# treangenlab/Seqwin

Measured on AMD Instinct MI355X. Metric: Gbp/s minimizer-indexed, higher is better.
Workload: dtype u64

## Files before the change

seqwin_amd/csrc/device.hpp:

```cpp
#pragma once

#include <hip/hip_runtime.h>

#include <functional>
#include <memory>
#include <string>

#include "common.hpp"

namespace sw {

#define SW_HIP(expr)                                                                                   \
    do {                                                                                               \
        hipError_t _e = (expr);                                                                        \
        if (_e != hipSuccess)                                                                          \
            ::sw::raise(SW_ERR_DEVICE, "HIP error %d (%s) at %s:%d: %s", (int)_e, hipGetErrorString(_e), \
                        __FILE__, __LINE__, #expr);                                                    \
    } while (0)

__host__ __device__ inline uint64_t mix64(uint64_t x)
{
    x ^= x >> 30; x *= 0xbf58476d1ce4e5b9ULL;
    x ^= x >> 27; x *= 0x94d049bb133111ebULL;
    x ^= x >> 31;
// ... 94 lines not shown
struct Plan {
    uint32_t k = 0, w = 0;
    uint32_t w_full = 0;
    uint32_t L = 0;
    uint32_t NE = 0;
    uint32_t TW = 0;
    uint32_t Lf = 0, Lg_list = 0, halo_f = 0;
    uint32_t n_tiles = 0, n_tiles_gen = 0;
    struct FastClass {
        uint32_t B = 0;
        uint32_t TW = 0;
        uint32_t n_tiles = 0, n_gap = 0;
        DevArray<uint32_t> rec_off;
        DevArray<TileDesc> desc;
        DevArray<uint32_t> gap_list;
    } fc[2];
    uint64_t n_windows = 0;
    uint64_t n_valid = 0;
    size_t lds_bytes = 0;
    DevArray<uint32_t> rec_seg_off;
    DevArray<uint32_t> rec_nvalid;
    DevArray<uint32_t> rec_tile_off;
    DevArray<uint32_t> gen_tile_off;
    DevArray<uint32_t> gen_tile_rec;
    uint32_t slot_cap = 0;
    DevArray<uint32_t> seg_pos;
    DevArray<uint32_t> seg_idx;
    DevArray<uint64_t> lut;
    DevArray<uint64_t> t4;
    uint64_t mult = 0;
    double build_ms = 0;
};

}

struct sw_batch {
    int device = 0;
    sw::HostBatch host;
    uint64_t n_records = 0;
    uint64_t packed_words = 0;
    sw::DevArray<uint32_t> d_packed;
    sw::DevArray<uint64_t> d_rec_base;
    sw::DevArray<uint32_t> d_rec_asm;
    std::mutex plan_mu;
    std::map<std::pair<uint32_t, uint32_t>, sw::Plan> plans;
};

namespace sw { struct OrderedOcc; }
namespace sw {
bool device_gz_ingest(const char *const *paths, size_t n_paths, uint64_t n_cpu, sw_batch &b);
}

struct sw_occ {
    const sw_batch *batch = nullptr;
    sw::OrderedOcc *occ = nullptr;
    float sketch_ms = 0.f;
    hipStream_t last_stream = nullptr;
    ~sw_occ();
};

namespace sw { struct EdgeHashJob; }
struct sw_index {
    int device = 0;
    uint64_t n_kmers = 0, n_nodes = 0, n_edges = 0;
    sw::DevArray<sw_kmer> kmers;
    sw::DevArray<sw_node> nodes;
    sw::DevArray<sw_edge> edges;
    sw_timings timings{};
    bool ranks_marked = false;
    hipStream_t last_stream = nullptr;
    bool edges_hold_ranks = false;
    sw::EdgeHashJob *hash_job = nullptr;
    sw_index() = default;
    sw_index(const sw_index &) = delete;
    sw_index &operator=(const sw_index &) = delete;
    ~sw_index();
};

namespace sw {

struct MultiGraph {
    std::vector<std::unique_ptr<sw_index>> slices;
    std::vector<uint32_t> record_offsets;
    std::string ids_blob;
    uint64_t n_assemblies = 0, total_bp = 0;
    const char *hash_route = "";
    std::string copy_route;
};
std::vector<int> devices_from_env();
void build_multi_device(const char *const *paths, size_t n_paths, uint64_t k, uint64_t w, uint64_t n_cpu, std::vector<int> devs,
                        MultiGraph &out, uint64_t chunk_bp = 0);

Plan &get_plan(sw_batch &b, uint64_t k, uint64_t w, bool *cached = nullptr);

struct SketchOut {
    DevArray<uint64_t> stage_hash;
    DevArray<uint64_t> stage_kmer;
    DevArray<uint32_t> tile_count;
    DevArray<uint64_t> tile_offset;
    uint64_t n_occ = 0;
    uint64_t launches = 0;
    uint64_t n_ovf_tiles = 0;
};
void run_sketch(const sw_batch &b, const Plan &plan, hipStream_t stream, SketchOut &out, float *sketch_ms);

void radix_sort_keys64(uint64_t *&keys, uint64_t *&alt, uint64_t n, unsigned begin_bit, unsigned end_bit, hipStream_t stream,
                       uint32_t *d_fail, bool perm_hi32 = false, unsigned long long *d_hist_given = nullptr, unsigned layout_bits = 0);
void radix_layout(unsigned bits, unsigned *digit_bits, unsigned *n_passes);
bool radix_unsort_perm(uint64_t *&keys, uint64_t *&alt, uint64_t n, unsigned low_bits, unsigned nbit, hipStream_t stream, uint32_t *d_fail);
constexpr uint32_t UNSORT_CURSOR_STRIDE = 32;
struct UnsortPerm {
    DevArray<unsigned long long> cur_a, cur_b;
    DevArray<uint32_t> tickets;
    unsigned low_bits = 0, hi_bits = 0;
    uint32_t n_groups = 0, n_tiles = 0, grid = 0;
};
bool radix_unsort_perm_begin(UnsortPerm &u, uint64_t n, unsigned low_bits, unsigned nbit, hipStream_t stream);
void radix_unsort_perm_first(UnsortPerm &u, const uint64_t *keys, uint64_t *alt, uint64_t n, hipStream_t stream, uint32_t *d_fail);
void radix_unsort_perm_second(UnsortPerm &u, const uint64_t *keys, uint64_t *alt, uint64_t n, hipStream_t stream, uint32_t *d_fail);

int radix_edge_buckets(uint64_t *&keys, uint64_t *&alt, uint64_t m, unsigned key_bits, uint64_t sentinel,
                       const unsigned long long *d_hist_top, uint32_t cap, uint32_t slots, uint64_t *ukeys, uint32_t *ucnt,
                       uint32_t *n_runs, hipStream_t stream, uint32_t *d_fail, bool debug);

void sort_keys64(uint64_t *&keys, uint64_t *&keys_alt, size_t n, unsigned begin_bit, unsigned end_bit, hipStream_t stream,
                 uint32_t *d_fail, bool perm_hi32 = false, unsigned long long *d_hist_given = nullptr, unsigned layout_bits = 0);
bool sort_keys64_is_own(size_t n);
void check_sort_failed(uint32_t fail_word);

struct alignas(16) OccPay {
    uint32_t low, pos, rec, idx;
};
int radix_rank_mode();
bool radix_pairs_available();
uint64_t radix_trim_state();
void radix_demote_rank();
constexpr uint32_t STAGE_WIN = 32;
constexpr uint32_t STAGE_ROW = STAGE_WIN + 9;
constexpr uint32_t STAGE_PAD = 1;
struct StageSource {
    const uint64_t *stage_hash, *stage_kmer;
    const uint32_t *tile_count;
    const uint64_t *tile_offset;
    const uint64_t *dst_off;
    uint32_t n_tiles;
    uint64_t mult;
    uint32_t *rec_out;
    const unsigned long long *chunk_dir;
    const uint64_t *rows;
};
void radix_sort_pairs32(uint32_t *&keys, uint32_t *&keys_alt, OccPay *&vals, OccPay *&vals_alt, uint64_t n, unsigned end_bit,
                        hipStream_t stream, uint32_t *d_fail, const StageSource *src = nullptr,
                        const std::function<void()> &after_first = std::function<void()>(), uint32_t *low_out = nullptr);
bool sort_pairs32(uint32_t *&keys, uint32_t *&keys_alt, OccPay *&vals, OccPay *&vals_alt, uint64_t n, unsigned end_bit,
                  hipStream_t stream, uint32_t *d_fail, uint32_t *low_out = nullptr);
struct PartState;
void part_state_delete(PartState *p);
uint32_t occ_partition_owners(const struct OrderedOcc &occ);
struct OrderedOcc {
    DevArray<uint64_t> hash;
    DevArray<uint64_t> kmer;
    DevArray<uint32_t> key32;
    DevArray<OccPay> pay;
    DevArray<uint32_t> rec;
    DevArray<uint64_t> cand_rows;
    bool staged = false;
    SketchOut stage;
    DevArray<uint64_t> dst_off;
    uint32_t stage_tiles = 0;
    uint64_t stage_mult = 0;
    uint64_t n = 0;
    PartState *part = nullptr;
    OrderedOcc() = default;
    OrderedOcc(OrderedOcc &&o) noexcept { *this = std::move(o); }
    OrderedOcc &operator=(OrderedOcc &&o) noexcept
    {
        if (this != &o) {
            hash = std::move(o.hash); kmer = std::move(o.kmer); key32 = std::move(o.key32); pay = std::move(o.pay);
            rec = std::move(o.rec); cand_rows = std::move(o.cand_rows); n = o.n; o.n = 0;
            staged = o.staged; o.staged = false; stage = std::move(o.stage); dst_off = std::move(o.dst_off);
            stage_tiles = o.stage_tiles; stage_mult = o.stage_mult;
            part_state_delete(part); part = o.part; o.part = nullptr;
        }
        return *this;
    }
    ~OrderedOcc() { part_state_delete(part); }
};
void order_tuples(SketchOut &sk, const Plan &plan, hipStream_t stream, OrderedOcc &out, bool index_form = false, bool take_stage = false);
void concat_occ(std::vector<OrderedOcc> &chunks, const std::vector<uint64_t> &rec_base, hipStream_t stream, OrderedOcc &out);
void build_index(const uint32_t *d_rec_asm, uint64_t n_records, uint64_t n_assemblies, OrderedOcc &occ,
                 const uint8_t *d_is_target, uint64_t n_targets, uint64_t n_non_targets, hipStream_t stream, sw_index &ix);
void pack_export(const sw_node *nodes, uint64_t n_nodes, uint64_t n_kmers, const sw_edge *edges, uint64_t n_edges, uint64_t per, uint32_t *pn,
                 uint64_t *bases, uint32_t *pe, uint32_t *flag, hipStream_t stream);
void device_get_penalty(const sw_kmer *d_kmers, uint64_t n_kmers, sw_node *d_nodes, uint64_t n_nodes,
                        const uint32_t *d_rec_asm, uint64_t n_records, const uint8_t *d_is_target,
                        uint64_t n_targets, uint64_t n_non_targets, hipStream_t stream, uint64_t *err_flags_host);
void device_filter_kmers(const sw_kmer *d_kmers, uint64_t n_kmers, const sw_node *d_nodes, uint64_t n_nodes,
                         const uint64_t *d_used_sorted, uint64_t n_used, hipStream_t stream,
                         DevArray<sw_kmer> &kmers_out, DevArray<sw_node> &nodes_out, uint64_t *n_kmers_out,
                         uint64_t *n_nodes_out);
void device_identity(const sw_index &ix, hipStream_t stream, uint64_t *sums2, uint64_t kbase = 0, uint64_t nbase = 0);
void slice_get_penalty(sw_index &ix, uint64_t kmer_base, const uint32_t *d_rec_asm, uint64_t n_records, const uint8_t *d_is_target,
                       uint64_t n_targets, uint64_t n_non_targets, hipStream_t stream, uint64_t *err_flags_host);
void device_checksums(const sw_index &ix, hipStream_t stream, uint64_t *sums3, uint64_t kbase = 0, uint64_t nbase = 0,
                      uint64_t ebase = 0);
void index_threshold_sums(const sw_index &ix, hipStream_t stream, uint64_t *sums3);
void index_verify(const sw_index &ix, uint64_t n_assemblies, bool scored, hipStream_t stream, uint64_t *out10);
void index_filter_graph(const sw_index &ix, uint64_t weight_th, hipStream_t stream, sw_index &out);
void index_occ_rows(const sw_index &ix, uint64_t rec_offset, uint64_t *d_rows, hipStream_t stream);
void index_splits(const sw_index &ix, const uint64_t *node_bounds, const uint64_t *edge_bounds, uint32_t n_bounds,
                  uint64_t *occ_split, uint64_t *edge_split, hipStream_t stream);
void merge_build(const uint64_t *d_occ_rows, uint64_t n, const uint64_t *d_edge_rows, uint64_t m, uint64_t kmer_base,
                 const uint32_t *d_rec_asm, uint64_t n_records, const uint8_t *d_is_target, uint64_t n_targets,
                 uint64_t n_non_targets, hipStream_t stream, sw_index &ix, uint32_t *d_rank_out = nullptr);
void occ_partition(const OrderedOcc &occ, const uint64_t *bounds, uint32_t n_bounds, uint64_t rec_offset, uint64_t *d_rows,
                   uint32_t *d_perm, uint64_t *counts_host, hipStream_t stream);
void occ_adjacency(const OrderedOcc &occ, const uint32_t *d_rec_asm, const uint32_t *d_perm, const uint32_t *d_rank_by_row,
                   unsigned nb, unsigned ab, uint64_t asm_base, const uint64_t *rank_bounds, uint32_t n_bounds,
                   uint64_t *d_rows_out, uint64_t *counts_host, hipStream_t stream);
void slice_edges(sw_index &ix, const uint64_t *d_adj_rows, uint64_t m, unsigned nb, unsigned ab, const uint64_t *d_rank_hash,
                 hipStream_t stream);
void occ_adjacency_pairs(OrderedOcc &occ, const uint32_t *d_rec_asm, const uint32_t *d_rank_by_row, const uint64_t *node_base,
                         uint64_t asm_base, const uint64_t *rank_bounds, uint32_t n_bounds, uint64_t *d_keys_out,
                         uint64_t *counts_host, uint64_t *cand_counts_host, uint64_t *key_bits_host, hipStream_t stream);
void slice_edges_pairs(sw_index &ix, uint64_t *d_keys, uint64_t m, const uint64_t *d_cand_rows, uint64_t c, unsigned lo_bits,
                       unsigned hi_bits, uint64_t lo_base, unsigned ab, const uint64_t *d_rank_hash, const uint64_t *node_base,
                       uint32_t n_owners, uint64_t pad, hipStream_t stream);
void index_node_hashes(const sw_index &ix, uint64_t *d_out, hipStream_t stream);
void subgraphs_csr(const sw_subgraphs *sg, int *device, uint64_t *n_sg, uint64_t *n_out, const uint64_t **offsets, const uint64_t **hashes);
uint64_t edge_hash_requests(sw_index &ix, const uint64_t *node_base, uint32_t n_owners, uint64_t *counts_host, hipStream_t stream);
void edge_hash_request_rows(const sw_index &ix, uint32_t *d_out, hipStream_t stream);
void node_hash_lookup(const sw_index &ix, const uint32_t *d_local_ranks, uint64_t n, uint64_t *d_out, hipStream_t stream);
void edge_hash_attach(sw_index &ix, const uint64_t *d_replies, uint64_t n, hipStream_t stream);

}
```

seqwin_amd/csrc/index.hip:

```cpp
#include <cstdlib>
#include <cstring>
#include <map>
#include <memory>

#include <rocprim/rocprim.hpp>

#include "device.hpp"

namespace sw {

namespace {

constexpr int TPB = 256;
inline unsigned blocks_for(uint64_t n, int per = TPB) { return (unsigned)((n + per - 1) / per); }
inline bool ranks_by_table()
{
    const char *e = SW_TEST_GETENV("SEQWIN_AMD_RANKS");
    return e && !strcmp(e, "table");
}

template <class K, class V>
void sort_pairs(K *&keys, K *&keys_alt, V *&vals, V *&vals_alt, size_t n, unsigned begin_bit, unsigned end_bit,
                hipStream_t stream)
{
    rocprim::double_buffer<K> dk(keys, keys_alt);
    rocprim::double_buffer<V> dv(vals, vals_alt);
    size_t tmp_bytes = 0;
    SW_HIP(rocprim::radix_sort_pairs(nullptr, tmp_bytes, dk, dv, n, begin_bit, end_bit, stream));
    DevArray<unsigned char> tmp(tmp_bytes);
    SW_HIP(rocprim::radix_sort_pairs(tmp.p, tmp_bytes, dk, dv, n, begin_bit, end_bit, stream));
    keys = dk.current();
    keys_alt = dk.alternate();
    vals = dv.current();
    vals_alt = dv.alternate();
}

}

bool sort_keys64_is_own(size_t n)
{
    const char *e = SW_TEST_GETENV("SEQWIN_AMD_SORT");
    const bool own = e ? !strcmp(e, "own") : n >= (1ull << 23);
    return own && !(e && !strcmp(e, "rocprim"));
}

void sort_keys64(uint64_t *&keys, uint64_t *&keys_alt, size_t n, unsigned begin_bit, unsigned end_bit, hipStream_t stream,
                 uint32_t *d_fail, bool perm_hi32, unsigned long long *d_hist_given, unsigned layout_bits)
{
    if (sort_keys64_is_own(n)) {
        radix_sort_keys64(keys, keys_alt, n, begin_bit, end_bit, stream, d_fail, perm_hi32, d_hist_given, layout_bits);
        return;
    }
    rocprim::double_buffer<uint64_t> dk(keys, keys_alt);
    size_t tmp_bytes = 0;
    SW_HIP(rocprim::radix_sort_keys(nullptr, tmp_bytes, dk, n, begin_bit, end_bit, stream));
    DevArray<unsigned char> tmp(tmp_bytes);
    SW_HIP(rocprim::radix_sort_keys(tmp.p, tmp_bytes, dk, n, begin_bit, end_bit, stream));
    keys = dk.current();
    keys_alt = dk.alternate();
}

bool sort_pairs_is_own(size_t n, unsigned bits)
{
    const char *e = SW_TEST_GETENV("SEQWIN_AMD_PAIR_SORT"), *all = SW_TEST_GETENV("SEQWIN_AMD_SORT");
    if (e && !strcmp(e, "rocprim")) return false;
    if (bits % 8 != 0 || bits > 32 || n >= 0xFFFFFFFFull) return false;
    bool own = n >= (1ull << 20);
    if (all) own = !strcmp(all, "own");
    if (e && !strcmp(e, "own")) own = true;
    return own && radix_pairs_available();
}

bool sort_pairs32(uint32_t *&keys, uint32_t *&keys_alt, OccPay *&vals, OccPay *&vals_alt, uint64_t n, unsigned end_bit,
                  hipStream_t stream, uint32_t *d_fail, uint32_t *low_out)
{
    if (sort_pairs_is_own(n, end_bit)) {
        radix_sort_pairs32(keys, keys_alt, vals, vals_alt, n, end_bit, stream, d_fail, nullptr, std::function<void()>(), low_out);
        return low_out != nullptr && n != 0 && end_bit != 0;
    }
    sort_pairs(keys, keys_alt, vals, vals_alt, n, 0, end_bit, stream);
    return false;
}

void check_sort_failed(uint32_t fail_word)
{
    if (fail_word)
        raise(SW_ERR_RUNTIME, "internal error: a radix pass gave up waiting for a lower-numbered workgroup (set SEQWIN_AMD_SORT=rocprim)");
}

namespace {

template <class InIt, class OutIt, class T>
void inclusive_sum(InIt in, OutIt out, size_t n, T, hipStream_t stream)
{
    size_t tmp_bytes = 0;
    SW_HIP(rocprim::inclusive_scan(nullptr, tmp_bytes, in, out, n, rocprim::plus<T>(), stream));
    DevArray<unsigned char> tmp(tmp_bytes);
    SW_HIP(rocprim::inclusive_scan(tmp.p, tmp_bytes, in, out, n, rocprim::plus<T>(), stream));
}

template <class InIt, class OutIt, class T>
void inclusive_sum_keep(InIt in, OutIt out, size_t n, T, hipStream_t stream, DevArray<unsigned char> &tmp)
{
    size_t tmp_bytes = 0;
    SW_HIP(rocprim::inclusive_scan(nullptr, tmp_bytes, in, out, n, rocprim::plus<T>(), stream));
    tmp.alloc(tmp_bytes);
    SW_HIP(rocprim::inclusive_scan(tmp.p, tmp_bytes, in, out, n, rocprim::plus<T>(), stream));
}

template <class InIt, class OutIt, class T>
void exclusive_sum(InIt in, OutIt out, size_t n, T init, hipStream_t stream)
{
    size_t tmp_bytes = 0;
    SW_HIP(rocprim::exclusive_scan(nullptr, tmp_bytes, in, out, init, n, rocprim::plus<T>(), stream));
    DevArray<unsigned char> tmp(tmp_bytes);
    SW_HIP(rocprim::exclusive_scan(tmp.p, tmp_bytes, in, out, init, n, rocprim::plus<T>(), stream));
}

struct U32ToU64 {
    __host__ __device__ uint64_t operator()(uint32_t v) const { return v; }
};

struct HeadFlag {
    const uint64_t *keys;
    uint64_t sentinel;
    __host__ __device__ uint32_t operator()(uint64_t s) const
    {
        const uint64_t k = keys[s];
        return (k != sentinel && (s == 0 || k != keys[s - 1])) ? 1u : 0u;
    }
};

template <bool INDEX, bool RAW = false>
__global__ void k_order(const uint64_t *__restrict__ stage_hash, const uint64_t *__restrict__ stage_kmer,
                        const uint32_t *__restrict__ tile_count, const uint64_t *__restrict__ tile_offset,
                        const uint64_t *__restrict__ dst_off, uint32_t n_tiles, uint64_t mult, uint64_t *__restrict__ hash,
                        uint64_t *__restrict__ kmer, uint32_t *__restrict__ key32, OccPay *__restrict__ pay,
                        uint32_t *__restrict__ rec)
{
    const uint32_t wave = (blockIdx.x * blockDim.x + threadIdx.x) >> 6;
    const uint32_t lane = threadIdx.x & 63u;
    if (wave >= n_tiles) return;
    const uint32_t c = tile_count[wave];
    const uint64_t src = tile_offset[wave], dst = dst_off[wave];
    for (uint32_t i = lane; i < c; i += 64) {
        uint64_t h = stage_hash[src + i];
        if (!RAW) {
            h *= mult;
            h ^= h >> 27;
        }
        const uint64_t km = stage_kmer[src + i];
        if (INDEX) {
            key32[dst + i] = (uint32_t)(h >> 32);
            OccPay p;
            p.low = (uint32_t)h;
            p.pos = (uint32_t)km;
            p.rec = (uint32_t)(km >> 32);
            p.idx = (uint32_t)(dst + i);
            pay[dst + i] = p;
            rec[dst + i] = p.rec;
            if (hash) hash[dst + i] = h;
        } else {
            hash[dst + i] = h;
            kmer[dst + i] = km;
        }
    }
}

__global__ void k_rows_to_pay(const uint64_t *__restrict__ rows, uint64_t n, uint32_t *__restrict__ key32, OccPay *__restrict__ pay)
{
    const uint64_t i = (uint64_t)blockIdx.x * blockDim.x + threadIdx.x;
    if (i >= n) return;
    const uint64_t h = rows[2 * i], km = rows[2 * i + 1];
    key32[i] = (uint32_t)(h >> 32);
    OccPay p;
    p.low = (uint32_t)h;
    p.pos = (uint32_t)km;
    p.rec = (uint32_t)(km >> 32);
    p.idx = (uint32_t)i;
    pay[i] = p;
}

__global__ void k_iota(uint32_t *v, uint64_t n)
{
    const uint64_t i = (uint64_t)blockIdx.x * blockDim.x + threadIdx.x;
    if (i < n) v[i] = (uint32_t)i;
}

#ifndef SW_NODES_ROWS
#define SW_NODES_ROWS 4
#endif
constexpr int NODES_ROWS = SW_NODES_ROWS;
constexpr int NODES_THREADS = 1024;
constexpr int NODES_WAVES = NODES_THREADS / 64;
constexpr uint32_t NODES_ROW = NODES_THREADS * 2;
constexpr uint32_t NODES_TILE = NODES_ROW * NODES_ROWS;
constexpr uint32_t UNSORT_BITS = 14;
constexpr uint32_t UNSORT_RANGE = 1u << UNSORT_BITS;
constexpr bool UNSORT_FUSED_DEFAULT = true;
constexpr uint64_t UNSORT_DIRECT_MAX = 1ull << 25;

constexpr unsigned long long TS_AGG = 1ull << 62, TS_INC = 2ull << 62;

__device__ __forceinline__ unsigned long long interleave32(uint32_t a, uint32_t b)
{
    unsigned long long x = a, y = b;
    x = (x | (x << 16)) & 0x0000FFFF0000FFFFull; y = (y | (y << 16)) & 0x0000FFFF0000FFFFull;
    x = (x | (x << 8)) & 0x00FF00FF00FF00FFull;  y = (y | (y << 8)) & 0x00FF00FF00FF00FFull;
    x = (x | (x << 4)) & 0x0F0F0F0F0F0F0F0Full;  y = (y | (y << 4)) & 0x0F0F0F0F0F0F0F0Full;
    x = (x | (x << 2)) & 0x3333333333333333ull;  y = (y | (y << 2)) & 0x3333333333333333ull;
    x = (x | (x << 1)) & 0x5555555555555555ull;  y = (y | (y << 1)) & 0x5555555555555555ull;
    return x | (y << 1);
}

constexpr uint32_t RANK_REP = 0x80000000u;
constexpr uint8_t OWNER_DROP = 0xFF;
constexpr uint32_t NODES_DIGITS = 256;
struct NodesScat {
    uint64_t stage[NODES_TILE];
    unsigned long long goff[NODES_DIGITS];
    uint32_t cnt[NODES_DIGITS];
    uint32_t lstart[NODES_DIGITS];
};
template <bool BITS, bool REP, bool SCAT = false>
__global__ __launch_bounds__(NODES_THREADS) void k_nodes(const uint32_t *__restrict__ key32, const OccPay *__restrict__ pay, uint64_t n,
                                               uint64_t base, const uint32_t *__restrict__ rec_flag, sw_kmer *__restrict__ kmers,
                                               uint64_t *__restrict__ node_hash, uint32_t *__restrict__ node_start,
                                               uint32_t *__restrict__ rank_direct,
                                               uint64_t *__restrict__ uval,
                                               unsigned long long *__restrict__ tbits, unsigned long long *__restrict__ nbits,
                                               unsigned long long *__restrict__ tile_state, uint32_t *__restrict__ ticket,
                                               uint32_t *__restrict__ n_nodes_out, uint32_t *__restrict__ order_bad,
                                               unsigned long long *__restrict__ cursor, uint32_t dig_shift, uint32_t dig_mask)
{
    __shared__ uint32_t s_tile, s_excl;
    __shared__ uint32_t s_row[NODES_ROWS * NODES_WAVES];
    static_assert(NODES_ROWS * NODES_WAVES <= 128, "the (row, wave) group counts are scanned by one wave, two per lane");
    const uint32_t lane = threadIdx.x & 63u, wave = threadIdx.x >> 6;
    NodesScat *sc = nullptr;
    if constexpr (SCAT) {
        __shared__ NodesScat s_scat;
        sc = &s_scat;
        if (threadIdx.x < NODES_DIGITS) sc->cnt[threadIdx.x] = 0;
    }
    if (threadIdx.x == 0) s_tile = atomicAdd(ticket, 1u);
    __syncthreads();
    const uint32_t tile = s_tile;
    const uint64_t s0 = (uint64_t)tile * NODES_TILE;
    uint32_t k[NODES_ROWS][2], within[NODES_ROWS], headm = 0, prec[NODES_ROWS];
    OccPay p[NODES_ROWS][2];
    unsigned long long misorder = 0;
#pragma unroll
    for (int r = 0; r < NODES_ROWS; ++r) {
        const uint64_t s = s0 + (uint64_t)r * NODES_ROW + 2 * threadIdx.x;
        k[r][0] = k[r][1] = 0;
        p[r][0] = p[r][1] = OccPay{0, 0, 0, 0};
        if (s + 1 < n) {
            const uint2 kk = *reinterpret_cast<const uint2 *>(key32 + s);
            k[r][0] = kk.x;
            k[r][1] = kk.y;
            p[r][0] = pay[s];
            p[r][1] = pay[s + 1];
        } else if (s < n) {
            k[r][0] = key32[s];
            p[r][0] = pay[s];
        }
        uint32_t pk = __shfl_up(k[r][1], 1, 64), plow = __shfl_up(p[r][1].low, 1, 64), pidx = __shfl_up(p[r][1].idx, 1, 64);
        prec[r] = __shfl_up(p[r][1].rec, 1, 64);
        if (lane == 0 && s < n && s) {
            pk = key32[s - 1];
            const OccPay q = pay[s - 1];
            plow = q.low;
            prec[r] = q.rec;
            pidx = q.idx;
        }
        const bool h0 = s < n && (s == 0 || k[r][0] != pk || p[r][0].low != plow);
        const bool h1 = s + 1 < n && (k[r][1] != k[r][0] || p[r][1].low != p[r][0].low);
#ifndef SW_NO_ORDER_GUARD
        {
            const unsigned long long hp = ((unsigned long long)pk << 32) | plow, h0v = ((unsigned long long)k[r][0] << 32) | p[r][0].low,
                                     h1v = ((unsigned long long)k[r][1] << 32) | p[r][1].low;
            const bool bad0 = s < n && s && (h0v < hp || (!h0 && p[r][0].idx <= pidx));
            const bool bad1 = s + 1 < n && (h1v < h0v || (!h1 && p[r][1].idx <= p[r][0].idx));
            misorder |= __ballot(bad0 || bad1);
        }
#else
        (void)pidx;
#endif
        const unsigned long long b0 = __ballot(h0), b1 = __ballot(h1), lt = (1ull << lane) - 1ull;
        within[r] = (uint32_t)__popcll(b0 & lt) + (uint32_t)__popcll(b1 & lt);
        if (h0) headm |= 1u << (2 * r);
        if (h1) headm |= 2u << (2 * r);
        if (lane == 0) s_row[r * NODES_WAVES + wave] = (uint32_t)__popcll(b0) + (uint32_t)__popcll(b1);
    }
    if (misorder && lane == 0) atomicAdd(order_bad, (uint32_t)__popcll(misorder));
    uint32_t drank[NODES_ROWS][2];
    if constexpr (SCAT) {
#pragma unroll
        for (int r = 0; r < NODES_ROWS; ++r)
#pragma unroll
            for (int e = 0; e < 2; ++e) {
                drank[r][e] = 0;
                if (s0 + (uint64_t)r * NODES_ROW + 2 * threadIdx.x + e < n)
                    drank[r][e] = atomicAdd(&sc->cnt[(p[r][e].idx >> dig_shift) & dig_mask], 1u);
            }
    }
    __syncthreads();
    if (SCAT && wave == 1) {
        const uint4 c4 = reinterpret_cast<const uint4 *>(sc->cnt)[lane];
        const uint32_t c[4] = {c4.x, c4.y, c4.z, c4.w};
        unsigned long long g[4];
#pragma unroll
        for (int j = 0; j < 4; ++j)
            g[j] = c[j] ? atomicAdd(&cursor[(size_t)(4 * lane + j) * UNSORT_CURSOR_STRIDE], (unsigned long long)c[j]) : 0ull;
        uint32_t incl = c[0] + c[1] + c[2] + c[3];
        for (uint32_t d = 1; d < 64; d <<= 1) {
            const uint32_t up = __shfl_up(incl, d, 64);
            if (lane >= d) incl += up;
        }
        uint32_t before = incl - (c[0] + c[1] + c[2] + c[3]);
#pragma unroll
        for (int j = 0; j < 4; ++j) {
            sc->lstart[4 * lane + j] = before;
            sc->goff[4 * lane + j] = g[j] - before;
            before += c[j];
        }
    }
    if (wave == 0) {
        constexpr uint32_t GROUPS = NODES_ROWS * NODES_WAVES;
        const uint32_t c0 = (2 * lane < GROUPS) ? s_row[2 * lane] : 0u, c1 = (2 * lane + 1 < GROUPS) ? s_row[2 * lane + 1] : 0u;
        uint32_t incl = c0 + c1;
        for (uint32_t d = 1; d < 64; d <<= 1) {
            const uint32_t up = __shfl_up(incl, d, 64);
            if (lane >= d) incl += up;
        }
        const uint32_t total = __shfl(incl, 63, 64);
        if (2 * lane < GROUPS) s_row[2 * lane] = incl - c0 - c1;
        if (2 * lane + 1 < GROUPS) s_row[2 * lane + 1] = incl - c1;
        if (lane == 0)
            __hip_atomic_store(&tile_state[tile], (tile == 0 ? TS_INC : TS_AGG) | total, __ATOMIC_RELAXED, __HIP_MEMORY_SCOPE_AGENT);
        uint32_t excl = 0;
        if (tile) {
            int64_t look = (int64_t)tile - 1;
            for (;;) {
                const int64_t idx = look - lane;
                const unsigned long long st = idx >= 0 ? __hip_atomic_load(&tile_state[idx], __ATOMIC_RELAXED, __HIP_MEMORY_SCOPE_AGENT)
                                                       : TS_INC;
                const unsigned long long inc = __ballot((st >> 62) == 2), none = __ballot((st >> 62) == 0);
                const uint32_t first_inc = inc ? (uint32_t)__builtin_ctzll(inc) : 64u;
                const unsigned long long needed = first_inc >= 63 ? ~0ull : ((2ull << first_inc) - 1ull);
                if (none & needed) {
                    __builtin_amdgcn_s_sleep(2);
                    continue;
                }
                uint32_t v = (lane <= first_inc) ? (uint32_t)st : 0u;
                for (int d = 32; d; d >>= 1) v += __shfl_xor(v, d, 64);
                excl += v;
                if (first_inc < 64) break;
                look -= 64;
            }
            if (lane == 0)
                __hip_atomic_store(&tile_state[tile], TS_INC | (unsigned long long)(excl + total), __ATOMIC_RELAXED,
                                   __HIP_MEMORY_SCOPE_AGENT);
        }
        if (lane == 0) {
            s_excl = excl;
            if (s0 + NODES_TILE >= n) *n_nodes_out = excl + total;
        }
    }
    __syncthreads();
    const uint32_t excl = s_excl;
    if constexpr (SCAT) {
#pragma unroll
        for (int r = 0; r < NODES_ROWS; ++r)
#pragma unroll
            for (int e = 0; e < 2; ++e) drank[r][e] += sc->lstart[(p[r][e].idx >> dig_shift) & dig_mask];
    }
#pragma unroll
    for (int r = 0; r < NODES_ROWS; ++r) {
        const uint64_t s = s0 + (uint64_t)r * NODES_ROW + 2 * threadIdx.x;
        const bool live0 = s < n, live1 = s + 1 < n;
        const bool h0 = (headm >> (2 * r)) & 1u, h1 = (headm >> (2 * r + 1)) & 1u;
        const uint32_t nid0 = excl + s_row[r * NODES_WAVES + wave] + within[r] + (h0 ? 1u : 0u) - 1u;
        const uint32_t nid1 = nid0 + (h1 ? 1u : 0u);
        uint32_t w0 = nid0, w1 = nid1;
        uint32_t f0 = 0, f1 = 0, pf = 0;
        if (BITS || REP) {
            f0 = live0 ? rec_flag[p[r][0].rec] : 0u;
            f1 = live1 ? rec_flag[p[r][1].rec] : 0u;
            pf = __shfl_up(f1, 1, 64);
            if (lane == 0 && live0 && s) pf = rec_flag[prec[r]];
        }
        if (REP) {
            uint32_t nk = __shfl_down(k[r][0], 1, 64), nlow = __shfl_down(p[r][0].low, 1, 64), nf = __shfl_down(f0, 1, 64);
            bool nlive = __shfl_down((int)live0, 1, 64) != 0;
            if (lane == 63) {
                nlive = s + 2 < n;
                if (nlive) {
                    nk = key32[s + 2];
                    const OccPay q = pay[s + 2];
                    nlow = q.low;
                    nf = rec_flag[q.rec];
                }
            }
            const bool same01 = live1 && !h1 && (f1 >> 1) == (f0 >> 1);
            const bool same_p0 = live0 && !h0 && (f0 >> 1) == (pf >> 1);
            const bool same_1n = live1 && nlive && nk == k[r][1] && nlow == p[r][1].low && (nf >> 1) == (f1 >> 1);
            if (same_p0 || same01) w0 |= RANK_REP;
            if (same01 || same_1n) w1 |= RANK_REP;
        }
        if (live1) {
            *reinterpret_cast<uint4 *>(kmers + s) = make_uint4(p[r][0].pos, p[r][0].rec, p[r][1].pos, p[r][1].rec);
            if (!SCAT && uval)
                *reinterpret_cast<ulonglong2 *>(uval + s) = make_ulonglong2(((uint64_t)p[r][0].idx << 32) | w0,
                                                                          ((uint64_t)p[r][1].idx << 32) | w1);
        } else if (live0) {
            sw_kmer km;
            km.pos = p[r][0].pos;
            km.record_idx = p[r][0].rec;
            kmers[s] = km;
            if (!SCAT && uval) uval[s] = ((uint64_t)p[r][0].idx << 32) | w0;
        }
        if constexpr (SCAT) {
            if (live0) sc->stage[drank[r][0]] = ((uint64_t)p[r][0].idx << 32) | w0;
            if (live1) sc->stage[drank[r][1]] = ((uint64_t)p[r][1].idx << 32) | w1;
        }
        if (rank_direct) {
            if (live0) rank_direct[p[r][0].idx] = w0;
            if (live1) rank_direct[p[r][1].idx] = w1;
        }
#pragma unroll
        for (int e = 0; e < 2; ++e) {
            const bool head = e ? h1 : h0;
            if (head) {
                const uint32_t nid = e ? nid1 : nid0;
                node_hash[nid] = ((uint64_t)k[r][e] << 32) | p[r][e].low;
                node_start[nid] = (uint32_t)(s + e);
            }
        }
        if (BITS) {
            const bool first0 = live0 && (h0 || (f0 >> 1) != (pf >> 1)), first1 = live1 && (h1 || (f1 >> 1) != (f0 >> 1));
            const unsigned long long t0 = __ballot(first0 && (f0 & 1u)), t1 = __ballot(first1 && (f1 & 1u));
            const unsigned long long g0 = __ballot(first0 && !(f0 & 1u)), g1 = __ballot(first1 && !(f1 & 1u));
            if (lane == 0 && live0) {
                const uint64_t wd = s >> 6;
                tbits[wd] = interleave32((uint32_t)t0, (uint32_t)t1);
                nbits[wd] = interleave32((uint32_t)g0, (uint32_t)g1);
                if (s + 64 < n) {
                    tbits[wd + 1] = interleave32((uint32_t)(t0 >> 32), (uint32_t)(t1 >> 32));
                    nbits[wd + 1] = interleave32((uint32_t)(g0 >> 32), (uint32_t)(g1 >> 32));
                }
            }
        }
    }
    if constexpr (SCAT) {
        asm volatile("s_waitcnt lgkmcnt(0)" ::: "memory");
        __builtin_amdgcn_s_barrier();
        asm volatile("" ::: "memory");
        const uint32_t cnt_tile = (uint32_t)min((uint64_t)NODES_TILE, n - s0);
        constexpr int OUT = NODES_TILE / NODES_THREADS;
        uint64_t word[OUT], at[OUT];
#pragma unroll
        for (int j = 0; j < OUT; ++j) word[j] = sc->stage[j * NODES_THREADS + threadIdx.x];
#pragma unroll
        for (int j = 0; j < OUT; ++j) at[j] = sc->goff[(uint32_t)(word[j] >> (32 + dig_shift)) & dig_mask] + (j * NODES_THREADS + threadIdx.x);
#pragma unroll
        for (int j = 0; j < OUT; ++j)
            if (j * NODES_THREADS + threadIdx.x < cnt_tile && at[j] < n) uval[at[j]] = word[j];
    }
}

__device__ __forceinline__ uint32_t popc_range(const unsigned long long *__restrict__ w, uint64_t a, uint64_t b)
{
    if (a >= b) return 0;
    const uint64_t wa = a >> 6, wb = (b - 1) >> 6;
    const unsigned long long ma = ~0ull << (a & 63u), mb = ~0ull >> (63u - ((b - 1) & 63u));
    if (wa == wb) return (uint32_t)__popcll(w[wa] & ma & mb);
    uint32_t c = (uint32_t)__popcll(w[wa] & ma) + (uint32_t)__popcll(w[wb] & mb);
    for (uint64_t i = wa + 1; i < wb; ++i) c += (uint32_t)__popcll(w[i]);
    return c;
}

constexpr int FIN_THREADS = 256;
template <bool BITS>
__global__ __launch_bounds__(FIN_THREADS) void k_finish_nodes(sw_node *__restrict__ nodes, uint64_t n_nodes, const uint64_t *__restrict__ node_hash,
                                                              const uint32_t *__restrict__ node_start, uint64_t base, uint64_t end,
                                                              const unsigned long long *__restrict__ tbits,
                                                              const unsigned long long *__restrict__ nbits, double inv_tar, double inv_neg)
{
    static_assert(sizeof(sw_node) == 40, "five 8-byte words per node");
    __shared__ __align__(16) unsigned long long stage[FIN_THREADS * 5];
    const uint64_t i0 = (uint64_t)blockIdx.x * FIN_THREADS, i = i0 + threadIdx.x;
    if (i < n_nodes) {
        const uint32_t a = node_start[i];
        const uint64_t b = i + 1 < n_nodes ? (uint64_t)node_start[i + 1] : end - base;
        uint32_t n_tar = 0, n_neg = 0;
        double pen = 0.0;
        if (BITS) {
            n_tar = popc_range(tbits, a, b);
            n_neg = popc_range(nbits, a, b);
            {
#pragma clang fp contract(off)
                const double ft = (double)n_tar * inv_tar;
                const double fn = (double)n_neg * inv_neg;
                const double omf = 1.0 - ft;
                const double aa = omf * omf;
                const double bb = fn * fn;
                const double sum = aa + bb;
                pen = __dsqrt_rn(sum);
            }
        }
        unsigned long long *w = stage + threadIdx.x * 5;
        w[0] = node_hash[i];
        w[1] = base + a;
        w[2] = base + b;
        w[3] = ((unsigned long long)n_neg << 32) | n_tar;
        w[4] = (unsigned long long)__double_as_longlong(pen);
    }
    __syncthreads();
    const uint64_t cnt = min((uint64_t)FIN_THREADS, n_nodes - i0);
    const uint32_t n16 = (uint32_t)(cnt * 40 / 16), tail8 = (uint32_t)((cnt * 40) % 16) / 8;
    uint4 *dst = reinterpret_cast<uint4 *>(nodes + i0);
    const uint4 *src = reinterpret_cast<const uint4 *>(stage);
    for (uint32_t t = threadIdx.x; t < n16; t += FIN_THREADS) dst[t] = src[t];
    if (tail8 && threadIdx.x == 0) reinterpret_cast<unsigned long long *>(nodes + i0)[n16 * 2] = stage[n16 * 2];
}

__global__ void k_rec_flag(const uint32_t *__restrict__ rec_asm, const uint8_t *__restrict__ is_target, uint64_t n_records,
                           uint32_t *__restrict__ rec_flag)
{
    const uint64_t r = (uint64_t)blockIdx.x * blockDim.x + threadIdx.x;
    if (r < n_records) {
        const uint32_t a = rec_asm[r];
        rec_flag[r] = (a << 1) | ((is_target && is_target[a]) ? 1u : 0u);
    }
}

constexpr unsigned long long TABLE_EMPTY = ~0ull;
__device__ __forceinline__ uint64_t table_mix(uint64_t x)
{
    return x ^ (x >> 29);
}

__global__ void k_table_build(const sw_node *__restrict__ nodes, uint64_t n_nodes, ulonglong2 *__restrict__ slots, uint64_t mask,
                              uint32_t *__restrict__ rank_of_empty_key)
{
    const uint64_t r = (uint64_t)blockIdx.x * blockDim.x + threadIdx.x;
    if (r >= n_nodes) return;
    const unsigned long long h = nodes[r].hash;
    if (h == TABLE_EMPTY) {
        *rank_of_empty_key = (uint32_t)r;
        return;
    }
    uint64_t s = table_mix(h) & mask;
    for (;;) {
// ... 942 lines not shown
    nd.start = ns;
    nd.stop = ns + sz;
    nodes_out[o] = nd;
}

__global__ void k_filter_kmers(const sw_kmer *__restrict__ kmers, const uint64_t *__restrict__ src_start,
                               const uint64_t *__restrict__ dst_start, uint64_t n_kept, uint64_t n_out,
                               sw_kmer *__restrict__ out)
{
    const uint64_t j = (uint64_t)blockIdx.x * blockDim.x + threadIdx.x;
    if (j >= n_out) return;
    uint64_t lo = 0, hi = n_kept;
    while (hi - lo > 1) {
        const uint64_t mid = (lo + hi) >> 1;
        if (dst_start[mid] <= j) lo = mid; else hi = mid;
    }
    out[j] = kmers[src_start[lo] + (j - dst_start[lo])];
}

__global__ void k_checksum(const sw_kmer *kmers, uint64_t nk, const sw_node *nodes, uint64_t nn, const sw_edge *edges,
                           uint64_t ne, uint64_t kbase, uint64_t nbase, uint64_t ebase, unsigned long long *sums)
{
    const uint64_t i = (uint64_t)blockIdx.x * blockDim.x + threadIdx.x;
    uint64_t a = 0, b = 0, c = 0;
    if (i < nk) a = ck_kmer(kbase + i, kmers[i]);
    if (i < nn) b = ck_node(nbase + i, nodes[i]);
    if (i < ne) c = ck_edge(ebase + i, edges[i]);
    for (int d = 32; d; d >>= 1) {
        a += __shfl_down(a, d, 64);
        b += __shfl_down(b, d, 64);
        c += __shfl_down(c, d, 64);
    }
    if ((threadIdx.x & 63u) == 0) {
        if (a) atomicAdd(&sums[0], (unsigned long long)a);
        if (b) atomicAdd(&sums[1], (unsigned long long)b);
        if (c) atomicAdd(&sums[2], (unsigned long long)c);
    }
}

__global__ void k_verify_nodes(const sw_node *__restrict__ nodes, uint64_t n_nodes, uint64_t n_kmers, uint64_t base,
                               uint64_t n_assemblies, int scored, uint32_t *__restrict__ start_bits,
                               unsigned long long *__restrict__ out)
{
    const uint64_t i = (uint64_t)blockIdx.x * blockDim.x + threadIdx.x;
    if (i >= n_nodes) return;
    const sw_node nd = nodes[i];
    if (i && !(nodes[i - 1].hash < nd.hash)) atomicAdd(&out[0], 1ull);
    const uint64_t prev_stop = i ? nodes[i - 1].stop : base;
    bool bad = nd.start != prev_stop || nd.stop <= nd.start || nd.stop - base > n_kmers;
    if (i == n_nodes - 1 && nd.stop - base != n_kmers) bad = true;
    if (bad) atomicAdd(&out[1], 1ull);
    else atomicOr(&start_bits[(nd.start - base) >> 5], 1u << ((nd.start - base) & 31u));
    if (scored) {
        const uint64_t c = (uint64_t)nd.n_tar + nd.n_neg, size = nd.stop - nd.start;
        if (c < 1 || c > size || c > n_assemblies) atomicAdd(&out[7], 1ull);
    }
}

__global__ void k_verify_kmers(const sw_kmer *__restrict__ kmers, uint64_t n, const uint32_t *__restrict__ start_bits,
                               unsigned long long *__restrict__ out)
{
    const uint64_t s = (uint64_t)blockIdx.x * blockDim.x + threadIdx.x;
    unsigned long long bad = 0, first_of_record = 0;
    if (s < n) {
        const uint64_t cur = ((uint64_t)kmers[s].record_idx << 32) | kmers[s].pos;
        const bool head = (start_bits[s >> 5] >> (s & 31u)) & 1u;
        if (s && !head) {
            const uint64_t prev = ((uint64_t)kmers[s - 1].record_idx << 32) | kmers[s - 1].pos;
            if (!(prev < cur)) bad = 1;
        }
    }
    (void)first_of_record;
    for (int d = 32; d; d >>= 1) bad += __shfl_down(bad, d, 64);
    if ((threadIdx.x & 63u) == 0 && bad) atomicAdd(&out[2], bad);
}

__global__ void k_verify_edges(const sw_edge *__restrict__ edges, uint64_t n_edges, const sw_node *__restrict__ nodes,
                               uint64_t n_nodes, const uint64_t *__restrict__ rank_hash, uint64_t n_rank_hash,
                               uint64_t n_assemblies, unsigned long long *__restrict__ out)
{
    const uint64_t e = (uint64_t)blockIdx.x * blockDim.x + threadIdx.x;
    unsigned long long wsum = 0;
    if (e < n_edges) {
        const sw_edge ed = edges[e];
        if (e) {
            const sw_edge pe = edges[e - 1];
            if (!(pe.first < ed.first || (pe.first == ed.first && pe.second < ed.second))) atomicAdd(&out[3], 1ull);
        }
        if (ed.first > ed.second) atomicAdd(&out[4], 1ull);
        if (ed.weight < 1 || ed.weight > n_assemblies) atomicAdd(&out[5], 1ull);
        wsum = ed.weight;
        for (int side = 0; side < 2; ++side) {
            const uint64_t h = side ? ed.second : ed.first;
            bool found;
            if (rank_hash) {
                uint64_t lo = 0, hi = n_rank_hash;
                while (lo < hi) {
                    const uint64_t mid = (lo + hi) >> 1;
                    if (rank_hash[mid] < h) lo = mid + 1; else hi = mid;
                }
                found = lo < n_rank_hash && rank_hash[lo] == h;
            } else {
                const uint64_t lo = node_index_of(nodes, n_nodes, h);
                found = lo < n_nodes && nodes[lo].hash == h;
            }
            if (!found) atomicAdd(&out[6], 1ull);
        }
    }
    for (int d = 32; d; d >>= 1) wsum += __shfl_down(wsum, d, 64);
    if ((threadIdx.x & 63u) == 0 && wsum) atomicAdd(&out[8], wsum);
}

__global__ void k_rot_keys(uint32_t *__restrict__ key32, uint64_t n, unsigned left)
{
    const uint64_t i = (uint64_t)blockIdx.x * blockDim.x + threadIdx.x;
    if (i < n) {
        const uint32_t k = key32[i];
        key32[i] = (k << left) | (k >> (32u - left));
    }
}

constexpr uint32_t DESC_BLOCK = 1024;

struct PayView {
    using Key = uint32_t;
    using Elem = OccPay;
    uint32_t *key32;
    OccPay *pay;
    __device__ uint32_t key(uint64_t q) const { return key32[q]; }
    __device__ uint64_t low(uint64_t q) const { return pay[q].low; }
    __device__ static uint64_t low_of(const OccPay &v) { return v.low; }
    __device__ void load(uint64_t q, uint32_t &k, OccPay &v) const { k = key32[q]; v = pay[q]; }
    __device__ void store(uint64_t q, uint32_t k, const OccPay &v) const { key32[q] = k; pay[q] = v; }
};
struct LowView {
    using Key = uint32_t;
    const uint32_t *key32;
    const uint32_t *low32;
    __device__ uint32_t key(uint64_t q) const { return key32[q]; }
    __device__ uint64_t low(uint64_t q) const { return low32[q]; }
};
struct EdgeKeyView {
    using Key = uint64_t;
    using Elem = uint64_t;
    uint64_t *keys;
    unsigned low_bits;
    __device__ uint64_t key(uint64_t q) const { return keys[q] >> low_bits; }
    __device__ uint64_t low(uint64_t q) const { return keys[q]; }
    __device__ static uint64_t low_of(const uint64_t &v) { return v; }
    __device__ void load(uint64_t q, uint64_t &k, uint64_t &v) const { v = keys[q]; k = v >> low_bits; }
    __device__ void store(uint64_t q, uint64_t, const uint64_t &v) const { keys[q] = v; }
};

template <class View>
__device__ __forceinline__ uint32_t descents_of_thread(const View &V, typename View::Key kmask, uint64_t n, uint64_t q0, uint32_t *heads = nullptr)
{
    uint32_t m = 0, hm = 0;
    if (heads) *heads = 0;
    if (q0 >= n) return 0;
    typename View::Key kp = q0 ? V.key(q0 - 1) : 0;
    uint64_t lp = q0 ? V.low(q0 - 1) : 0;
#pragma unroll
    for (uint32_t i = 0; i < 4; ++i) {
        const uint64_t q = q0 + i;
        if (q >= n) break;
        const typename View::Key kq = V.key(q);
        const uint64_t lq = V.low(q);
        if (q && (kq & kmask) == (kp & kmask) && (kq < kp || (kq == kp && lq < lp))) m |= 1u << i;
        if (q == 0 || kq != kp || lq != lp) hm |= 1u << i;
        kp = kq;
        lp = lq;
    }
    if (heads) *heads = (uint32_t)__popc(hm);
    return m;
}

__device__ __forceinline__ uint32_t descents_of_thread(const PayView &V, uint32_t kmask, uint64_t n, uint64_t q0, uint32_t *heads = nullptr)
{
    uint32_t m = 0, hm = 0;
    if (heads) *heads = 0;
    if (q0 >= n) return 0;
    uint32_t kq[4];
    uint64_t lq[4];
    if (q0 + 4 <= n) {
        const uint4 kv = *reinterpret_cast<const uint4 *>(V.key32 + q0);
        kq[0] = kv.x; kq[1] = kv.y; kq[2] = kv.z; kq[3] = kv.w;
#pragma unroll
        for (uint32_t i = 0; i < 4; ++i) lq[i] = reinterpret_cast<const uint4 *>(V.pay + q0 + i)->x;
    } else {
#pragma unroll
        for (uint32_t i = 0; i < 4; ++i) {
            kq[i] = (q0 + i < n) ? V.key32[q0 + i] : 0u;
            lq[i] = (q0 + i < n) ? V.pay[q0 + i].low : 0u;
        }
    }
    uint32_t kp = q0 ? V.key32[q0 - 1] : 0;
    uint64_t lp = q0 ? V.pay[q0 - 1].low : 0;
#pragma unroll
    for (uint32_t i = 0; i < 4; ++i) {
        const uint64_t q = q0 + i;
        if (q >= n) break;
        if (q && (kq[i] & kmask) == (kp & kmask) && (kq[i] < kp || (kq[i] == kp && lq[i] < lp))) m |= 1u << i;
        if (q == 0 || kq[i] != kp || lq[i] != lp) hm |= 1u << i;
        kp = kq[i];
        lp = lq[i];
    }
    if (heads) *heads = (uint32_t)__popc(hm);
    return m;
}

__device__ __forceinline__ uint32_t descents_of_thread(const LowView &V, uint32_t kmask, uint64_t n, uint64_t q0, uint32_t *heads = nullptr)
{
    uint32_t m = 0, hm = 0;
    if (heads) *heads = 0;
    if (q0 >= n) return 0;
    uint32_t kq[4], lq[4];
    if (q0 + 4 <= n) {
        const uint4 kv = *reinterpret_cast<const uint4 *>(V.key32 + q0), lv = *reinterpret_cast<const uint4 *>(V.low32 + q0);
        kq[0] = kv.x; kq[1] = kv.y; kq[2] = kv.z; kq[3] = kv.w;
        lq[0] = lv.x; lq[1] = lv.y; lq[2] = lv.z; lq[3] = lv.w;
    } else {
#pragma unroll
        for (uint32_t i = 0; i < 4; ++i) {
            kq[i] = (q0 + i < n) ? V.key32[q0 + i] : 0u;
            lq[i] = (q0 + i < n) ? V.low32[q0 + i] : 0u;
        }
    }
    uint32_t kp = q0 ? V.key32[q0 - 1] : 0, lp = q0 ? V.low32[q0 - 1] : 0;
#pragma unroll
    for (uint32_t i = 0; i < 4; ++i) {
        const uint64_t q = q0 + i;
        if (q >= n) break;
        if (q && (kq[i] & kmask) == (kp & kmask) && (kq[i] < kp || (kq[i] == kp && lq[i] < lp))) m |= 1u << i;
        if (q == 0 || kq[i] != kp || lq[i] != lp) hm |= 1u << i;
        kp = kq[i];
        lp = lq[i];
    }
    if (heads) *heads = (uint32_t)__popc(hm);
    return m;
}

constexpr uint32_t DESC_SLOT = 4;
template <class View>
__global__ __launch_bounds__(256) void k_count_descents(const View V, typename View::Key kmask, uint64_t n, unsigned long long *__restrict__ cnt,
                                                        uint32_t *__restrict__ slot_q, uint32_t *__restrict__ slot_k)
{
    const uint64_t q0 = (uint64_t)blockIdx.x * DESC_BLOCK + threadIdx.x * 4u;
    uint32_t heads = 0;
    const uint32_t m = descents_of_thread(V, kmask, n, q0, &heads);
    const uint32_t c = (uint32_t)__popc(m);
    __shared__ unsigned long long s;
    __shared__ uint32_t s_n, s_q[DESC_SLOT], s_kk[DESC_SLOT];
    if (threadIdx.x == 0) {
        s = 0;
        s_n = 0;
    }
    __syncthreads();
    unsigned long long w = ((unsigned long long)heads << 32) | c;
    for (int d = 32; d; d >>= 1) w += __shfl_down(w, d, 64);
    if ((threadIdx.x & 63u) == 0 && w) atomicAdd(&s, w);
    __syncthreads();
    const uint32_t dc = (uint32_t)s;
    if (threadIdx.x == 0) cnt[blockIdx.x] = s;
    if (dc == 0 || dc > DESC_SLOT) return;
    uint32_t mm = m;
    while (mm) {
        const uint32_t i = (uint32_t)__builtin_ctz(mm);
        mm &= mm - 1;
        const uint32_t at = atomicAdd(&s_n, 1u);
        s_q[at] = (uint32_t)(q0 + i);
        s_kk[at] = (uint32_t)(V.key(q0 + i) & kmask);
    }
    __syncthreads();
    if (threadIdx.x == 0) {
        for (uint32_t i = 1; i < dc; ++i)
            for (uint32_t j = i; j > 0 && s_q[j] < s_q[j - 1]; --j) {
                const uint32_t tq = s_q[j], tk = s_kk[j];
                s_q[j] = s_q[j - 1];
                s_kk[j] = s_kk[j - 1];
                s_q[j - 1] = tq;
                s_kk[j - 1] = tk;
            }
        for (uint32_t i = 0; i < dc; ++i) {
            slot_q[(size_t)blockIdx.x * DESC_SLOT + i] = s_q[i];
            slot_k[(size_t)blockIdx.x * DESC_SLOT + i] = s_kk[i];
        }
    }
}

template <class View>
__global__ __launch_bounds__(256) void k_list_descents(const View V, typename View::Key kmask, uint64_t n,
                                                       const unsigned long long *__restrict__ cnt,
                                                       const unsigned long long *__restrict__ off, uint32_t n_blocks,
                                                       uint32_t *__restrict__ bad, uint32_t cap, uint32_t *__restrict__ bad_q,
                                                       uint32_t cap_q, unsigned long long *__restrict__ n_desc,
                                                       const uint32_t *__restrict__ slot_q, const uint32_t *__restrict__ slot_k)
{
    const uint32_t b = blockIdx.x;
    const uint32_t c_blk = (uint32_t)cnt[b];
    if (b == n_blocks - 1 && threadIdx.x == 0) {
        const unsigned long long tot = off[b] + cnt[b];
        n_desc[0] = tot & 0xFFFFFFFFull;
        n_desc[1] = tot >> 32;
    }
    if (c_blk == 0) return;
    if (c_blk <= DESC_SLOT) {
        if (threadIdx.x < c_blk) {
            const uint32_t at = (uint32_t)off[b] + threadIdx.x;
            if (bad && at < cap) bad[at] = slot_k[(size_t)b * DESC_SLOT + threadIdx.x];
            if (at < cap_q) bad_q[at] = slot_q[(size_t)b * DESC_SLOT + threadIdx.x];
        }
        return;
    }
    const uint64_t q0 = (uint64_t)b * DESC_BLOCK + threadIdx.x * 4u;
    const uint32_t m = descents_of_thread(V, kmask, n, q0);
    const uint32_t c = (uint32_t)__popc(m);
    __shared__ uint32_t wsum[4];
    const uint32_t lane = threadIdx.x & 63u, wave = threadIdx.x >> 6;
    uint32_t incl = c;
    for (uint32_t d = 1; d < 64; d <<= 1) {
        const uint32_t up = __shfl_up(incl, d, 64);
        if (lane >= d) incl += up;
    }
    if (lane == 63) wsum[wave] = incl;
    __syncthreads();
    uint32_t base = (uint32_t)off[b] + (incl - c);
    for (uint32_t i = 0; i < wave; ++i) base += wsum[i];
    uint32_t mm = m;
    while (mm) {
        const uint32_t i = (uint32_t)__builtin_ctz(mm);
        mm &= mm - 1;
        if (base < cap) bad[base] = (uint32_t)(V.key(q0 + i) & kmask);
        if (base < cap_q) bad_q[base] = (uint32_t)(q0 + i);
        ++base;
    }
}

constexpr uint32_t REPAIR_MAX_DESC = 1u << 26;
constexpr uint32_t REPAIR_MAX_MID = 1u << 22;
constexpr uint32_t REPAIR_THREAD_RUN = 6;
constexpr uint32_t REPAIR_MAX_RUN = 2048;
constexpr uint32_t REPAIR_GRID = 2048;

__device__ __forceinline__ uint64_t readlane64(uint64_t v, uint32_t lane)
{
    const uint32_t lo = (uint32_t)__builtin_amdgcn_readlane((int)(uint32_t)v, (int)lane);
    const uint32_t hi = (uint32_t)__builtin_amdgcn_readlane((int)(uint32_t)(v >> 32), (int)lane);
    return ((uint64_t)hi << 32) | lo;
}

__device__ __forceinline__ uint32_t readlane_key(uint32_t v, uint32_t lane) { return (uint32_t)__builtin_amdgcn_readlane((int)v, (int)lane); }
__device__ __forceinline__ uint64_t readlane_key(uint64_t v, uint32_t lane) { return readlane64(v, lane); }

template <class View>
__global__ __launch_bounds__(256) void k_repair_thread(const View V, typename View::Key kmask, uint64_t n, const uint32_t *__restrict__ bad_q,
                                                       const unsigned long long *__restrict__ n_desc, uint32_t *__restrict__ mid,
                                                       uint32_t *__restrict__ n_mid, uint32_t *__restrict__ status)
{
// ... 95 lines not shown
        if (have) {
            V.load(a + lane, ki, vi);
            li = View::low_of(vi);
        }
        uint32_t rank = 0;
        for (uint32_t j = 0; j < len; ++j) {
            const typename View::Key kj = readlane_key(ki, j);
            const uint64_t lj = readlane64(li, j);
            rank += (kj < ki || (kj == ki && (lj < li || (lj == li && j < lane)))) ? 1u : 0u;
        }
        if (have) V.store(a + rank, ki, vi);
    }
}

constexpr uint32_t REPAIR_MAX_VALUES = 12;
template <class View>
__global__ __launch_bounds__(256) void k_repair_sort(const View V, const uint32_t *__restrict__ n_big, const uint32_t *__restrict__ big)
{
    __shared__ typename View::Elem sv[REPAIR_MAX_RUN];
    __shared__ typename View::Key sk[REPAIR_MAX_RUN];
    __shared__ uint16_t srank[REPAIR_MAX_RUN];
    __shared__ typename View::Key w_k[4];
    __shared__ uint32_t w_cnt[4];
    __shared__ uint64_t w_l[4];
    const uint32_t B = *n_big;
    const uint32_t tid = threadIdx.x, lane = tid & 63u, wave = tid >> 6;
    for (uint32_t b = blockIdx.x; b < B; b += gridDim.x) {
        const uint32_t a = big[2 * b], len = big[2 * b + 1];
        __syncthreads();
        for (uint32_t i = tid; i < len; i += blockDim.x) V.load(a + i, sk[i], sv[i]);
        __syncthreads();
        const uint32_t per = (len + 255u) / 256u, i0 = min(len, tid * per), i1 = min(len, i0 + per);
        uint32_t placed = 0;
        typename View::Key last_k = 0;
        uint64_t last_l = 0;
        bool have_last = false;
        for (uint32_t it = 0; it < REPAIR_MAX_VALUES && placed < len; ++it) {
            typename View::Key mk = ~(typename View::Key)0;
            uint64_t ml = ~0ull;
            bool any = false;
            for (uint32_t i = i0; i < i1; ++i) {
                const typename View::Key k = sk[i];
                const uint64_t l = View::low_of(sv[i]);
                if (have_last && !(k > last_k || (k == last_k && l > last_l))) continue;
                if (!any || k < mk || (k == mk && l < ml)) {
                    mk = k;
                    ml = l;
                    any = true;
                }
            }
            for (int d = 32; d; d >>= 1) {
                const typename View::Key ok = __shfl_xor(mk, d, 64);
                const uint64_t ol = __shfl_xor(ml, d, 64);
                const bool oany = __shfl_xor((int)any, d, 64) != 0;
                if (oany && (!any || ok < mk || (ok == mk && ol < ml))) {
                    mk = ok;
                    ml = ol;
                    any = true;
                }
            }
            __syncthreads();
            if (lane == 0) {
                w_k[wave] = mk;
                w_l[wave] = ml;
                w_cnt[wave] = any ? 1u : 0u;
            }
            __syncthreads();
            any = false;
            for (uint32_t w = 0; w < 4; ++w)
                if (w_cnt[w] && (!any || w_k[w] < mk || (w_k[w] == mk && w_l[w] < ml))) {
                    mk = w_k[w];
                    ml = w_l[w];
                    any = true;
                }
            uint32_t c = 0;
            for (uint32_t i = i0; i < i1; ++i) c += (sk[i] == mk && View::low_of(sv[i]) == ml) ? 1u : 0u;
            uint32_t incl = c;
            for (uint32_t d = 1; d < 64; d <<= 1) {
                const uint32_t up = __shfl_up(incl, d, 64);
                if (lane >= d) incl += up;
            }
            __syncthreads();
            if (lane == 63) w_cnt[wave] = incl;
            __syncthreads();
            uint32_t before = placed + incl - c, total = 0;
            for (uint32_t w = 0; w < 4; ++w) {
                if (w < wave) before += w_cnt[w];
                total += w_cnt[w];
            }
            for (uint32_t i = i0; i < i1; ++i)
                if (sk[i] == mk && View::low_of(sv[i]) == ml) srank[i] = (uint16_t)before++;
            placed += total;
            last_k = mk;
            last_l = ml;
            have_last = true;
        }
        __syncthreads();
        if (placed == len) {
            for (uint32_t i = tid; i < len; i += blockDim.x) V.store(a + srank[i], sk[i], sv[i]);
        } else {
            for (uint32_t i = tid; i < len; i += blockDim.x) {
                const typename View::Key ki = sk[i];
                const typename View::Elem vi = sv[i];
                const uint64_t li = View::low_of(vi);
                uint32_t rank = 0;
                for (uint32_t j = 0; j < len; ++j) {
                    const typename View::Key kj = sk[j];
                    const uint64_t lj = View::low_of(sv[j]);
                    rank += (kj < ki || (kj == ki && (lj < li || (lj == li && j < i)))) ? 1u : 0u;
                }
                V.store(a + rank, ki, vi);
            }
        }
    }
}

struct RepairState {
    DevArray<unsigned long long> n_desc;
    DevArray<unsigned long long> blk_cnt, blk_off;
    DevArray<uint32_t> slot_q, slot_k;
    DevArray<uint32_t> bad_q, mid, big, status;
};

template <class View, class Sweep>
void enqueue_repair(const View &V, const Sweep &W, typename View::Key kmask, uint64_t n, uint32_t *bad, uint32_t cap, RepairState &r,
                    hipStream_t stream)
{
    const uint32_t n_blocks = (uint32_t)((n + DESC_BLOCK - 1) / DESC_BLOCK);
    const uint32_t max_desc = (uint32_t)std::min<uint64_t>(REPAIR_MAX_DESC, std::max<uint64_t>(n, 1));
    const uint32_t max_mid = std::min(max_desc, REPAIR_MAX_MID);
    r.bad_q.alloc(max_desc);
    r.mid.alloc(max_mid);
    r.big.alloc(2 * (size_t)max_mid);
    r.n_desc.alloc(2);
    r.status.alloc(3);
    r.blk_cnt.alloc(n_blocks);
    r.blk_off.alloc(n_blocks);
    r.slot_q.alloc((size_t)n_blocks * DESC_SLOT);
    r.slot_k.alloc((size_t)n_blocks * DESC_SLOT);
    SW_HIP(hipMemsetAsync(r.status.p, 0, 12, stream));
    hipLaunchKernelGGL(k_count_descents<Sweep>, dim3(n_blocks), dim3(256), 0, stream, W, kmask, n, r.blk_cnt.p, r.slot_q.p, r.slot_k.p);
    SW_HIP(hipGetLastError());
    exclusive_sum(r.blk_cnt.p, r.blk_off.p, n_blocks, 0ull, stream);
    hipLaunchKernelGGL(k_list_descents<Sweep>, dim3(n_blocks), dim3(256), 0, stream, W, kmask, n, r.blk_cnt.p, r.blk_off.p,
                       n_blocks, bad, cap, r.bad_q.p, max_desc, r.n_desc.p, r.slot_q.p, r.slot_k.p);
    hipLaunchKernelGGL(k_repair_thread<View>, dim3(REPAIR_GRID), dim3(256), 0, stream, V, kmask, n, r.bad_q.p, r.n_desc.p, r.mid.p,
                       r.status.p + 2, r.status.p);
    hipLaunchKernelGGL(k_repair_wave<View>, dim3(REPAIR_GRID), dim3(256), 0, stream, V, kmask, n, r.bad_q.p, r.n_desc.p,
                       (const uint32_t *)r.mid.p, (const uint32_t *)(r.status.p + 2), r.big.p, r.status.p + 1, r.status.p);
    hipLaunchKernelGGL(k_repair_sort<View>, dim3(REPAIR_GRID), dim3(256), 0, stream, V, r.status.p + 1, r.big.p);
    SW_HIP(hipGetLastError());
}

__global__ void k_bad_runs(const uint32_t *__restrict__ bad, uint32_t n_bad, const uint32_t *__restrict__ key32,
                           uint32_t kmask, uint64_t n, uint32_t *__restrict__ run_start, uint32_t *__restrict__ run_len)
{
    const uint32_t i = blockIdx.x * blockDim.x + threadIdx.x;
    if (i >= n_bad) return;
    const uint32_t k = bad[i];
    if (i && bad[i - 1] == k) {
        run_start[i] = 0;
        run_len[i] = 0;
        return;
    }
    uint64_t lo = 0, hi = n;
    while (lo < hi) {
        const uint64_t mid = (lo + hi) >> 1;
        if ((key32[mid] & kmask) < k) lo = mid + 1; else hi = mid;
    }
    const uint64_t a = lo;
    hi = n;
    while (lo < hi) {
        const uint64_t mid = (lo + hi) >> 1;
        if ((key32[mid] & kmask) <= k) lo = mid + 1; else hi = mid;
    }
    run_start[i] = (uint32_t)a;
    run_len[i] = (uint32_t)(lo - a);
}

__global__ void k_gather_sub(const uint32_t *__restrict__ key32, const OccPay *__restrict__ pay,
                             const uint32_t *__restrict__ run_start, const uint64_t *__restrict__ run_off, uint32_t n_bad,
                             uint64_t n_sub, uint64_t *__restrict__ sub_h, OccPay *__restrict__ sub_v,
                             uint32_t *__restrict__ pos)
{
    const uint64_t t = (uint64_t)blockIdx.x * blockDim.x + threadIdx.x;
    if (t >= n_sub) return;
    uint64_t q = t;
    if (run_off) {
        uint32_t lo = 0, hi = n_bad;
        while (hi - lo > 1) {
            const uint32_t mid = (lo + hi) >> 1;
            if (run_off[mid] <= t) lo = mid; else hi = mid;
        }
        q = (uint64_t)run_start[lo] + (t - run_off[lo]);
        pos[t] = (uint32_t)q;
    }
    const OccPay v = pay[q];
    sub_h[t] = ((uint64_t)key32[q] << 32) | v.low;
    sub_v[t] = v;
}

__global__ void k_scatter_sub(const uint64_t *__restrict__ sub_h, const OccPay *__restrict__ sub_v,
                              const uint32_t *__restrict__ pos, uint64_t n_sub, uint32_t *__restrict__ key32,
                              OccPay *__restrict__ pay)
{
    const uint64_t t = (uint64_t)blockIdx.x * blockDim.x + threadIdx.x;
    if (t >= n_sub) return;
    const uint64_t q = pos ? pos[t] : t;
    key32[q] = (uint32_t)(sub_h[t] >> 32);
    pay[q] = sub_v[t];
}

struct PaySort {
    DevArray<uint32_t> key_a, key_b;
    DevArray<OccPay> pay_a, pay_b;
    uint32_t *key32 = nullptr;
    OccPay *pay = nullptr;
    uint64_t n_repaired = 0;
    DevArray<uint32_t> bad;
    RepairState rep;
    uint32_t cap = 0, kmask = ~0u;
    uint64_t n = 0;
    DevArray<uint32_t> fail;
    DevArray<uint32_t> low;
    const uint64_t *rows_src = nullptr;
    OrderedOcc *staged = nullptr;
};

void sort_pay(uint64_t n, hipStream_t stream, PaySort &o)
{
    unsigned bits = 32;
    if (const char *e = SW_TEST_GETENV("SEQWIN_AMD_SORT_KEYBITS")) {
        const int b = atoi(e);
        if (b >= 1 && b <= 32) bits = (unsigned)b;
    }
    o.kmask = ~0u << (32 - bits);
    o.n = n;
    o.key_b.alloc(n);
    o.pay_b.alloc(n);
    uint32_t *keys = o.key_a.p, *keys_alt = o.key_b.p;
    OccPay *vals = o.pay_a.p, *vals_alt = o.pay_b.p;
    bool have_low = false;
    const bool want_low = bits == 32 && !(SW_AB_GETENV("SEQWIN_AMD_DESC_LOW") && atoi(SW_AB_GETENV("SEQWIN_AMD_DESC_LOW")) == 0);
    if (o.staged) {
        OrderedOcc &occ = *o.staged;
        StageSource S{};
        S.stage_hash = occ.stage.stage_hash.p;
        S.stage_kmer = occ.stage.stage_kmer.p;
        S.tile_count = occ.stage.tile_count.p;
        S.tile_offset = occ.stage.tile_offset.p;
        S.dst_off = occ.dst_off.p;
        S.n_tiles = occ.stage_tiles;
        S.mult = occ.stage_mult;
        S.rec_out = occ.rec.p;
        o.fail.alloc(1);
        SW_HIP(hipMemsetAsync(o.fail.p, 0, 4, stream));
        if (want_low) o.low.alloc(n);
        have_low = want_low && n != 0;
        radix_sort_pairs32(keys, keys_alt, vals, vals_alt, n, 32, stream, o.fail.p, &S, [&] {
            occ.stage = SketchOut();
            occ.dst_off.release();
            occ.staged = false;
            o.key_a.alloc(n);
            o.pay_a.alloc(n);
            keys = o.key_a.p;
            vals = o.pay_a.p;
        }, o.low.p);
        o.staged = nullptr;
    } else if (o.rows_src) {
        StageSource S{};
        S.rows = o.rows_src;
        o.fail.alloc(1);
        SW_HIP(hipMemsetAsync(o.fail.p, 0, 4, stream));
        if (want_low) o.low.alloc(n);
        have_low = want_low && n != 0;
        radix_sort_pairs32(keys, keys_alt, vals, vals_alt, n, 32, stream, o.fail.p, &S, [&] {
            o.key_a.alloc(n);
            o.pay_a.alloc(n);
            keys = o.key_a.p;
            vals = o.pay_a.p;
        }, o.low.p);
    } else {
        if (bits < 32) {
            hipLaunchKernelGGL(k_rot_keys, dim3(blocks_for(n)), dim3(TPB), 0, stream, keys, n, bits);
            SW_HIP(hipGetLastError());
        }
        o.fail.alloc(1);
        SW_HIP(hipMemsetAsync(o.fail.p, 0, 4, stream));
        if (want_low && sort_pairs_is_own(n, bits)) o.low.alloc(n);
        have_low = sort_pairs32(keys, keys_alt, vals, vals_alt, n, bits, stream, o.fail.p, o.low.p);
        if (bits < 32) {
            hipLaunchKernelGGL(k_rot_keys, dim3(blocks_for(n)), dim3(TPB), 0, stream, keys, n, 32 - bits);
            SW_HIP(hipGetLastError());
        }
    }
    o.key32 = keys;
    o.pay = vals;
    o.cap = (uint32_t)std::min<uint64_t>(n, std::max<uint64_t>(1u << 16, n / 16));
    o.bad.alloc(o.cap);
    if (have_low) enqueue_repair(PayView{keys, vals}, LowView{keys, o.low.p}, o.kmask, n, o.bad.p, o.cap, o.rep, stream);
    else enqueue_repair(PayView{keys, vals}, PayView{keys, vals}, o.kmask, n, o.bad.p, o.cap, o.rep, stream);
}

bool sort_pay_settle(PaySort &o, unsigned long long D, uint32_t status, hipStream_t stream)
{
    if (D == 0 || status == 0) {
        o.n_repaired = D;
        return false;
    }
    const uint64_t n = o.n;
    const uint32_t kmask = o.kmask, cap = o.cap;
    uint32_t *keys = o.key32;
    OccPay *vals = o.pay;
    DevArray<uint32_t> &bad = o.bad;
    uint64_t n_sub = n;
    DevArray<uint32_t> run_start, run_len, pos;
    DevArray<uint64_t> run_off;
    const bool listed = D <= cap;
    if (listed) {
        const uint32_t nb = (uint32_t)D;
        run_start.alloc(nb);
        run_len.alloc(nb);
        run_off.alloc((size_t)nb + 1);
        hipLaunchKernelGGL(k_bad_runs, dim3((unsigned)blocks_for(nb)), dim3(TPB), 0, stream, bad.p, nb, keys, kmask, n,
                           run_start.p, run_len.p);
        SW_HIP(hipGetLastError());
        exclusive_sum(rocprim::make_transform_iterator(run_len.p, U32ToU64()), run_off.p, nb, (uint64_t)0, stream);
        uint64_t last_off = 0;
        uint32_t last_len = 0;
        SW_HIP(hipMemcpyAsync(&last_off, run_off.p + (nb - 1), 8, hipMemcpyDeviceToHost, stream));
        SW_HIP(hipMemcpyAsync(&last_len, run_len.p + (nb - 1), 4, hipMemcpyDeviceToHost, stream));
        SW_HIP(hipStreamSynchronize(stream));
        n_sub = last_off + last_len;
        pos.alloc(n_sub);
    }
    DevArray<uint64_t> sh0(n_sub), sh1(n_sub);
    DevArray<OccPay> sp0(n_sub), sp1(n_sub);
    hipLaunchKernelGGL(k_gather_sub, dim3(blocks_for(n_sub)), dim3(TPB), 0, stream, keys, vals, run_start.p,
                       listed ? run_off.p : (const uint64_t *)nullptr, (uint32_t)(listed ? D : 0), n_sub, sh0.p, sp0.p, pos.p);
    SW_HIP(hipGetLastError());
    uint64_t *sk = sh0.p, *sk_alt = sh1.p;
    OccPay *sv = sp0.p, *sv_alt = sp1.p;
    sort_pairs(sk, sk_alt, sv, sv_alt, n_sub, 0, 64, stream);
    hipLaunchKernelGGL(k_scatter_sub, dim3(blocks_for(n_sub)), dim3(TPB), 0, stream, sk, sv,
                       listed ? pos.p : (const uint32_t *)nullptr, n_sub, keys, vals);
    SW_HIP(hipGetLastError());
    SW_HIP(hipStreamSynchronize(stream));
    o.n_repaired = n_sub;
    return true;
}

uint64_t settle_sort(PaySort &ps, hipStream_t stream)
{
    uint32_t status = 0, failed = 0;
    unsigned long long dh[2] = {0, 0};
    SW_HIP(hipMemcpyAsync(&status, ps.rep.status.p, 4, hipMemcpyDeviceToHost, stream));
    SW_HIP(hipMemcpyAsync(dh, ps.rep.n_desc.p, 16, hipMemcpyDeviceToHost, stream));
    if (ps.fail.p) SW_HIP(hipMemcpyAsync(&failed, ps.fail.p, 4, hipMemcpyDeviceToHost, stream));
    SW_HIP(hipStreamSynchronize(stream));
    check_sort_failed(failed);
    sort_pay_settle(ps, dh[0], status, stream);
    return dh[1];
}

struct UnsortHold {
    DevArray<uint64_t> a, b;
    const uint64_t *sorted = nullptr;
};
struct NodeParts {
    DevArray<uint64_t> hash;
    DevArray<uint32_t> start;
};
void finish_nodes(sw_index &ix, const NodeParts &np, uint64_t base, uint64_t end, const unsigned long long *tbits,
                  const unsigned long long *nbits, double inv_tar, double inv_neg, hipStream_t stream)
{
    if (!ix.n_nodes) return;
    const dim3 grid((unsigned)((ix.n_nodes + FIN_THREADS - 1) / FIN_THREADS));
    if (tbits && nbits)
        hipLaunchKernelGGL(k_finish_nodes<true>, grid, dim3(FIN_THREADS), 0, stream, ix.nodes.p, ix.n_nodes, (const uint64_t *)np.hash.p,
                           (const uint32_t *)np.start.p, base, end, tbits, nbits, inv_tar, inv_neg);
    else
        hipLaunchKernelGGL(k_finish_nodes<false>, grid, dim3(FIN_THREADS), 0, stream, ix.nodes.p, ix.n_nodes, (const uint64_t *)np.hash.p,
                           (const uint32_t *)np.start.p, base, end, (const unsigned long long *)nullptr,
                           (const unsigned long long *)nullptr, 0.0, 0.0);
    SW_HIP(hipGetLastError());
}

__global__ void k_restore_stream(const uint32_t *__restrict__ key32, const OccPay *__restrict__ pay, uint64_t n, uint64_t *__restrict__ key64,
                                 OccPay *__restrict__ out, uint32_t *__restrict__ bad)
{
    const uint64_t i = (uint64_t)blockIdx.x * blockDim.x + threadIdx.x;
    if (i >= n) return;
    const OccPay q = pay[i];
    if (q.idx >= n) {
        atomicAdd(bad, 1u);
        return;
    }
    key64[q.idx] = ((uint64_t)key32[i] << 32) | q.low;
    out[q.idx] = q;
}
__global__ void k_split_restored(const uint64_t *__restrict__ key64, const OccPay *__restrict__ pay, uint64_t n, uint32_t *__restrict__ key32,
                                 uint32_t *__restrict__ bad)
{
    const uint64_t i = (uint64_t)blockIdx.x * blockDim.x + threadIdx.x;
    if (i >= n) return;
    key32[i] = (uint32_t)(key64[i] >> 32);
    if (pay[i].idx == 0xFFFFFFFFu) atomicAdd(bad, 1u);
}
void resort_pay_stable(PaySort &ps, uint64_t n, hipStream_t stream)
{
    OccPay *cur = ps.pay, *other = (ps.pay == ps.pay_a.p) ? ps.pay_b.p : ps.pay_a.p;
    if (!other || !cur) raise(SW_ERR_RUNTIME, "internal error: the node sort's second buffer is gone");
    DevArray<uint64_t> k0(n), k1(n);
    DevArray<uint32_t> bad(1);
    SW_HIP(hipMemsetAsync(bad.p, 0, 4, stream));
    SW_HIP(hipMemsetAsync(other, 0xFF, n * sizeof(OccPay), stream));
    hipLaunchKernelGGL(k_restore_stream, dim3(blocks_for(n)), dim3(TPB), 0, stream, ps.key32, cur, n, k0.p, other, bad.p);
    SW_HIP(hipGetLastError());
    uint64_t *k = k0.p, *k_alt = k1.p;
    OccPay *v = other, *v_alt = cur;
    sort_pairs(k, k_alt, v, v_alt, n, 0, 64, stream);
    hipLaunchKernelGGL(k_split_restored, dim3(blocks_for(n)), dim3(TPB), 0, stream, k, v, n, ps.key32, bad.p);
    SW_HIP(hipGetLastError());
    uint32_t nbad = 0;
    SW_HIP(hipMemcpyAsync(&nbad, bad.p, 4, hipMemcpyDeviceToHost, stream));
    SW_HIP(hipStreamSynchronize(stream));
    if (nbad) raise(SW_ERR_RUNTIME, "internal error: the node sort lost %u occurrences (not a permutation of its input)", nbad);
    ps.pay = v;
}
uint32_t group_occurrences(PaySort &ps, uint64_t n, uint64_t base, const uint32_t *rec_flag, hipStream_t stream, sw_index &ix,
                           uint32_t *rank_out, DevArray<unsigned long long> *tbits, DevArray<unsigned long long> *nbits,
                           bool *rep_marked = nullptr, UnsortHold *hold = nullptr, NodeParts *parts = nullptr)
{
    sort_pay(n, stream, ps);
    const uint64_t node_cap = settle_sort(ps, stream);
    ix.nodes.alloc(node_cap);
    NodeParts own_parts;
    NodeParts &np = parts ? *parts : own_parts;
    np.hash.alloc(node_cap);
    np.start.alloc(node_cap);
    uint64_t direct_max = UNSORT_DIRECT_MAX;
    if (const char *e = SW_TEST_GETENV("SEQWIN_AMD_UNSORT_DIRECT")) direct_max = 1ull << std::min(40, std::max(0, atoi(e)));
    const bool direct = rank_out && n <= direct_max;
    DevArray<uint64_t> uv0, uv1;
    if (rank_out && !direct) uv0.alloc(n);
    const bool bits = rec_flag && tbits && nbits;
    const bool rep = rec_flag && rep_marked && rank_out && node_cap < (1ull << 31);
    if (rep_marked) *rep_marked = rep;
    if (bits) {
        tbits->alloc((n + 63) / 64);
        nbits->alloc((n + 63) / 64);
    }
    const unsigned blocks = (unsigned)((n + NODES_TILE - 1) / NODES_TILE);
    DevArray<unsigned long long> tile_state(blocks);
    DevArray<uint32_t> words(4);
    uint32_t back[3] = {0, 0, 0};
    if (rank_out && !direct) uv1.alloc(n);
    unsigned nbit = 1;
    while (nbit < 32 && (1ull << nbit) < n) ++nbit;
    bool want_fused = UNSORT_FUSED_DEFAULT;
    if (const char *e = SW_TEST_GETENV("SEQWIN_AMD_UNSORT_FUSED")) want_fused = atoi(e) != 0;
    UnsortPerm perm;
    const char *route = !rank_out ? "none" : direct ? "direct" : nbit <= UNSORT_BITS ? "one bucket" : "sort";
    for (int attempt = 0;; ++attempt) {
        SW_HIP(hipMemsetAsync(tile_state.p, 0, (size_t)blocks * 8, stream));
        SW_HIP(hipMemsetAsync(words.p, 0, 16, stream));
        const bool fused = want_fused && rank_out && !direct && nbit > UNSORT_BITS && sort_keys64_is_own(n) &&
                           radix_unsort_perm_begin(perm, n, UNSORT_BITS, nbit, stream);
        {
            auto launch = [&](auto kern) {
                hipLaunchKernelGGL(kern, dim3(blocks), dim3(NODES_THREADS), 0, stream, ps.key32, ps.pay, n, base, rec_flag, ix.kmers.p,
                                   np.hash.p, np.start.p, direct ? rank_out : (uint32_t *)nullptr, fused ? uv1.p : uv0.p,
                                   bits ? tbits->p : (unsigned long long *)nullptr, bits ? nbits->p : (unsigned long long *)nullptr,
                                   tile_state.p, words.p, words.p + 1, words.p + 3, fused ? perm.cur_a.p : (unsigned long long *)nullptr,
                                   fused ? perm.low_bits + 8 : 0u, fused ? (1u << perm.hi_bits) - 1u : 0u);
            };
            if (fused) {
                if (bits && rep) launch(k_nodes<true, true, true>);
                else if (bits) launch(k_nodes<true, false, true>);
                else if (rep) launch(k_nodes<false, true, true>);
                else launch(k_nodes<false, false, true>);
            } else if (bits && rep) launch(k_nodes<true, true>);
            else if (bits) launch(k_nodes<true, false>);
            else if (rep) launch(k_nodes<false, true>);
            else launch(k_nodes<false, false>);
        }
        SW_HIP(hipGetLastError());
        if (rank_out && !direct) {
            uint64_t *v = uv0.p;
            if (fused) {
                radix_unsort_perm_second(perm, uv1.p, uv0.p, n, stream, words.p + 2);
                route = "fused";
            } else if (nbit > UNSORT_BITS) {
                uint64_t *v_alt = uv1.p;
                if (sort_keys64_is_own(n) && radix_unsort_perm(v, v_alt, n, UNSORT_BITS, nbit, stream, words.p + 2)) route = "two passes";
                else sort_keys64(v, v_alt, n, 32 + UNSORT_BITS, 32 + nbit, stream, words.p + 2, true);
            }
            if (hold && rep && nbit > UNSORT_BITS && !SW_TEST_GETENV("SEQWIN_AMD_ADJ_SEPARATE")) {
                hold->sorted = v;
            } else {
                hipLaunchKernelGGL(k_unsort_bucket, dim3((unsigned)((n + UNSORT_RANGE - 1) / UNSORT_RANGE)), dim3(1024), 0, stream, v, n,
                                   rank_out);
                SW_HIP(hipGetLastError());
            }
        }
        SW_HIP(hipMemcpyAsync(back, words.p + 1, 12, hipMemcpyDeviceToHost, stream));
        SW_HIP(hipStreamSynchronize(stream));
        if (getenv("SEQWIN_AMD_DEBUG_NODES"))
            fprintf(stderr, "[nodes] %llu occurrences (indices of %u bits), attempt %d: unsort route %s, %u nodes, order guard %u\n",
                    (unsigned long long)n, nbit, attempt, route, back[0], back[2]);
        if (back[2] == 0) break;
        if (attempt)
            raise(SW_ERR_RUNTIME, "internal error: the node sort is still out of order after the rocPRIM re-sort (%u places)", back[2]);
        order_guard_tripped(0, back[2]);
        radix_demote_rank();
        resort_pay_stable(ps, n, stream);
    }
    const uint32_t n_nodes = back[0];
    check_sort_failed(back[1]);
    if (n_nodes > node_cap) raise(SW_ERR_RUNTIME, "internal error: %u nodes exceed the bound %llu", n_nodes, (unsigned long long)node_cap);
    ix.n_nodes = n_nodes;
    if (!parts) {
        finish_nodes(ix, np, base, base + n, nullptr, nullptr, 0.0, 0.0, stream);
        SW_HIP(hipStreamSynchronize(stream));
    }
    if (hold && hold->sorted) {
        hold->a = std::move(uv0);
        hold->b = std::move(uv1);
    }
    return n_nodes;
}

void ranks_from_table(const sw_index &ix, const uint64_t *hash, uint64_t n, hipStream_t stream, uint32_t *rank)
{
    uint64_t cap = 1024;
    while (cap < 2 * ix.n_nodes) cap <<= 1;
    DevArray<ulonglong2> slots(cap);
    DevArray<uint32_t> special(1);
    SW_HIP(hipMemsetAsync(slots.p, 0xFF, cap * sizeof(ulonglong2), stream));
    SW_HIP(hipMemsetAsync(special.p, 0xFF, 4, stream));
    if (ix.n_nodes)
        hipLaunchKernelGGL(k_table_build, dim3(blocks_for(ix.n_nodes)), dim3(TPB), 0, stream, ix.nodes.p, ix.n_nodes, slots.p, cap - 1,
                           special.p);
    hipLaunchKernelGGL(k_table_lookup, dim3(blocks_for(n)), dim3(TPB), 0, stream, hash, n, slots.p, cap - 1, special.p, rank);
    SW_HIP(hipGetLastError());
    SW_HIP(hipStreamSynchronize(stream));
}

__global__ void k_append_chunk(const uint32_t *__restrict__ key32, const OccPay *__restrict__ pay, const uint32_t *__restrict__ rec,
                               uint64_t n, uint32_t occ_base, uint32_t rec_base, uint32_t *__restrict__ key32_out,
                               OccPay *__restrict__ pay_out, uint32_t *__restrict__ rec_out)
{
    const uint64_t i = (uint64_t)blockIdx.x * blockDim.x + threadIdx.x;
    if (i >= n) return;
    OccPay p = pay[i];
    p.rec += rec_base;
    p.idx += occ_base;
    key32_out[occ_base + i] = key32[i];
    pay_out[occ_base + i] = p;
    rec_out[occ_base + i] = rec[i] + rec_base;
}

}

void concat_occ(std::vector<OrderedOcc> &chunks, const std::vector<uint64_t> &rec_base, hipStream_t stream, OrderedOcc &out)
{
    uint64_t n = 0;
    for (const OrderedOcc &c : chunks) n += c.n;
    if (n > occ_cap()) raise_occ_cap(n, "minimizer occurrences");
    out.n = n;
    out.key32.alloc(n);
    out.pay.alloc(n);
    out.rec.alloc(n);
    uint64_t at = 0;
    for (size_t c = 0; c < chunks.size(); ++c) {
        OrderedOcc &ch = chunks[c];
        if (ch.n) {
            hipLaunchKernelGGL(k_append_chunk, dim3(blocks_for(ch.n)), dim3(TPB), 0, stream, ch.key32.p, ch.pay.p, ch.rec.p, ch.n,
                               (uint32_t)at, (uint32_t)rec_base[c], out.key32.p, out.pay.p, out.rec.p);
            SW_HIP(hipGetLastError());
        }
        at += ch.n;
        ch = OrderedOcc();
    }
    if (chunks.size() > 1) {
        SW_HIP(hipStreamSynchronize(stream));
        dev_pool_trim();
    }
}

namespace {

struct MinTree {
    const uint64_t *lvl[7];
    uint64_t size[7];
    int levels;
};
constexpr uint64_t LW_NONE = ~0ull;

__global__ void k_lw_level(const uint64_t *__restrict__ in, uint64_t n_in, uint64_t *__restrict__ out, uint64_t n_out)
{
    const uint64_t node = ((uint64_t)blockIdx.x * blockDim.x + threadIdx.x) >> 6;
    const uint32_t lane = threadIdx.x & 63u;
    if (node >= n_out) return;
    const uint64_t i = node * 64 + lane;
    uint64_t v = i < n_in ? in[i] : ~0ull;
    for (int d = 32; d; d >>= 1) {
        const uint64_t o = __shfl_xor(v, d, 64);
        v = o < v ? o : v;
    }
    if (lane == 0) out[node] = v;
}

__device__ uint64_t lw_nearest_left(const MinTree &T, uint64_t i, uint64_t lo, uint64_t h)
{
    uint64_t pos = i, q = 0;
    int t = 0;
    for (;;) {
        const uint64_t gstart = pos & ~63ull, lo_t = lo >> (6 * t), stop = gstart > lo_t ? gstart : lo_t;
        bool found = false;
        for (q = pos; q > stop;) {
            --q;
            if (T.lvl[t][q] < h) {
                found = true;
                break;
            }
        }
        if (found) break;
        if (gstart <= lo_t || t + 1 >= T.levels) return LW_NONE;
        pos >>= 6;
        ++t;
    }
    while (t > 0) {
        const uint64_t cfirst = q << 6, clo = lo >> (6 * (t - 1));
        uint64_t c = cfirst + 64 < T.size[t - 1] ? cfirst + 64 : T.size[t - 1];
        const uint64_t stop = cfirst > clo ? cfirst : clo;
        bool found = false;
        while (c > stop) {
            --c;
            if (T.lvl[t - 1][c] < h) {
                found = true;
                break;
            }
        }
        if (!found) return LW_NONE;
        q = c;
        --t;
    }
    return q;
}

__device__ uint64_t lw_nearest_right(const MinTree &T, uint64_t i, uint64_t hi, uint64_t h)
{
    uint64_t pos = i, q = 0;
    int t = 0;
    for (;;) {
        const uint64_t gend = (pos | 63ull) + 1, hi_t = (hi + ((1ull << (6 * t)) - 1)) >> (6 * t);
        uint64_t stop = gend < hi_t ? gend : hi_t;
        if (T.size[t] < stop) stop = T.size[t];
        bool found = false;
        for (q = pos + 1; q < stop; ++q)
            if (T.lvl[t][q] <= h) {
                found = true;
                break;
            }
        if (found) break;
        if (gend >= hi_t || gend >= T.size[t] || t + 1 >= T.levels) return LW_NONE;
        pos >>= 6;
        ++t;
    }
    while (t > 0) {
        const uint64_t cfirst = q << 6, chi = (hi + ((1ull << (6 * (t - 1))) - 1)) >> (6 * (t - 1));
        uint64_t stop = cfirst + 64 < T.size[t - 1] ? cfirst + 64 : T.size[t - 1];
        if (chi < stop) stop = chi;
        uint64_t c = cfirst;
        bool found = false;
        for (; c < stop; ++c)
            if (T.lvl[t - 1][c] <= h) {
                found = true;
                break;
            }
        if (!found) return LW_NONE;
        q = c;
        --t;
    }
    return q;
}

__global__ void k_lw_index(const uint64_t *__restrict__ kmer, uint64_t c, const uint32_t *__restrict__ rec_seg_off,
                           const uint32_t *__restrict__ seg_pos, const uint32_t *__restrict__ seg_idx, uint32_t *__restrict__ g)
{
    const uint64_t i = (uint64_t)blockIdx.x * blockDim.x + threadIdx.x;
    if (i >= c) return;
    const uint32_t pos = (uint32_t)kmer[i], rec = (uint32_t)(kmer[i] >> 32);
    uint32_t a = rec_seg_off[rec], b = rec_seg_off[rec + 1];
    while (b - a > 1) {
        const uint32_t mid = (a + b) >> 1;
        if (seg_pos[mid] <= pos) a = mid; else b = mid;
    }
    g[i] = seg_idx[a] + (pos - seg_pos[a]);
}

__global__ void k_lw_select(const MinTree T, const uint64_t *__restrict__ kmer, const uint32_t *__restrict__ g, uint64_t c,
                            const uint32_t *__restrict__ rec_nvalid, uint32_t w, uint32_t *__restrict__ keep)
{
    const uint64_t i = (uint64_t)blockIdx.x * blockDim.x + threadIdx.x;
    if (i >= c) return;
    const uint64_t h = T.lvl[0][i];
    const uint32_t rec = (uint32_t)(kmer[i] >> 32);
    const int64_t n = rec_nvalid[rec], gi = g[i];
    uint32_t k = 0;
    if (n >= (int64_t)w && h != ~0ull) {
        uint64_t lo = 0, hi = i;
        while (lo < hi) {
            const uint64_t mid = (lo + hi) >> 1;
            if ((uint32_t)(kmer[mid] >> 32) < rec) lo = mid + 1; else hi = mid;
        }
        uint64_t a = i + 1;
        hi = c;
        while (a < hi) {
            const uint64_t mid = (a + hi) >> 1;
            if ((uint32_t)(kmer[mid] >> 32) <= rec) a = mid + 1; else hi = mid;
        }
        const uint64_t jl = lw_nearest_left(T, i, lo, h), jr = lw_nearest_right(T, i, hi, h);
        const int64_t Lg = jl == LW_NONE ? -1 : (int64_t)g[jl], Rg = jr == LW_NONE ? n : (int64_t)g[jr];
        int64_t x_lo = Lg + 1, x_hi = Rg - (int64_t)w;
        if (gi - (int64_t)w + 1 > x_lo) x_lo = gi - (int64_t)w + 1;
        if (x_lo < 0) x_lo = 0;
        if (gi < x_hi) x_hi = gi;
        if (n - (int64_t)w < x_hi) x_hi = n - (int64_t)w;
        k = x_lo <= x_hi ? 1u : 0u;
    }
    keep[i] = k;
}

template <bool INDEX>
__global__ void k_lw_emit(const uint64_t *__restrict__ canon, const uint64_t *__restrict__ kmer, const uint32_t *__restrict__ keep,
                          const uint64_t *__restrict__ dst, uint64_t c, uint64_t mult, uint64_t *__restrict__ hash,
                          uint64_t *__restrict__ kmer_out, uint32_t *__restrict__ key32, OccPay *__restrict__ pay,
                          uint32_t *__restrict__ rec, unsigned long long *__restrict__ total)
{
    const uint64_t i = (uint64_t)blockIdx.x * blockDim.x + threadIdx.x;
    if (i >= c) return;
    if (i == c - 1) *total = dst[i] + keep[i];
    if (!keep[i]) return;
    const uint64_t d = dst[i], km = kmer[i];
    uint64_t h = canon[i] * mult;
    h ^= h >> 27;
    if (INDEX) {
        key32[d] = (uint32_t)(h >> 32);
        OccPay p;
        p.low = (uint32_t)h;
        p.pos = (uint32_t)km;
        p.rec = (uint32_t)(km >> 32);
        p.idx = (uint32_t)d;
        pay[d] = p;
        rec[d] = p.rec;
        if (hash) hash[d] = h;
    } else {
        hash[d] = h;
        kmer_out[d] = km;
    }
}

}

static bool stage_fits_sort(uint64_t n, uint32_t n_tiles)
{
    if (const char *e = SW_TEST_GETENV("SEQWIN_AMD_ORDER")) {
        if (!strcmp(e, "copy")) return false;
        if (!strcmp(e, "stage")) return n > 0 && radix_pairs_available() && !SW_TEST_GETENV("SEQWIN_AMD_SORT_KEYBITS");
    }
    return n > 0 && sort_pairs_is_own(n, 32) && !SW_TEST_GETENV("SEQWIN_AMD_SORT_KEYBITS") && n / 16 >= n_tiles;
}

__global__ void k_fill_u64(uint64_t *p, uint32_t n, uint64_t v)
{
    if (threadIdx.x < n) p[threadIdx.x] = v;
}

void order_tuples(SketchOut &sk, const Plan &plan, hipStream_t stream, OrderedOcc &out, bool index_form, bool take_stage)
{
    const bool large = plan.w_full > plan.w;
    out.n = sk.n_occ;
    out.staged = false;
    if (!large && out.n > occ_cap()) raise_occ_cap(out.n, "minimizer occurrences");
    const bool table_ranks = index_form && ranks_by_table();
    if (take_stage && index_form && !large && !table_ranks && plan.n_tiles && stage_fits_sort(sk.n_occ, plan.n_tiles)) {
        out.rec.alloc(out.n);
        out.dst_off.alloc((size_t)plan.n_tiles + STAGE_PAD);
        exclusive_sum(rocprim::make_transform_iterator(sk.tile_count.p, U32ToU64()), out.dst_off.p, plan.n_tiles, (uint64_t)0, stream);
        hipLaunchKernelGGL(k_fill_u64, dim3(1), dim3(64), 0, stream, out.dst_off.p + plan.n_tiles, STAGE_PAD, out.n);
        SW_HIP(hipGetLastError());
        out.stage = std::move(sk);
        out.stage_tiles = plan.n_tiles;
        out.stage_mult = plan.mult;
        out.staged = true;
        return;
    }
    auto alloc_out = [&](uint64_t n) {
        if (index_form) {
            out.key32.alloc(n);
            out.pay.alloc(n);
            out.rec.alloc(n);
            if (table_ranks) out.hash.alloc(n);
        } else {
            out.hash.alloc(n);
            out.kmer.alloc(n);
        }
    };
    if (!large) alloc_out(out.n);
    if (plan.n_tiles == 0 || sk.n_occ == 0) {
        out.n = 0;
        if (large) alloc_out(0);
        return;
    }
    DevArray<uint64_t> dst_off(plan.n_tiles);
    exclusive_sum(rocprim::make_transform_iterator(sk.tile_count.p, U32ToU64()), dst_off.p, plan.n_tiles,
                  (uint64_t)0, stream);
    const uint64_t threads = (uint64_t)plan.n_tiles * 64;
    if (large) {
        const uint64_t c = sk.n_occ;
        if (c > occ_cap()) raise_occ_cap(c, "window candidates");
        DevArray<uint64_t> canon(c), kmer(c), keep_off(c);
        DevArray<uint32_t> g(c), keep(c);
        DevArray<unsigned long long> total(1);
        hipLaunchKernelGGL((k_order<false, true>), dim3(blocks_for(threads)), dim3(TPB), 0, stream, sk.stage_hash.p, sk.stage_kmer.p,
                           sk.tile_count.p, sk.tile_offset.p, dst_off.p, plan.n_tiles, plan.mult, canon.p, kmer.p,
                           (uint32_t *)nullptr, (OccPay *)nullptr, (uint32_t *)nullptr);
        hipLaunchKernelGGL(k_lw_index, dim3(blocks_for(c)), dim3(TPB), 0, stream, kmer.p, c, plan.rec_seg_off.p, plan.seg_pos.p,
                           plan.seg_idx.p, g.p);
        SW_HIP(hipGetLastError());
        MinTree T;
        std::vector<DevArray<uint64_t>> levels;
        levels.reserve(7);
        T.lvl[0] = canon.p;
        T.size[0] = c;
        T.levels = 1;
        while (T.size[T.levels - 1] > 64) {
            const int t = T.levels;
            if (t >= 7) raise(SW_ERR_RUNTIME, "internal error: more than 2^36 window candidates");
            const uint64_t n_in = T.size[t - 1], n_out = (n_in + 63) / 64;
            levels.emplace_back(n_out);
            hipLaunchKernelGGL(k_lw_level, dim3(blocks_for(n_out * 64)), dim3(TPB), 0, stream, T.lvl[t - 1], n_in, levels.back().p,
                               n_out);
            SW_HIP(hipGetLastError());
            T.lvl[t] = levels.back().p;
            T.size[t] = n_out;
            T.levels = t + 1;
        }
        for (int t = T.levels; t < 7; ++t) {
            T.lvl[t] = nullptr;
            T.size[t] = 0;
        }
        hipLaunchKernelGGL(k_lw_select, dim3(blocks_for(c)), dim3(TPB), 0, stream, T, kmer.p, g.p, c, plan.rec_nvalid.p, plan.w_full,
                           keep.p);
        SW_HIP(hipGetLastError());
        exclusive_sum(rocprim::make_transform_iterator(keep.p, U32ToU64()), keep_off.p, c, (uint64_t)0, stream);
        alloc_out(c);
        if (index_form)
            hipLaunchKernelGGL(k_lw_emit<true>, dim3(blocks_for(c)), dim3(TPB), 0, stream, canon.p, kmer.p, keep.p, keep_off.p, c,
                               plan.mult, table_ranks ? out.hash.p : (uint64_t *)nullptr, (uint64_t *)nullptr, out.key32.p,
                               out.pay.p, out.rec.p, total.p);
        else
            hipLaunchKernelGGL(k_lw_emit<false>, dim3(blocks_for(c)), dim3(TPB), 0, stream, canon.p, kmer.p, keep.p, keep_off.p, c,
                               plan.mult, out.hash.p, out.kmer.p, (uint32_t *)nullptr, (OccPay *)nullptr, (uint32_t *)nullptr,
                               total.p);
        SW_HIP(hipGetLastError());
        unsigned long long n_keep = 0;
        SW_HIP(hipMemcpyAsync(&n_keep, total.p, 8, hipMemcpyDeviceToHost, stream));
        SW_HIP(hipStreamSynchronize(stream));
        out.n = n_keep;
        if (out.n > occ_cap()) raise_occ_cap(out.n, "minimizer occurrences");
        return;
    }
    if (index_form)
        hipLaunchKernelGGL(k_order<true>, dim3(blocks_for(threads)), dim3(TPB), 0, stream, sk.stage_hash.p, sk.stage_kmer.p,
                           sk.tile_count.p, sk.tile_offset.p, dst_off.p, plan.n_tiles, plan.mult,
                           table_ranks ? out.hash.p : (uint64_t *)nullptr, (uint64_t *)nullptr, out.key32.p, out.pay.p, out.rec.p);
    else
        hipLaunchKernelGGL(k_order<false>, dim3(blocks_for(threads)), dim3(TPB), 0, stream, sk.stage_hash.p, sk.stage_kmer.p,
                           sk.tile_count.p, sk.tile_offset.p, dst_off.p, plan.n_tiles, plan.mult, out.hash.p, out.kmer.p,
                           (uint32_t *)nullptr, (OccPay *)nullptr, (uint32_t *)nullptr);
    SW_HIP(hipGetLastError());
}

namespace {
struct PenaltyJob {
    DevArray<uint64_t> X, Y;
    DevArray<uint32_t> err;
    DevArray<unsigned char> tmp_x, tmp_y;
    hipStream_t stream = nullptr;
    bool active = false;
    ~PenaltyJob() { if (active) (void)hipStreamSynchronize(stream); }
};

void penalty_launch(const sw_kmer *d_kmers, uint64_t n_kmers, sw_node *d_nodes, uint64_t n_nodes,
                    const uint32_t *d_rec_asm, uint64_t n_records, const uint8_t *d_is_target, uint64_t n_targets,
                    uint64_t n_non_targets, hipStream_t stream, PenaltyJob &job)
{
    job.stream = stream;
    job.active = n_nodes != 0;
    if (!job.active) return;
    job.X.alloc(n_kmers);
    job.Y.alloc(n_kmers);
    job.err.alloc(1);
    DevArray<uint64_t> &X = job.X, &Y = job.Y;
    DevArray<uint32_t> &err = job.err;
    SW_HIP(hipMemsetAsync(err.p, 0, 4, stream));
    const double inv_tar = 1.0 / (double)n_targets;
    const double inv_neg = 1.0 / (double)n_non_targets;
    if (n_kmers) {
        hipLaunchKernelGGL(k_pen_flags, dim3(blocks_for(n_kmers)), dim3(TPB), 0, stream, d_kmers, n_kmers, d_rec_asm, n_records,
                           d_is_target, X.p, Y.p);
        SW_HIP(hipGetLastError());
        inclusive_sum_keep(X.p, X.p, n_kmers, (uint64_t)0, stream, job.tmp_x);
        inclusive_sum_keep(Y.p, Y.p, n_kmers, (uint64_t)0, stream, job.tmp_y);
    }
    hipLaunchKernelGGL(k_pen_nodes, dim3(blocks_for(n_nodes)), dim3(TPB), 0, stream, d_kmers, n_kmers, d_nodes, n_nodes, d_rec_asm,
                       n_records, d_is_target, X.p, Y.p, inv_tar, inv_neg, err.p);
    SW_HIP(hipGetLastError());
}

uint64_t penalty_finish(PenaltyJob &job)
{
    if (!job.active) return 0;
    uint32_t e = 0;
    SW_HIP(hipMemcpyAsync(&e, job.err.p, 4, hipMemcpyDeviceToHost, job.stream));
    SW_HIP(hipStreamSynchronize(job.stream));
    job.active = false;
    return e;
}

hipStream_t side_stream()
{
    static thread_local std::map<int, hipStream_t> streams;
    int dev = 0;
    SW_HIP(hipGetDevice(&dev));
    hipStream_t &s = streams[dev];
    if (!s) SW_HIP(hipStreamCreateWithFlags(&s, hipStreamNonBlocking));
    return s;
}
}

namespace {
struct PackedChangeAny {
// ... 205 lines not shown
        auto flags = rocprim::make_transform_iterator(rocprim::make_counting_iterator<uint64_t>(0), RepeatFlag{k, a});
        size_t tmp_bytes = 0;
        SW_HIP(rocprim::reduce_by_key(nullptr, tmp_bytes, k, flags, c, rkeys.p, rdups.p, rcount.p, rocprim::plus<uint32_t>(),
                                      rocprim::equal_to<uint64_t>(), stream));
        DevArray<unsigned char> tmp(tmp_bytes);
        SW_HIP(rocprim::reduce_by_key(tmp.p, tmp_bytes, k, flags, c, rkeys.p, rdups.p, rcount.p, rocprim::plus<uint32_t>(),
                                      rocprim::equal_to<uint64_t>(), stream));
        uint32_t n_runs = 0;
        SW_HIP(hipMemcpyAsync(&n_runs, rcount.p, 4, hipMemcpyDeviceToHost, stream));
        SW_HIP(hipStreamSynchronize(stream));
        if (n_runs) {
            hipLaunchKernelGGL(k_subtract_repeats, dim3(blocks_for(n_runs)), dim3(TPB), 0, stream, rkeys.p, rdups.p, n_runs, ukeys.p,
                               (uint64_t)ix.n_edges, ix.edges.p);
            SW_HIP(hipGetLastError());
        }
    }
    SW_HIP(hipStreamSynchronize(stream));
}

void edges_from_adjacency(uint64_t *keys, uint64_t *keys_alt, uint32_t *vals, uint32_t *vals_alt, uint64_t m,
                          uint64_t sentinel, unsigned nb, const uint64_t *rank_hash, hipStream_t stream, sw_index &ix)
{
    ix.n_edges = 0;
    if (m == 0) return;
    sort_pairs(keys, keys_alt, vals, vals_alt, m, 0, 2 * nb, stream);
    DevArray<uint64_t> ukeys(m);
    DevArray<uint32_t> usum(m);
    DevArray<uint32_t> ucount(1);
    {
        auto flags = rocprim::make_transform_iterator(rocprim::make_counting_iterator<uint64_t>(0), AsmChangeAny{keys, vals});
        size_t tmp_bytes = 0;
        SW_HIP(rocprim::reduce_by_key(nullptr, tmp_bytes, keys, flags, m, ukeys.p, usum.p, ucount.p, rocprim::plus<uint32_t>(),
                                      rocprim::equal_to<uint64_t>(), stream));
        DevArray<unsigned char> tmp(tmp_bytes);
        SW_HIP(rocprim::reduce_by_key(tmp.p, tmp_bytes, keys, flags, m, ukeys.p, usum.p, ucount.p, rocprim::plus<uint32_t>(),
                                      rocprim::equal_to<uint64_t>(), stream));
        hipLaunchKernelGGL(k_drop_sentinel_run, dim3(1), dim3(1), 0, stream, ukeys.p, sentinel, ucount.p);
        SW_HIP(hipGetLastError());
        uint32_t n_edges = 0;
        SW_HIP(hipMemcpyAsync(&n_edges, ucount.p, 4, hipMemcpyDeviceToHost, stream));
        SW_HIP(hipStreamSynchronize(stream));
        ix.n_edges = n_edges;
    }
    if (ix.n_edges == 0) return;
    ix.edges.alloc(ix.n_edges);
    hipLaunchKernelGGL(k_edges_runs<false>, dim3(blocks_for(ix.n_edges)), dim3(TPB), 0, stream, ukeys.p, usum.p, 0u, ~0ull,
                       (uint64_t)ix.n_edges, nb, ix.nodes.p, rank_hash, ix.edges.p);
    SW_HIP(hipGetLastError());
    SW_HIP(hipStreamSynchronize(stream));
}
}

__global__ void k_pack_export_nodes(const sw_node *__restrict__ nodes, uint64_t n, uint64_t n_kmers, uint64_t per, uint32_t *__restrict__ out,
                                    uint64_t *__restrict__ bases, uint32_t *__restrict__ flag)
{
    const uint64_t i = (uint64_t)blockIdx.x * blockDim.x + threadIdx.x;
    if (i >= n) return;
    const sw_node nd = nodes[i];
    const uint64_t cnt = nd.stop - nd.start, next = i + 1 < n ? nodes[i + 1].start : n_kmers;
    uint64_t pen;
    memcpy(&pen, &nd.penalty, 8);
    if (nd.stop < nd.start || cnt > 0xFFFFFFFFull || next != nd.stop || (i == 0 && nd.start != 0) || nd.n_tar || nd.n_neg || pen) atomicOr(flag, 1u);
    out[3 * i] = (uint32_t)nd.hash;
    out[3 * i + 1] = (uint32_t)(nd.hash >> 32);
    out[3 * i + 2] = (uint32_t)cnt;
    if (i % per == 0) bases[i / per] = nd.start;
}
__global__ void k_pack_export_edges(const sw_edge *__restrict__ edges, uint64_t n, uint32_t *__restrict__ out, uint32_t *__restrict__ flag)
{
    const uint64_t i = (uint64_t)blockIdx.x * blockDim.x + threadIdx.x;
    if (i >= n) return;
    const sw_edge e = edges[i];
    if (e.weight > 0xFFFFFFFFull) atomicOr(flag, 1u);
    out[5 * i] = (uint32_t)e.first;
    out[5 * i + 1] = (uint32_t)(e.first >> 32);
    out[5 * i + 2] = (uint32_t)e.second;
    out[5 * i + 3] = (uint32_t)(e.second >> 32);
    out[5 * i + 4] = (uint32_t)e.weight;
}
void pack_export(const sw_node *nodes, uint64_t n_nodes, uint64_t n_kmers, const sw_edge *edges, uint64_t n_edges, uint64_t per, uint32_t *pn,
                 uint64_t *bases, uint32_t *pe, uint32_t *flag, hipStream_t stream)
{
    hipLaunchKernelGGL(k_pack_export_nodes, dim3(blocks_for(n_nodes)), dim3(TPB), 0, stream, nodes, n_nodes, n_kmers, per, pn, bases, flag);
    SW_HIP(hipGetLastError());
    hipLaunchKernelGGL(k_pack_export_edges, dim3(blocks_for(n_edges)), dim3(TPB), 0, stream, edges, n_edges, pe, flag);
    SW_HIP(hipGetLastError());
    SW_HIP(hipStreamSynchronize(stream));
}

void device_get_penalty(const sw_kmer *d_kmers, uint64_t n_kmers, sw_node *d_nodes, uint64_t n_nodes,
                        const uint32_t *d_rec_asm, uint64_t n_records, const uint8_t *d_is_target,
                        uint64_t n_targets, uint64_t n_non_targets, hipStream_t stream, uint64_t *err_flags_host)
{
    PenaltyJob job;
    penalty_launch(d_kmers, n_kmers, d_nodes, n_nodes, d_rec_asm, n_records, d_is_target, n_targets, n_non_targets,
                   stream, job);
    *err_flags_host = penalty_finish(job);
}

void slice_get_penalty(sw_index &ix, uint64_t kmer_base, const uint32_t *d_rec_asm, uint64_t n_records, const uint8_t *d_is_target,
                       uint64_t n_targets, uint64_t n_non_targets, hipStream_t stream, uint64_t *err_flags_host)
{
    *err_flags_host = 0;
    if (!ix.n_nodes) return;
    hipLaunchKernelGGL(k_rebase_nodes, dim3(blocks_for(ix.n_nodes)), dim3(TPB), 0, stream, ix.nodes.p, ix.n_nodes, (uint64_t)0 - kmer_base);
    SW_HIP(hipGetLastError());
    struct Restore {
        sw_index &ix;
        uint64_t base;
        hipStream_t st;
        ~Restore()
        {
            hipLaunchKernelGGL(k_rebase_nodes, dim3(blocks_for(ix.n_nodes)), dim3(TPB), 0, st, ix.nodes.p, ix.n_nodes, base);
            (void)hipGetLastError();
            (void)hipStreamSynchronize(st);
        }
    } restore{ix, kmer_base, stream};
    device_get_penalty(ix.kmers.p, ix.n_kmers, ix.nodes.p, ix.n_nodes, d_rec_asm, n_records, d_is_target, n_targets, n_non_targets,
                       stream, err_flags_host);
}

void build_index(const uint32_t *d_rec_asm, uint64_t n_records, uint64_t n_assemblies, OrderedOcc &occ,
                 const uint8_t *d_is_target, uint64_t n_targets, uint64_t n_non_targets, hipStream_t stream, sw_index &ix)
{
    const uint64_t n = occ.n;
    if (n > occ_cap()) raise_occ_cap(n, "minimizer occurrences");
    Event ev[6];
    SW_HIP(hipEventRecord(ev[0], stream));

    ix.n_kmers = n;
    ix.kmers.alloc(n);
    DevArray<uint32_t> rank(n);
    const bool want_counts = d_is_target != nullptr;
    const bool check_order = want_counts && SW_TEST_GETENV("SEQWIN_AMD_CHECK_ORDER") != nullptr;
    const bool by_table = occ.hash.p != nullptr;
    const bool pair_edges = !SW_TEST_GETENV("SEQWIN_AMD_NO_PACKED_EDGES") && !by_table;
    bool rep_marked = false;
    DevArray<uint32_t> rec_flag;
    DevArray<unsigned long long> tbits, nbits;
    NodeParts parts;
    UnsortHold unsort_hold;
    if (n) {
        const bool bits = want_counts && !check_order;
        if (bits || pair_edges) {
            rec_flag.alloc(n_records);
            hipLaunchKernelGGL(k_rec_flag, dim3(blocks_for(n_records)), dim3(TPB), 0, stream, d_rec_asm, bits ? d_is_target : nullptr,
                               n_records, rec_flag.p);
            SW_HIP(hipGetLastError());
        }
        PaySort ps;
        ps.key_a = std::move(occ.key32);
        ps.pay_a = std::move(occ.pay);
        if (occ.staged) ps.staged = &occ;
        group_occurrences(ps, n, 0, rec_flag.p, stream, ix, by_table ? nullptr : rank.p, bits ? &tbits : nullptr,
                          bits ? &nbits : nullptr, pair_edges ? &rep_marked : nullptr, pair_edges ? &unsort_hold : nullptr, &parts);
        if (!bits || by_table) {
            finish_nodes(ix, parts, 0, n, nullptr, nullptr, 0.0, 0.0, stream);
            if (by_table) ranks_from_table(ix, occ.hash.p, n, stream, rank.p);
        }
    } else {
        ix.n_nodes = 0;
        ix.nodes.alloc(0);
    }
    SW_HIP(hipEventRecord(ev[1], stream));

    PenaltyJob pen;
    hipStream_t side = side_stream();
    bool forked = false;
    if (want_counts && ix.n_nodes) {
        alloc_fork(side);
        forked = true;
        SW_HIP(hipStreamWaitEvent(side, ev[1], 0));
        SW_HIP(hipEventRecord(ev[4], side));
        if (check_order) {
            penalty_launch(ix.kmers.p, n, ix.nodes.p, ix.n_nodes, d_rec_asm, n_records, d_is_target, n_targets, n_non_targets,
                           side, pen);
        } else {
            finish_nodes(ix, parts, 0, n, tbits.p, nbits.p, 1.0 / (double)n_targets, 1.0 / (double)n_non_targets, side);
        }
        SW_HIP(hipEventRecord(ev[5], side));
    }
    SW_HIP(hipEventRecord(ev[2], stream));

    ix.n_edges = 0;
    if (n >= 2) {
        const uint64_t m = n - 1;
        unsigned nb = 1;
        while (((1ull << nb) - 1ull) < ix.n_nodes) ++nb;
        unsigned ab = 1;
        while ((1ull << ab) < n_assemblies) ++ab;
        const unsigned adj_blocks = (unsigned)((n + 1023) / 1024);
        const uint64_t sentinel = (nb == 32) ? ~0ull : ((1ull << (2 * nb)) - 1ull);
        DevArray<uint64_t> k0(m), k1(m);
        if (rep_marked) {
            DevArray<uint64_t> ck(m);
            DevArray<uint32_t> ca(m);
            DevArray<unsigned long long> n_cand(1);
            SW_HIP(hipMemsetAsync(n_cand.p, 0, 8, stream));
            DevArray<unsigned long long> ehist;
            unsigned hbits = 0, hpasses = 0;
            uint32_t iters = 1;
            if (sort_keys64_is_own(m) && !SW_AB_GETENV("SEQWIN_AMD_NO_ADJ_HIST")) {
                radix_layout(2 * nb, &hbits, &hpasses);
                ehist.alloc((size_t)hpasses << hbits);
                SW_HIP(hipMemsetAsync(ehist.p, 0, ehist.bytes(), stream));
                iters = 32;
            }
            if (unsort_hold.sorted) {
                const uint32_t n_buckets = (uint32_t)((n + UNSORT_RANGE - 1) / UNSORT_RANGE);
                const uint32_t per_wg = 4;
                DevArray<uint32_t> edge_rank(2 * (size_t)n_buckets);
                hipLaunchKernelGGL(k_unsort_adj<RecArray>, dim3((n_buckets + per_wg - 1) / per_wg), dim3(1024),
                                   ehist.p ? ((size_t)hpasses << hbits) * 4 : 0, stream, unsort_hold.sorted,
                                   n, RecArray{occ.rec.p}, d_rec_asm, 0u, nb, sentinel, k0.p, ck.p, ca.p, n_cand.p,
                                   ehist.p, hbits, hpasses, 2 * nb, edge_rank.p, per_wg);
                hipLaunchKernelGGL(k_adj_bounds<RecArray>, dim3((n_buckets + 255) / 256), dim3(256), 0, stream, edge_rank.p, n_buckets,
                                   RecArray{occ.rec.p}, d_rec_asm, 0u, nb, sentinel, k0.p, ck.p, ca.p, n_cand.p, ehist.p, hbits, hpasses,
                                   2 * nb);
                unsort_hold.a.release();
                unsort_hold.b.release();
            } else {
                hipLaunchKernelGGL(k_adj_pairs<RecArray>, dim3((adj_blocks + iters - 1) / iters), dim3(256), 0, stream, RecArray{occ.rec.p},
                                   rank.p, d_rec_asm, 0u, n, nb, sentinel, k0.p, ck.p, ca.p, n_cand.p, ehist.p, hbits, hpasses, 2 * nb, iters);
            }
            SW_HIP(hipGetLastError());
            edges_from_pairs(k0.p, k1.p, m, sentinel, nb, ab, ck.p, ca.p, n_cand.p, 0, parts.hash.p, stream, ix, (hipEvent_t) nullptr,
                             ehist.p);
        } else {
            DevArray<uint32_t> v0(m), v1(m);
            hipLaunchKernelGGL(k_adj_keys, dim3(adj_blocks), dim3(256), 0, stream, occ.rec.p, rank.p, d_rec_asm, n, nb,
                               sentinel, k0.p, v0.p);
            SW_HIP(hipGetLastError());
            edges_from_adjacency(k0.p, k1.p, v0.p, v1.p, m, sentinel, nb, parts.hash.p, stream, ix);
        }
    }
    if (ix.n_edges == 0) ix.edges.alloc(0);
    if (forked) {
        const uint64_t err = pen.active ? penalty_finish(pen) : 0;
        SW_HIP(hipStreamWaitEvent(stream, ev[5], 0));
        alloc_join(side);
        if (err) raise(SW_ERR_RUNTIME, "internal error: inconsistent occurrence order in device index (%llu)",
                       (unsigned long long)err);
    }
    SW_HIP(hipEventRecord(ev[3], stream));
    SW_HIP(hipEventSynchronize(ev[3]));
    float ms = 0.f;
    SW_HIP(hipEventElapsedTime(&ms, ev[0], ev[1]));
    ix.timings.nodes_ms = ms;
    ix.timings.counts_ms = 0;
    if (forked) {
        SW_HIP(hipEventElapsedTime(&ms, ev[4], ev[5]));
        ix.timings.counts_ms = ms;
    }
    SW_HIP(hipEventElapsedTime(&ms, ev[2], ev[3]));
    ix.timings.edges_ms = ms;
}

void index_occ_rows(const sw_index &ix, uint64_t rec_offset, uint64_t *d_rows, hipStream_t stream)
{
    if (ix.n_kmers == 0) return;
    DevArray<uint32_t> start(ix.n_nodes);
    hipLaunchKernelGGL(k_node_starts, dim3(blocks_for(ix.n_nodes)), dim3(TPB), 0, stream, ix.nodes.p, ix.n_nodes, start.p);
    hipLaunchKernelGGL(k_occ_rows, dim3(blocks_for(ix.n_kmers)), dim3(TPB), 0, stream, ix.kmers.p, ix.nodes.p, start.p,
                       ix.n_nodes, ix.n_kmers, rec_offset, d_rows);
    SW_HIP(hipGetLastError());
    SW_HIP(hipStreamSynchronize(stream));
}

void index_splits(const sw_index &ix, const uint64_t *node_bounds, const uint64_t *edge_bounds, uint32_t n_bounds,
                  uint64_t *occ_split, uint64_t *edge_split, hipStream_t stream)
{
    if (n_bounds == 0) return;
    DevArray<uint64_t> nb(n_bounds), eb(n_bounds), os(n_bounds), es(n_bounds);
    SW_HIP(hipMemcpyAsync(nb.p, node_bounds, n_bounds * 8, hipMemcpyHostToDevice, stream));
    SW_HIP(hipMemcpyAsync(eb.p, edge_bounds, n_bounds * 8, hipMemcpyHostToDevice, stream));
    hipLaunchKernelGGL(k_lower_bounds, dim3(blocks_for(n_bounds)), dim3(TPB), 0, stream, ix.nodes.p, ix.n_nodes, ix.n_kmers,
                       ix.edges.p, ix.n_edges, nb.p, eb.p, n_bounds, os.p, es.p);
    SW_HIP(hipGetLastError());
    SW_HIP(hipMemcpyAsync(occ_split, os.p, n_bounds * 8, hipMemcpyDeviceToHost, stream));
    SW_HIP(hipMemcpyAsync(edge_split, es.p, n_bounds * 8, hipMemcpyDeviceToHost, stream));
    SW_HIP(hipStreamSynchronize(stream));
}

void merge_build(const uint64_t *d_occ_rows, uint64_t n, const uint64_t *d_edge_rows, uint64_t m, uint64_t kmer_base,
                 const uint32_t *d_rec_asm, uint64_t n_records, const uint8_t *d_is_target, uint64_t n_targets,
                 uint64_t n_non_targets, hipStream_t stream, sw_index &ix, uint32_t *d_rank_out)
{
    if (n > occ_cap() || m > occ_cap()) raise_occ_cap(std::max<uint64_t>(n, m), "rows");
    ix.n_kmers = n;
    ix.kmers.alloc(n);
    ix.n_nodes = 0;
    ix.n_edges = 0;
    const bool slice = d_rank_out && m == 0 && d_rec_asm && n_records && !SW_TEST_GETENV("SEQWIN_AMD_CHECK_ORDER");
    if (n) {
        PaySort ps;
        const char *order = SW_TEST_GETENV("SEQWIN_AMD_ORDER");
        if (sort_pairs_is_own(n, 32) && !SW_TEST_GETENV("SEQWIN_AMD_SORT_KEYBITS") && !(order && !strcmp(order, "copy"))) {
            ps.rows_src = d_occ_rows;
        } else {
            ps.key_a.alloc(n);
            ps.pay_a.alloc(n);
            hipLaunchKernelGGL(k_rows_to_pay, dim3(blocks_for(n)), dim3(TPB), 0, stream, d_occ_rows, n, ps.key_a.p, ps.pay_a.p);
            SW_HIP(hipGetLastError());
        }
        DevArray<uint32_t> rec_flag;
        DevArray<unsigned long long> tbits, nbits;
// ... 772 lines not shown
```

seqwin_amd/csrc/radix.hip:

```cpp
#include <algorithm>
#include <cstdlib>
#include <cstring>
#include <vector>
#include <map>
#include <mutex>

#include "device.hpp"

namespace sw {
namespace {

constexpr int RS_ITEMS = 16;
#ifdef SW_RS_STAMPS
__device__ unsigned long long *g_rs_stamps = nullptr;
#define RS_STAMP(i)                                                                                        \
    do {                                                                                                   \
        if (g_rs_stamps && (tile & 63u) == 0 && threadIdx.x == 0) g_rs_stamps[(size_t)(tile >> 6) * 16 + (i)] = clock64(); \
    } while (0)
#else
#define RS_STAMP(i) do { } while (0)
#endif
#ifndef RS_LOOK
#define RS_LOOK 4
#endif
// ... 402 lines not shown
        unsigned long long pre[RS_LOOK];
        unsigned long long *st = state + (size_t)tile * RADIX;
        if (tid < RADIX) {
            const uint32_t d = tid;
#pragma unroll
            for (uint32_t w = 0; w < WAVES; ++w) {
                const uint32_t c = whist[w][d];
                whist[w][d] = (uint16_t)total;
                total += c;
            }
            if (cursor) {
                const uint64_t group = SEG ? seg_bucket(seg) : group_shift < 64u ? (((uint64_t)tile * TILE) >> group_shift) : 0ull;
                pre[0] = total ? atomicAdd(&cursor[(group * RADIX + d) * cursor_stride], (unsigned long long)total) : 0ull;
            } else {
                __hip_atomic_store(&st[d], rse_pack(epoch, tile == 0 ? 2u : 1u, total), __ATOMIC_RELAXED, __HIP_MEMORY_SCOPE_AGENT);
#pragma unroll
                for (int j = 0; j < RS_LOOK; ++j)
                    pre[j] = (int64_t)tile - 1 - j >= 0
                                 ? __hip_atomic_load(&state[(size_t)(tile - 1 - j) * RADIX + d], __ATOMIC_RELAXED, __HIP_MEMORY_SCOPE_AGENT)
                                 : rse_pack(epoch, 2u, 0);
            }
            incl = total;
            for (uint32_t dd = 1; dd < 64; dd <<= 1) {
                const uint32_t up = __shfl_up(incl, dd, 64);
                if (lane >= dd) incl += up;
            }
            if (lane == 63) wsum[wave] = incl;
        }
        RS_STAMP(3);
        __syncthreads();
        uint32_t before = 0;
        if (tid < RADIX) {
            before = incl - total;
            for (uint32_t w = 0; w < wave; ++w) before += wsum[w];
            lstart[tid] = before;
        }
        if (tid == 0) s_tile = fut;
        __syncthreads();
        const uint32_t ntile = s_tile;
        if constexpr (SEG) nseg = ntile < n_tiles ? digit_base[ntile] : 0ull;
        auto place_and_fetch = [&]() {
#pragma unroll
            for (int i = 0; i < RS_ITEMS; ++i) {
                const uint32_t li = wave * (64 * RS_ITEMS) + i * 64 + lane;
                if (li < cnt_tile) {
                    const uint32_t d = (uint32_t)(key[i] >> shift) & dmask;
                    sk[lstart[d] + whist[wave][d] + rank[i]] = key[i];
                }
            }
#pragma unroll
            for (int i = 0; i < RS_ITEMS; ++i) {
                const uint32_t li = wave * (64 * RS_ITEMS) + i * 64 + lane;
                if constexpr (SEG) {
                    key[i] = li < seg_count(nseg) ? in[seg_first(nseg) + li] : ~0ull;
                } else {
                    const uint64_t g = (uint64_t)ntile * TILE + li;
                    key[i] = (ntile < n_tiles && g < n && !(dbg & 4u)) ? in[g] : (dbg & 4u ? g * 0x9E3779B97F4A7C15ull : ~0ull);
                }
            }
            if (tid == 0) fut = atomicAdd(ticket, 1u);
        };
        const bool digit_wave = tid < RADIX;
        if (!digit_wave || cursor) place_and_fetch();
        RS_STAMP(4);
        if (tid < RADIX && cursor) {
            goff[tid] = pre[0] - before;
        } else if (tid < RADIX) {
            const uint32_t d = tid;
            unsigned long long excl = 0;
            if (tile) {
                int64_t t = (int64_t)tile - 1;
                uint32_t spins = 0;
                bool done = false;
                bool first_step = true;
#ifdef SW_RS_STAMPS
                uint32_t n_steps = 0, n_polls = 0;
#endif
                while (!done && t >= 0 && !(dbg & 1u)) {
#ifdef SW_RS_STAMPS
                    ++n_steps;
#endif
                    unsigned long long v[RS_LOOK];
#pragma unroll
                    for (int j = 0; j < RS_LOOK; ++j)
                        v[j] = first_step ? pre[j]
                               : t - j >= 0 ? __hip_atomic_load(&state[(size_t)(t - j) * RADIX + d], __ATOMIC_RELAXED, __HIP_MEMORY_SCOPE_AGENT)
                                            : rse_pack(epoch, 2u, 0);
                    first_step = false;
                    int j = 0;
#pragma unroll
                    for (; j < RS_LOOK; ++j) {
                        const uint32_t f = rse_flag(v[j], epoch);
                        if (f == 0) break;
                        excl += v[j] & RSE_VAL;
                        if (f == 2) {
                            done = true;
                            break;
                        }
                    }
                    if (done) break;
                    t -= j;
                    if (j < RS_LOOK) {
#ifdef SW_RS_STAMPS
                        ++n_polls;
#endif
                        if (++spins > RS_SPIN_LIMIT) {
                            atomicOr(fail, 1u);
                            break;
                        }
                        __builtin_amdgcn_s_sleep(1);
                    }
                }
#ifdef SW_RS_STAMPS
                if (g_rs_stamps && (tile & 63u) == 0 && tid == 0) {
                    g_rs_stamps[(size_t)(tile >> 6) * 16 + 8] = n_steps;
                    g_rs_stamps[(size_t)(tile >> 6) * 16 + 9] = n_polls;
                    g_rs_stamps[(size_t)(tile >> 6) * 16 + 10] = (unsigned long long)((int64_t)tile - 1 - t);
                }
#endif
                __hip_atomic_store(&st[d], rse_pack(epoch, 2u, excl + total), __ATOMIC_RELAXED, __HIP_MEMORY_SCOPE_AGENT);
            }
            goff[d] = digit_base[d] + excl - before;
        }
        RS_STAMP(5);
        if (digit_wave && !cursor) place_and_fetch();
        __syncthreads();
        RS_STAMP(6);
#pragma unroll
        for (int j = 0; j < RS_ITEMS; ++j) {
            const uint32_t t = j * THREADS + tid;
            if (t < cnt_tile) {
                const uint64_t k = sk[t];
                if (!(dbg & 2u)) out[goff[(uint32_t)(k >> shift) & dmask] + t] = k;
            }
        }
        RS_STAMP(7);
        tile = ntile;
        seg = nseg;
    }
}


__device__ __forceinline__ unsigned long long stage_search(const StageSource &S, uint32_t lo, uint64_t g)
{
    uint32_t hi = S.n_tiles;
    while (hi - lo > 1u) {
        const uint32_t mid = lo + ((hi - lo) >> 1);
        if (S.dst_off[mid] <= g) lo = mid; else hi = mid;
    }
    return S.tile_offset[lo] - S.dst_off[lo];
}

constexpr int RP_THREADS = 1024, RP_ITEMS = 7, RP_BITS = 8;
template <int SRC>
__global__ __launch_bounds__(RP_THREADS) void k_rs_pair_pass(const uint32_t *__restrict__ kin, const uint4 *__restrict__ pin,
                                                             uint32_t *__restrict__ kout, uint4 *__restrict__ pout, uint64_t n,
                                                             uint32_t n_tiles, unsigned shift,
                                                             const unsigned long long *__restrict__ digit_base,
                                                             unsigned long long *__restrict__ state, uint32_t epoch,
                                                             uint32_t *__restrict__ ticket, uint32_t *__restrict__ fail,
                                                             const StageSource S, uint32_t *__restrict__ lowout, uint32_t fault)
{
    constexpr bool STAGE = SRC == 1, ROWS = SRC == 2;
    constexpr uint32_t THREADS = RP_THREADS, ITEMS = RP_ITEMS, RADIX = 1u << RP_BITS, WAVES = THREADS / 64, TILE = THREADS * ITEMS;
    __shared__ uint4 sp[TILE];
    __shared__ uint32_t skey[TILE];
    __shared__ uint16_t whist[WAVES][RADIX];
    __shared__ uint32_t lstart[RADIX];
    __shared__ unsigned long long goff[RADIX];
    __shared__ uint32_t wsum[RADIX / 64];
    __shared__ uint32_t s_tile;
    const uint32_t tid0 = threadIdx.x;
    if (tid0 == 0) s_tile = atomicAdd(ticket, 1u);
    __syncthreads();
    uint32_t tile = s_tile;
    uint32_t key[ITEMS];
    uint4 pay[ITEMS];
    struct Window {
        unsigned long long word;
        bool ok;
    };
    auto fetch_window = [&](uint32_t tl, uint32_t lane, uint32_t wave) __attribute__((always_inline)) {
        Window w{0ull, false};
        if constexpr (STAGE) {
            const uint32_t wv = (uint32_t)__builtin_amdgcn_readfirstlane((int)wave);
            const uint64_t chunk = (uint64_t)tl * WAVES + wv;
            w.ok = tl < n_tiles && chunk * (64 * ITEMS) < n;
            if (w.ok && lane < STAGE_ROW) w.word = S.chunk_dir[chunk * STAGE_ROW + lane];
        }
        return w;
    };
    auto fetch = [&](uint32_t tl, uint32_t lane, uint32_t wave, const Window &w) __attribute__((always_inline)) {
        if constexpr (ROWS) {
#pragma unroll
            for (int i = 0; i < (int)ITEMS; ++i) {
                const uint64_t g = (uint64_t)tl * TILE + wave * (64 * ITEMS) + i * 64 + lane;
                pay[i] = (tl < n_tiles && g < n) ? reinterpret_cast<const uint4 *>(S.rows)[g] : uint4{0, 0, 0, 0};
            }
        } else if constexpr (!STAGE) {
#pragma unroll
            for (int i = 0; i < (int)ITEMS; ++i) {
                const uint64_t g = (uint64_t)tl * TILE + wave * (64 * ITEMS) + i * 64 + lane;
                const bool in_range = tl < n_tiles && g < n;
                key[i] = in_range ? kin[g] : ~0u;
                pay[i] = in_range ? pin[g] : uint4{0, 0, 0, 0};
            }
        } else {
#pragma unroll
            for (int i = 0; i < (int)ITEMS; ++i) pay[i] = uint4{0, 0, 0, 0};
            const uint32_t wv = (uint32_t)__builtin_amdgcn_readfirstlane((int)wave);
            const uint64_t c0 = ((uint64_t)tl * WAVES + wv) * (64 * ITEMS);
            if (w.ok) {
                const unsigned long long d_end = __shfl(w.word, (int)(STAGE_WIN + 7), 64);
                uint32_t before = 0;
#pragma unroll
                for (int i = 0; i < (int)ITEMS; ++i) {
                    const unsigned long long m = __shfl(w.word, (int)STAGE_WIN + i, 64);
                    const uint64_t g = c0 + i * 64 + lane;
                    const uint32_t r = before + (uint32_t)__popcll(m & ((2ull << lane) - 1ull));
                    before += (uint32_t)__popcll(m);
                    unsigned long long delta = __shfl(w.word, (int)min(r, STAGE_WIN - 1u), 64);
                    if (g < n) {
                        if (g >= d_end) delta = stage_search(S, (uint32_t)__shfl(w.word, (int)(STAGE_WIN + 8), 64) + STAGE_WIN, g);
                        const uint2 h = *reinterpret_cast<const uint2 *>(S.stage_hash + (g + delta));
                        const uint2 km = *reinterpret_cast<const uint2 *>(S.stage_kmer + (g + delta));
                        pay[i] = uint4{h.x, h.y, km.x, km.y};
                    }
                }
            }
        }
    };
    fetch(tile, tid0 & 63u, tid0 >> 6, fetch_window(tile, tid0 & 63u, tid0 >> 6));
    uint32_t fut = 0;
    if (tid0 == 0) fut = atomicAdd(ticket, 1u);
    while (tile < n_tiles) {
        uint32_t tid = tid0;
        asm volatile("" : "+v"(tid));
        const uint32_t lane = tid & 63u, wave = tid >> 6;
        for (uint32_t i = tid; i < WAVES * RADIX / 2; i += THREADS) (reinterpret_cast<uint32_t *>(&whist[0][0]))[i] = 0;
        const uint64_t t0 = (uint64_t)tile * TILE;
        const uint32_t cnt_tile = (uint32_t)min((uint64_t)TILE, n - t0);
        if constexpr (ROWS) {
#pragma unroll
            for (int i = 0; i < (int)ITEMS; ++i) {
                const uint32_t li = wave * (64 * ITEMS) + i * 64 + lane;
                key[i] = li < cnt_tile ? pay[i].y : ~0u;
                pay[i] = uint4{pay[i].x, pay[i].z, pay[i].w, (uint32_t)(t0 + li)};
            }
        }
        if constexpr (STAGE) {
#pragma unroll
            for (int i = 0; i < (int)ITEMS; ++i) {
                const uint32_t li = wave * (64 * ITEMS) + i * 64 + lane;
                unsigned long long h = ((unsigned long long)pay[i].y << 32) | pay[i].x;
                h *= S.mult;
                h ^= h >> 27;
                const uint32_t rec = pay[i].w;
                key[i] = li < cnt_tile ? (uint32_t)(h >> 32) : ~0u;
                pay[i] = uint4{(uint32_t)h, pay[i].z, rec, (uint32_t)(t0 + li)};
                if (li < cnt_tile) S.rec_out[t0 + li] = rec;
            }
        }
        __syncthreads();
        uint32_t pos[ITEMS];
#pragma unroll
        for (int i = 0; i < (int)ITEMS; ++i) {
            const uint32_t li = wave * (64 * ITEMS) + i * 64 + lane;
            const uint32_t d = (key[i] >> shift) & (RADIX - 1u);
            pos[i] = 0;
            if (li < cnt_tile) pos[i] = atomicAdd(reinterpret_cast<uint32_t *>(&whist[wave][d & ~1u]), 1u << ((d & 1u) << 4));
        }
#pragma unroll
        for (int i = 0; i < (int)ITEMS; ++i) {
            const uint32_t d = (key[i] >> shift) & (RADIX - 1u);
            pos[i] = (pos[i] >> ((d & 1u) << 4)) & 0xFFFFu;
        }
        if (fault && wave == 0) {
#pragma unroll
            for (int i = 0; i < (int)ITEMS; ++i) {
                const uint32_t li = i * 64 + lane;
                const uint32_t d = li < cnt_tile ? ((key[i] >> shift) & (RADIX - 1u)) : ~lane;
                const uint32_t od = __shfl_xor(d, 1, 64), opos = __shfl_xor(pos[i], 1, 64);
                if (od == d) pos[i] = opos;
            }
        }
        __syncthreads();
        uint32_t total = 0, incl = 0;
        unsigned long long *st = state + (size_t)tile * RADIX;
        if (tid < RADIX) {
            const uint32_t d = tid;
#pragma unroll
            for (uint32_t w = 0; w < WAVES; ++w) {
                const uint32_t c = whist[w][d];
                whist[w][d] = (uint16_t)total;
                total += c;
            }
            __hip_atomic_store(&st[d], rse_pack(epoch, tile == 0 ? 2u : 1u, total), __ATOMIC_RELAXED, __HIP_MEMORY_SCOPE_AGENT);
            incl = total;
            for (uint32_t dd = 1; dd < 64; dd <<= 1) {
                const uint32_t up = __shfl_up(incl, dd, 64);
                if (lane >= dd) incl += up;
            }
            if (lane == 63) wsum[wave] = incl;
        }
        __syncthreads();
        uint32_t before = 0;
        if (tid < RADIX) {
            before = incl - total;
            for (uint32_t w = 0; w < wave; ++w) before += wsum[w];
            lstart[tid] = before;
        }
        if (tid == 0) s_tile = fut;
        __syncthreads();
        const uint32_t ntile = s_tile;
        auto place_keys = [&](const Window &win) {
#pragma unroll
            for (int i = 0; i < (int)ITEMS; ++i) {
                const uint32_t li = wave * (64 * ITEMS) + i * 64 + lane;
                const uint32_t d = (key[i] >> shift) & (RADIX - 1u);
                const uint32_t at = pos[i] + lstart[d] + whist[wave][d];
                if (li < cnt_tile) {
                    skey[at] = key[i];
                    sp[at] = pay[i];
                }
            }
            fetch(ntile, lane, wave, win);
            if (tid == 0) fut = atomicAdd(ticket, 1u);
        };
        const bool look_wave = tid < RADIX;
        const Window win = fetch_window(ntile, lane, wave);
        if (!look_wave) place_keys(win);
        if (look_wave) {
            const uint32_t d = tid;
            unsigned long long excl = 0;
            if (tile) {
                int64_t t = (int64_t)tile - 1;
                uint32_t spins = 0;
                bool done = false;
                while (!done && t >= 0) {
                    unsigned long long v[RS_LOOK];
#pragma unroll
                    for (int j = 0; j < RS_LOOK; ++j)
                        v[j] = t - j >= 0 ? __hip_atomic_load(&state[(size_t)(t - j) * RADIX + d], __ATOMIC_RELAXED, __HIP_MEMORY_SCOPE_AGENT)
                                          : rse_pack(epoch, 2u, 0);
                    int j = 0;
#pragma unroll
                    for (; j < RS_LOOK; ++j) {
                        const uint32_t f = rse_flag(v[j], epoch);
                        if (f == 0) break;
                        excl += v[j] & RSE_VAL;
                        if (f == 2) {
                            done = true;
                            break;
                        }
                    }
                    if (done) break;
                    t -= j;
                    if (j < RS_LOOK) {
                        if (++spins > RS_SPIN_LIMIT) {
                            atomicOr(fail, 1u);
                            break;
                        }
                        __builtin_amdgcn_s_sleep(1);
                    }
                }
                __hip_atomic_store(&st[d], rse_pack(epoch, 2u, excl + total), __ATOMIC_RELAXED, __HIP_MEMORY_SCOPE_AGENT);
            }
            goff[d] = digit_base[d] + excl - before;
            place_keys(win);
        }
        __syncthreads();
#pragma unroll
        for (int j = 0; j < (int)ITEMS; ++j) {
            const uint32_t t = j * THREADS + tid;
            if (t < cnt_tile) {
                const uint32_t k = skey[t];
                const uint64_t dst = goff[(k >> shift) & (RADIX - 1u)] + t;
                const uint4 pv = sp[t];
                kout[dst] = k;
                pout[dst] = pv;
                if (lowout) lowout[dst] = pv.x;
            }
        }
        tile = ntile;
    }
}

__global__ __launch_bounds__(256) void k_rs_hist32(const uint32_t *__restrict__ keys, uint64_t n, unsigned n_passes,
                                                   unsigned long long *__restrict__ hist)
{
    constexpr uint32_t RADIX = 1u << RP_BITS;
    __shared__ uint32_t h[4 * RADIX];
    for (uint32_t i = threadIdx.x; i < n_passes * RADIX; i += 256) h[i] = 0;
    __syncthreads();
    const uint64_t chunk = 65536;
    const uint64_t i0 = (uint64_t)blockIdx.x * chunk, i1 = min(n, i0 + chunk);
    auto count = [&](uint32_t k) {
        for (unsigned p = 0; p < n_passes; ++p) atomicAdd(&h[p * RADIX + ((k >> (RP_BITS * p)) & (RADIX - 1u))], 1u);
    };
    for (uint64_t i = i0 + 4 * threadIdx.x; i < i1; i += 1024) {
        if (i + 3 < i1) {
            const uint4 kk = *reinterpret_cast<const uint4 *>(keys + i);
            count(kk.x); count(kk.y); count(kk.z); count(kk.w);
        } else {
            for (uint64_t j = i; j < i1; ++j) count(keys[j]);
        }
    }
    __syncthreads();
    for (uint32_t i = threadIdx.x; i < n_passes * RADIX; i += 256)
        if (h[i]) atomicAdd(&hist[i], (unsigned long long)h[i]);
}

__global__ __launch_bounds__(256) void k_rs_hist32_rows(const uint4 *__restrict__ rows, uint64_t n, unsigned n_passes,
                                                        unsigned long long *__restrict__ hist)
{
    constexpr uint32_t RADIX = 1u << RP_BITS;
    __shared__ uint32_t h[4 * RADIX];
    for (uint32_t i = threadIdx.x; i < n_passes * RADIX; i += 256) h[i] = 0;
    __syncthreads();
    const uint64_t chunk = 16384;
    const uint64_t i0 = (uint64_t)blockIdx.x * chunk, i1 = min(n, i0 + chunk);
    for (uint64_t i = i0 + threadIdx.x; i < i1; i += 1024) {
        uint32_t k[4];
#pragma unroll
        for (int j = 0; j < 4; ++j) k[j] = i + 256u * j < i1 ? rows[i + 256u * j].y : 0u;
#pragma unroll
        for (int j = 0; j < 4; ++j)
            if (i + 256u * j < i1)
                for (unsigned p = 0; p < n_passes; ++p) atomicAdd(&h[p * RADIX + ((k[j] >> (RP_BITS * p)) & (RADIX - 1u))], 1u);
    }
    __syncthreads();
    for (uint32_t i = threadIdx.x; i < n_passes * RADIX; i += 256)
        if (h[i]) atomicAdd(&hist[i], (unsigned long long)h[i]);
}

__global__ void k_rs_chunk_tiles(const uint32_t *__restrict__ tile_count, const uint64_t *__restrict__ dst_off, uint32_t n_tiles,
                                 uint32_t *__restrict__ chunk_tile)
{
    constexpr uint64_t CHUNK = 64 * RP_ITEMS;
    const uint32_t T = blockIdx.x * blockDim.x + threadIdx.x;
    if (T >= n_tiles) return;
    const uint32_t c = tile_count[T];
    const uint64_t d = dst_off[T];
    for (uint64_t m = (d + CHUNK - 1) / CHUNK; m * CHUNK < d + c; ++m) chunk_tile[m] = T;
}

__global__ __launch_bounds__(256) void k_rs_stage_prepare(const StageSource S, const uint32_t *__restrict__ chunk_tile, uint64_t n,
                                                          unsigned n_passes, unsigned long long *__restrict__ chunk_dir,
                                                          unsigned long long *__restrict__ hist)
{
    constexpr uint32_t RADIX = 1u << RP_BITS, CHUNK = 64 * RP_ITEMS;
    __shared__ uint32_t h[4 * RADIX];
    __shared__ unsigned long long s_row[4][STAGE_ROW];
    for (uint32_t i = threadIdx.x; i < n_passes * RADIX; i += 256) h[i] = 0;
    __syncthreads();
    const uint32_t lane = threadIdx.x & 63u, wv = (uint32_t)__builtin_amdgcn_readfirstlane((int)(threadIdx.x >> 6));
    const uint64_t n_chunks = (n + CHUNK - 1) / CHUNK;
    for (uint64_t chunk = (uint64_t)blockIdx.x * 4u + wv; chunk < n_chunks; chunk += (uint64_t)gridDim.x * 4u) {
        const uint64_t c0 = chunk * CHUNK;
        const uint32_t T0 = (uint32_t)__builtin_amdgcn_readfirstlane((int)chunk_tile[chunk]);
        const uint32_t Tj = T0 + lane;
        const bool in_win = lane < STAGE_WIN && Tj < S.n_tiles;
        const unsigned long long dj = lane <= STAGE_WIN ? S.dst_off[min(Tj, S.n_tiles)] : ~0ull;
        const unsigned long long oj = in_win ? S.tile_offset[Tj] - dj : 0ull;
        const uint32_t cj = in_win ? S.tile_count[Tj] : 0u;
        const bool marks = in_win && lane >= 1u && cj != 0u && dj < c0 + CHUNK;
        const unsigned long long bal = __ballot(marks);
        const uint32_t rank = 1u + (uint32_t)__popcll(bal & ((1ull << lane) - 1ull));
        if (lane < STAGE_ROW) s_row[wv][lane] = 0ull;
        __builtin_amdgcn_fence(__ATOMIC_RELEASE, "wavefront");
        __builtin_amdgcn_wave_barrier();
        if (lane == 0u) {
            s_row[wv][0] = oj;
            s_row[wv][STAGE_WIN + 8] = T0;
        }
        if (lane == STAGE_WIN) s_row[wv][STAGE_WIN + 7] = dj;
        if (marks) {
            const uint32_t rel = (uint32_t)(dj - c0);
            atomicOr(&s_row[wv][STAGE_WIN + (rel >> 6)], 1ull << (rel & 63u));
            s_row[wv][rank] = oj;
        }
        __builtin_amdgcn_fence(__ATOMIC_RELEASE, "wavefront");
        __builtin_amdgcn_wave_barrier();
        __builtin_amdgcn_fence(__ATOMIC_ACQUIRE, "wavefront");
        const unsigned long long word = lane < STAGE_ROW ? s_row[wv][lane] : 0ull;
        if (lane < STAGE_ROW) chunk_dir[chunk * STAGE_ROW + lane] = word;
        __builtin_amdgcn_wave_barrier();
        const unsigned long long d_end = __shfl(word, (int)(STAGE_WIN + 7), 64);
        uint32_t before = 0;
        unsigned long long hv[RP_ITEMS];
#pragma unroll
        for (int i = 0; i < RP_ITEMS; ++i) {
            const unsigned long long m = __shfl(word, (int)STAGE_WIN + i, 64);
            const uint64_t g = c0 + i * 64 + lane;
            const uint32_t r = before + (uint32_t)__popcll(m & ((2ull << lane) - 1ull));
            before += (uint32_t)__popcll(m);
            unsigned long long delta = __shfl(word, (int)min(r, STAGE_WIN - 1u), 64);
            hv[i] = 0;
            if (g < n) {
                if (g >= d_end) delta = stage_search(S, T0 + STAGE_WIN, g);
                hv[i] = S.stage_hash[g + delta];
            }
        }
#pragma unroll
        for (int i = 0; i < RP_ITEMS; ++i) {
            if (c0 + i * 64 + lane < n) {
                unsigned long long v = hv[i] * S.mult;
                v ^= v >> 27;
                const uint32_t k = (uint32_t)(v >> 32);
                for (unsigned p = 0; p < n_passes; ++p) atomicAdd(&h[p * RADIX + ((k >> (RP_BITS * p)) & (RADIX - 1u))], 1u);
            }
        }
    }
    __syncthreads();
    for (uint32_t i = threadIdx.x; i < n_passes * RADIX; i += 256)
        if (h[i]) atomicAdd(&hist[i], (unsigned long long)h[i]);
}

struct StateBuf {
    std::mutex mu;
    unsigned long long *p = nullptr;
    size_t words = 0;
    uint32_t epoch = 0;
};
std::mutex &state_registry_mu()
{
    static std::mutex &mu = *new std::mutex;
    return mu;
}
std::map<std::pair<int, hipStream_t>, StateBuf *> &state_registry()
{
    static auto &bufs = *new std::map<std::pair<int, hipStream_t>, StateBuf *>;
    return bufs;
}
thread_local int g_state_uses = 0;
struct StateUse {
    StateBuf &b;
    std::unique_lock<std::mutex> lock;
    StateUse(StateBuf &buf, std::unique_lock<std::mutex> &&l) : b(buf), lock(std::move(l)) { ++g_state_uses; }
    StateUse(StateUse &&o) : b(o.b), lock(std::move(o.lock)) { ++g_state_uses; }
    StateUse(const StateUse &) = delete;
    StateUse &operator=(const StateUse &) = delete;
    ~StateUse() { --g_state_uses; }
};
StateUse state_buf(hipStream_t stream, size_t words)
{
    int dev = 0;
    SW_HIP(hipGetDevice(&dev));
    StateBuf *b = nullptr;
    {
        std::lock_guard<std::mutex> lock(state_registry_mu());
        StateBuf *&slot = state_registry()[std::make_pair(dev, stream)];
        if (!slot) slot = new StateBuf;
        b = slot;
    }
    StateUse u(*b, std::unique_lock<std::mutex>(b->mu));
    if (b->words < words) {
        if (b->p) (void)hipFree(b->p);
        b->p = nullptr;
        b->words = 0;
        const size_t want = words + words / 4;
        SW_HIP(hipMalloc(&b->p, want * 8));
        b->words = want;
        b->epoch = 0;
        SW_HIP(hipMemsetAsync(b->p, 0, want * 8, stream));
    }
    return u;
}
uint32_t next_epoch(StateBuf &b, hipStream_t stream)
{
    if (++b.epoch >= 0xFFFFu) {
        SW_HIP(hipMemsetAsync(b.p, 0, b.words * 8, stream));
        b.epoch = 1;
    }
    return b.epoch;
}

template <int THREADS, int BITS>
void sort_passes(uint64_t *&keys, uint64_t *&alt, uint64_t n, unsigned begin_bit, unsigned end_bit, hipStream_t stream, uint32_t *d_fail,
                 bool perm_hi32, unsigned long long *d_hist_given)
{
    constexpr uint32_t RADIX = 1u << BITS, TILE = THREADS * RS_ITEMS;
    const unsigned n_passes = (end_bit - begin_bit + BITS - 1) / BITS;
    const uint64_t n_tiles = (n + TILE - 1) / TILE;
    const char *kind = SW_AB_GETENV("SEQWIN_AMD_RADIX_KERNEL");
    const bool persistent = !(kind && !strcmp(kind, "classic"));
    uint32_t dbg = 0;
#ifdef SW_RADIX_ABLATION
    if (const char *e = getenv("SEQWIN_AMD_RADIX_DEBUG")) dbg = (uint32_t)atoi(e) & 15u;
#endif
    if (fault_rank()) dbg |= 16u;
    int grid_p = 0;
    if (persistent) {
        static std::mutex &mu = *new std::mutex;
        static std::map<int, int> &grids = *new std::map<int, int>;
        int dev = 0;
        SW_HIP(hipGetDevice(&dev));
        std::lock_guard<std::mutex> lock(mu);
        int &g = grids[dev];
        if (!g) {
            int per_cu = 0;
            hipDeviceProp_t prop;
            SW_HIP(hipGetDeviceProperties(&prop, dev));
            SW_HIP(hipOccupancyMaxActiveBlocksPerMultiprocessor(&per_cu, k_rs_pass_p<THREADS, BITS, 0>, THREADS, 0));
            g = std::max(1, per_cu) * std::max(1, prop.multiProcessorCount);
        }
        grid_p = g;
    }
    const bool atomic_rank = persistent && rank_mode() == 1;
    DevArray<unsigned long long> hist_own(d_hist_given ? 0 : (size_t)n_passes * RADIX), state(persistent ? 0 : (size_t)n_tiles * RADIX);
    std::unique_ptr<StateUse> su(persistent ? new StateUse(state_buf(stream, (size_t)n_tiles * RADIX)) : nullptr);
    StateBuf *sb = su ? &su->b : nullptr;
    struct { unsigned long long *p; } hist{d_hist_given ? d_hist_given : hist_own.p};
    const bool unstable = perm_hi32 && persistent && !SW_AB_GETENV("SEQWIN_AMD_RADIX_STABLE_UNSORT");
    DevArray<unsigned long long> cursor(unstable ? (size_t)RADIX * RS_CURSOR_STRIDE : 0);
    DevArray<uint32_t> tickets(n_passes);
    SW_HIP(hipMemsetAsync(tickets.p, 0, tickets.bytes(), stream));
    if (d_hist_given) {
    } else if (perm_hi32 && begin_bit >= 32) {
        hipLaunchKernelGGL(k_rs_perm_hist<BITS>, dim3(n_passes), dim3(RADIX), 0, stream, n, begin_bit, end_bit, hist.p);
    } else {
        SW_HIP(hipMemsetAsync(hist.p, 0, hist_own.bytes(), stream));
        hipLaunchKernelGGL(k_rs_hist<BITS>, dim3((unsigned)((n + 32767) / 32768)), dim3(256), 0, stream, keys, n, begin_bit, end_bit,
                           n_passes, hist.p);
    }
    SW_HIP(hipGetLastError());
#ifdef SW_RS_STAMPS
    DevArray<unsigned long long> stamps;
    const size_t n_st = (size_t)(n_tiles / 64 + 1) * 16;
    if (getenv("SEQWIN_AMD_STAMPS") && persistent) stamps.alloc(n_st);
#endif
    for (unsigned p = 0; p < n_passes; ++p) {
        const unsigned sh = begin_bit + BITS * p, bits = std::min<unsigned>(BITS, end_bit - sh);
#ifdef SW_RS_STAMPS
        if (stamps.p) {
            SW_HIP(hipMemsetAsync(stamps.p, 0, stamps.bytes(), stream));
            unsigned long long *ptr = stamps.p;
            SW_HIP(hipMemcpyToSymbolAsync(HIP_SYMBOL(g_rs_stamps), &ptr, sizeof ptr, 0, hipMemcpyHostToDevice, stream));
        }
#endif
        unsigned long long *cur = unstable && p == 0 ? cursor.p : nullptr;
        hipLaunchKernelGGL(k_rs_scan<BITS>, dim3(1), dim3(RADIX), 0, stream, hist.p + (size_t)p * RADIX, cur);
        if (!cur && !persistent) SW_HIP(hipMemsetAsync(state.p, 0, state.bytes(), stream));
        if (persistent) {
            const uint32_t epoch = cur ? 0u : next_epoch(*sb, stream);
            auto launch = [&](auto kern) {
                hipLaunchKernelGGL(kern, dim3((unsigned)std::min<uint64_t>(n_tiles, (uint64_t)grid_p)), dim3(THREADS), 0, stream, keys, alt, n,
                                   (uint32_t)n_tiles, sh, bits, hist.p + (size_t)p * RADIX, sb->p, tickets.p + p, d_fail, dbg, cur,
                                   RS_CURSOR_STRIDE, 64u, epoch);
            };
            if (cur ? !ballot_forced() : atomic_rank) launch(k_rs_pass_p<THREADS, BITS, 1>);
            else launch(k_rs_pass_p<THREADS, BITS, 0>);
        } else {
#ifdef SW_AB
            hipLaunchKernelGGL((k_rs_pass<THREADS, BITS>), dim3((unsigned)n_tiles), dim3(THREADS), 0, stream, keys, alt, n, sh, bits,
                               hist.p + (size_t)p * RADIX, state.p, d_fail);
#endif
        }
        SW_HIP(hipGetLastError());
#ifdef SW_RS_STAMPS
        if (stamps.p) {
            std::vector<unsigned long long> hs(n_st);
            SW_HIP(hipStreamSynchronize(stream));
            SW_HIP(hipMemcpy(hs.data(), stamps.p, stamps.bytes(), hipMemcpyDeviceToHost));
            double acc[8] = {0}, look[3] = {0};
            size_t cnt = 0;
            for (size_t t = 0; t + 16 <= n_st; t += 16) {
                if (!hs[t] || !hs[t + 7]) continue;
                for (int i = 1; i <= 7; ++i) acc[i] += (double)(hs[t + i] - hs[t + i - 1]);
                for (int i = 0; i < 3; ++i) look[i] += (double)hs[t + 8 + i];
                ++cnt;
            }
            static const char *nm[] = {"", "rank", "barrier", "totals+scan", "barrier+scatter", "lookback(d0)", "barrier", "write-out"};
            fprintf(stderr, "[rs stamps] %d x %d bits, pass %u, %zu tiles sampled; mean clocks:", THREADS, BITS, p, cnt);
            double sum = 0;
            for (int i = 1; i <= 7; ++i) { fprintf(stderr, " %s=%.0f", nm[i], cnt ? acc[i] / cnt : 0.0); sum += cnt ? acc[i] / cnt : 0.0; }
            fprintf(stderr, " | tile %.0f | look-back of digit 0: %.1f steps, %.1f polls of an unpublished record, %.1f records behind\n", sum,
                    cnt ? look[0] / cnt : 0.0, cnt ? look[1] / cnt : 0.0, cnt ? look[2] / cnt : 0.0);
        }
#endif
        std::swap(keys, alt);
    }
}

}

namespace {
__global__ void k_rs_perm_cursors(unsigned long long *__restrict__ cursor, uint32_t n_groups, uint32_t radix, uint32_t stride,
                                  unsigned group_bits, unsigned digit_shift)
{
    const uint32_t i = blockIdx.x * blockDim.x + threadIdx.x;
    if (i >= n_groups * radix) return;
    const uint64_t g = i / radix, d = i % radix;
    cursor[(size_t)i * stride] = (group_bits < 64 ? g << group_bits : 0ull) + (d << digit_shift);
}
}

bool radix_unsort_perm_begin(UnsortPerm &u, uint64_t n, unsigned low_bits, unsigned nbit, hipStream_t stream)
{
    constexpr int THREADS = 512, BITS = 8;
    constexpr uint32_t RADIX = 1u << BITS, TILE = THREADS * RS_ITEMS;
    static_assert(UNSORT_CURSOR_STRIDE == RS_CURSOR_STRIDE, "one cursor layout for the first pass and for a producer that scatters itself");
    if (n == 0 || nbit <= low_bits + 8 || nbit > low_bits + 16 || SW_AB_GETENV("SEQWIN_AMD_RADIX_STABLE_UNSORT")) return false;
    if ((1ull << (low_bits + 8)) % TILE) return false;
    const char *kind = SW_AB_GETENV("SEQWIN_AMD_RADIX_KERNEL");
    if (kind && !strcmp(kind, "classic")) return false;
    u.low_bits = low_bits;
    u.hi_bits = nbit - low_bits - 8;
    u.n_groups = (uint32_t)((n + (1ull << (low_bits + 8)) - 1) >> (low_bits + 8));
    const uint64_t n_tiles = (n + TILE - 1) / TILE;
    u.n_tiles = (uint32_t)n_tiles;
    int dev = 0, per_cu = 0;
    SW_HIP(hipGetDevice(&dev));
    hipDeviceProp_t prop;
    SW_HIP(hipGetDeviceProperties(&prop, dev));
    SW_HIP(hipOccupancyMaxActiveBlocksPerMultiprocessor(&per_cu, k_rs_pass_p<THREADS, BITS, 0>, THREADS, 0));
    u.grid = (unsigned)std::min<uint64_t>(n_tiles, (uint64_t)std::max(1, per_cu) * std::max(1, prop.multiProcessorCount));
    if (!u.cur_a.p) {
        u.cur_a.alloc((size_t)RADIX * RS_CURSOR_STRIDE);
        u.cur_b.alloc((size_t)u.n_groups * RADIX);
        u.tickets.alloc(2);
    }
    SW_HIP(hipMemsetAsync(u.tickets.p, 0, 8, stream));
    hipLaunchKernelGGL(k_rs_perm_cursors, dim3(1), dim3(RADIX), 0, stream, u.cur_a.p, 1u, RADIX, RS_CURSOR_STRIDE, 64u, low_bits + 8);
    hipLaunchKernelGGL(k_rs_perm_cursors, dim3((u.n_groups * RADIX + 255) / 256), dim3(256), 0, stream, u.cur_b.p, u.n_groups, RADIX, 1u,
                       low_bits + 8, low_bits);
    SW_HIP(hipGetLastError());
    return true;
}

void radix_unsort_perm_first(UnsortPerm &u, const uint64_t *keys, uint64_t *alt, uint64_t n, hipStream_t stream, uint32_t *d_fail)
{
    constexpr int THREADS = 512, BITS = 8;
    auto pass = ballot_forced() ? k_rs_pass_p<THREADS, BITS, 0> : k_rs_pass_p<THREADS, BITS, 1>;
    hipLaunchKernelGGL(pass, dim3(u.grid), dim3(THREADS), 0, stream, keys, alt, n, u.n_tiles, 32u + u.low_bits + 8, u.hi_bits,
                       (const unsigned long long *)nullptr, (unsigned long long *)nullptr, u.tickets.p, d_fail, 0u, u.cur_a.p,
                       RS_CURSOR_STRIDE, 64u, 0u);
    SW_HIP(hipGetLastError());
}

void radix_unsort_perm_second(UnsortPerm &u, const uint64_t *keys, uint64_t *alt, uint64_t n, hipStream_t stream, uint32_t *d_fail)
{
    constexpr int THREADS = 512, BITS = 8;
    auto pass = ballot_forced() ? k_rs_pass_p<THREADS, BITS, 0> : k_rs_pass_p<THREADS, BITS, 1>;
    hipLaunchKernelGGL(pass, dim3(u.grid), dim3(THREADS), 0, stream, keys, alt, n, u.n_tiles, 32u + u.low_bits, 8u,
                       (const unsigned long long *)nullptr, (unsigned long long *)nullptr, u.tickets.p + 1, d_fail, 0u, u.cur_b.p, 1u,
                       u.low_bits + 8, 0u);
    SW_HIP(hipGetLastError());
}

bool radix_unsort_perm(uint64_t *&keys, uint64_t *&alt, uint64_t n, unsigned low_bits, unsigned nbit, hipStream_t stream, uint32_t *d_fail)
{
    UnsortPerm u;
    if (!radix_unsort_perm_begin(u, n, low_bits, nbit, stream)) return false;
    radix_unsort_perm_first(u, keys, alt, n, stream, d_fail);
    std::swap(keys, alt);
    radix_unsort_perm_second(u, keys, alt, n, stream, d_fail);
    std::swap(keys, alt);
    return true;
}

bool radix_pairs_available() { return rank_mode() == 1; }
int radix_rank_mode() { return rank_mode(); }

uint64_t radix_trim_state()
{
    uint64_t freed = 0;
    if (g_state_uses) return 0;
    std::lock_guard<std::mutex> lock(state_registry_mu());
    for (auto &kv : state_registry()) {
        StateBuf &b = *kv.second;
        std::unique_lock<std::mutex> use(b.mu, std::try_to_lock);
        if (!use.owns_lock() || !b.p) continue;
        int cur = -1;
        (void)hipGetDevice(&cur);
        if (cur != kv.first.first) (void)hipSetDevice(kv.first.first);
        (void)hipFree(b.p);
        if (cur != kv.first.first && cur >= 0) (void)hipSetDevice(cur);
        freed += b.words * 8;
        b.p = nullptr;
        b.words = 0;
        b.epoch = 0;
    }
    return freed;
}

void radix_demote_rank()
{
    int dev = 0;
    SW_HIP(hipGetDevice(&dev));
    std::lock_guard<std::mutex> lock(rank_mu());
    rank_modes()[dev] = 0;
}

void radix_sort_pairs32(uint32_t *&keys, uint32_t *&keys_alt, OccPay *&vals, OccPay *&vals_alt, uint64_t n, unsigned end_bit,
                        hipStream_t stream, uint32_t *d_fail, const StageSource *src, const std::function<void()> &after_first,
                        uint32_t *low_out)
{
    constexpr uint32_t RADIX = 1u << RP_BITS, TILE = RP_THREADS * RP_ITEMS;
    if (n == 0 || end_bit == 0) return;
    if (end_bit > 32 || end_bit % RP_BITS) raise(SW_ERR_RUNTIME, "radix_sort_pairs32: key bits must be a multiple of 8 up to 32");
    if (n >= 0xFFFFFFFFull) raise(SW_ERR_RUNTIME, "radix_sort_pairs32: more than 2^32-2 elements");
    const unsigned n_passes = end_bit / RP_BITS;
    const uint64_t n_tiles = (n + TILE - 1) / TILE;
    int grid_p = 0;
    {
        static std::mutex &mu = *new std::mutex;
        static std::map<int, int> &grids = *new std::map<int, int>;
        int dev = 0;
        SW_HIP(hipGetDevice(&dev));
        std::lock_guard<std::mutex> lock(mu);
        int &g = grids[dev];
        if (!g) {
            int per_cu = 0;
            hipDeviceProp_t prop;
            SW_HIP(hipGetDeviceProperties(&prop, dev));
            SW_HIP(hipOccupancyMaxActiveBlocksPerMultiprocessor(&per_cu, k_rs_pair_pass<0>, RP_THREADS, 0));
            g = std::max(1, per_cu) * std::max(1, prop.multiProcessorCount);
        }
        grid_p = g;
    }
    DevArray<unsigned long long> hist((size_t)n_passes * RADIX);
    DevArray<uint32_t> tickets(n_passes);
    SW_HIP(hipMemsetAsync(tickets.p, 0, tickets.bytes(), stream));
    SW_HIP(hipMemsetAsync(hist.p, 0, hist.bytes(), stream));
    StageSource stage{};
    DevArray<uint32_t> chunk_tile;
    DevArray<unsigned long long> chunk_dir;
    if (src && src->rows) {
        stage = *src;
        hipLaunchKernelGGL(k_rs_hist32_rows, dim3((unsigned)((n + 16383) / 16384)), dim3(256), 0, stream,
                           reinterpret_cast<const uint4 *>(src->rows), n, n_passes, hist.p);
    } else if (src) {
        constexpr uint64_t CHUNK = 64 * RP_ITEMS;
        static_assert(TILE == (RP_THREADS / 64) * CHUNK, "a tile is one chunk per wave");
        const uint64_t n_chunks = (n + CHUNK - 1) / CHUNK;
        stage = *src;
        chunk_tile.alloc(n_chunks);
        chunk_dir.alloc(n_chunks * STAGE_ROW);
        stage.chunk_dir = chunk_dir.p;
        hipLaunchKernelGGL(k_rs_chunk_tiles, dim3((stage.n_tiles + 255u) / 256u), dim3(256), 0, stream, stage.tile_count, stage.dst_off,
                           stage.n_tiles, chunk_tile.p);
        hipLaunchKernelGGL(k_rs_stage_prepare, dim3((unsigned)std::min<uint64_t>(2048, (n_chunks + 3) / 4)), dim3(256), 0, stream, stage,
                           (const uint32_t *)chunk_tile.p, n, n_passes, chunk_dir.p, hist.p);
    } else {
        hipLaunchKernelGGL(k_rs_hist32, dim3((unsigned)((n + 65535) / 65536)), dim3(256), 0, stream, keys, n, n_passes, hist.p);
    }
    SW_HIP(hipGetLastError());
    StateUse su = state_buf(stream, (size_t)n_tiles * RADIX);
    StateBuf &sb = su.b;
    const StageSource none{};
    const uint32_t fault = fault_rank();
    for (unsigned p = 0; p < n_passes; ++p) {
        hipLaunchKernelGGL(k_rs_scan<RP_BITS>, dim3(1), dim3(RADIX), 0, stream, hist.p + (size_t)p * RADIX, (unsigned long long *)nullptr);
        const uint32_t epoch = next_epoch(sb, stream);
        const dim3 grid((unsigned)std::min<uint64_t>(n_tiles, (uint64_t)grid_p));
        if (p == 0 && src) {
            auto first = src->rows ? k_rs_pair_pass<2> : k_rs_pair_pass<1>;
            hipLaunchKernelGGL(first, grid, dim3(RP_THREADS), 0, stream, (const uint32_t *)nullptr, (const uint4 *)nullptr,
                               keys_alt, reinterpret_cast<uint4 *>(vals_alt), n, (uint32_t)n_tiles, 0u,
                               (const unsigned long long *)hist.p, sb.p, epoch, tickets.p, d_fail, stage,
                               n_passes == 1 ? low_out : (uint32_t *)nullptr, fault);
            SW_HIP(hipGetLastError());
            if (after_first) after_first();
        } else {
            hipLaunchKernelGGL(k_rs_pair_pass<0>, grid, dim3(RP_THREADS), 0, stream, (const uint32_t *)keys,
                               reinterpret_cast<const uint4 *>(vals), keys_alt, reinterpret_cast<uint4 *>(vals_alt), n, (uint32_t)n_tiles,
                               RP_BITS * p, (const unsigned long long *)(hist.p + (size_t)p * RADIX), sb.p, epoch, tickets.p + p, d_fail,
                               none, p + 1 == n_passes ? low_out : (uint32_t *)nullptr, fault);
            SW_HIP(hipGetLastError());
        }
        std::swap(keys, keys_alt);
        std::swap(vals, vals_alt);
    }
}

namespace {
constexpr uint32_t EB_RADIX = 512, EB_TABLE = EB_RADIX * EB_RADIX, EB_THREADS = 512;
constexpr uint64_t EB_EMPTY = ~0ull;
static_assert(EB_THREADS == EB_RADIX, "k_eb_finish: one bin per thread");
enum : uint32_t { EB_F_OVERFLOW = 1u, EB_F_RANGE = 2u, EB_F_ORDER = 4u };
struct EbInfo {
    unsigned long long n_sentinels;
    uint32_t n_tiles2, max_bucket, flags, n_runs, n_live, pad;
};

__global__ __launch_bounds__(EB_RADIX) void k_eb_level1(const unsigned long long *__restrict__ h1, uint32_t tile_keys,
                                                        unsigned long long *__restrict__ cursor, unsigned long long *__restrict__ segtab,
                                                        EbInfo *__restrict__ info)
{
    __shared__ unsigned long long s[EB_RADIX];
    __shared__ uint32_t st[EB_RADIX];
    const uint32_t d = threadIdx.x;
    const unsigned long long c = h1[d];
    const uint32_t tiles = (uint32_t)((c + tile_keys - 1) / tile_keys);
    s[d] = c;
    st[d] = tiles;
    __syncthreads();
    for (uint32_t o = 1; o < EB_RADIX; o <<= 1) {
        const unsigned long long a = d >= o ? s[d - o] : 0;
        const uint32_t b = d >= o ? st[d - o] : 0;
        __syncthreads();
        s[d] += a;
        st[d] += b;
        __syncthreads();
    }
    const unsigned long long first = s[d] - c;
    cursor[(size_t)d * RS_CURSOR_STRIDE] = first;
    uint32_t w = st[d] - tiles;
    for (uint32_t t = 0; t < tiles; ++t)
        segtab[w + t] = seg_pack(first + (uint64_t)t * tile_keys, d, (uint32_t)min((unsigned long long)tile_keys, c - (uint64_t)t * tile_keys));
    if (d == EB_RADIX - 1) info->n_tiles2 = st[d];
}

__global__ __launch_bounds__(1024) void k_eb_count(const uint64_t *__restrict__ in, const unsigned long long *__restrict__ segtab,
                                                   const EbInfo *__restrict__ info, unsigned shift, uint32_t dmask, uint64_t sentinel,
                                                   uint32_t *__restrict__ table, EbInfo *__restrict__ out)
{
    __shared__ uint32_t hist[EB_RADIX];
    __shared__ uint32_t s_sent;
    const uint32_t n_tiles = info->n_tiles2;
    for (uint32_t w = blockIdx.x; w < n_tiles; w += gridDim.x) {
        const unsigned long long seg = segtab[w];
        const uint64_t first = seg_first(seg);
        const uint32_t cnt = seg_count(seg);
        if (threadIdx.x < EB_RADIX) hist[threadIdx.x] = 0;
        if (threadIdx.x == 0) s_sent = 0;
        __syncthreads();
        uint64_t key[RS_ITEMS];
#pragma unroll
        for (int i = 0; i < RS_ITEMS; ++i) {
            const uint32_t li = i * 1024 + threadIdx.x;
            key[i] = li < cnt ? in[first + li] : EB_EMPTY;
        }
        uint32_t sent = 0;
#pragma unroll
        for (int i = 0; i < RS_ITEMS; ++i) {
            if (key[i] == EB_EMPTY) continue;
            if (key[i] == sentinel) ++sent;
            atomicAdd(&hist[(uint32_t)(key[i] >> shift) & dmask], 1u);
        }
        if (sent) atomicAdd(&s_sent, sent);
        __syncthreads();
        if (threadIdx.x < EB_RADIX && hist[threadIdx.x]) atomicAdd(&table[seg_bucket(seg) * EB_RADIX + threadIdx.x], hist[threadIdx.x]);
        if (threadIdx.x == 0 && s_sent) atomicAdd(&out->n_sentinels, (unsigned long long)s_sent);
        __syncthreads();
    }
}

__global__ __launch_bounds__(1024) void k_eb_scan(const uint32_t *__restrict__ cnt, const unsigned long long *__restrict__ n_sent,
                                                  uint32_t sent_at, uint32_t *__restrict__ start, unsigned long long *__restrict__ cursor,
                                                  uint32_t *__restrict__ max_out, uint32_t *__restrict__ total_out,
                                                  uint4 *__restrict__ live, uint32_t *__restrict__ n_live_out)
{
    constexpr uint32_t PER4 = EB_TABLE / 1024 / 4;
    __shared__ uint32_t ws[16], wm[16], wz[16];
    const uint32_t tid = threadIdx.x, lane = tid & 63u, wave = tid >> 6;
    const uint32_t sent = n_sent ? (uint32_t)*n_sent : 0u;
    const uint4 *cnt4 = reinterpret_cast<const uint4 *>(cnt) + (size_t)tid * PER4;
    uint32_t sum = 0, mx = 0, nz = 0;
#pragma unroll 16
    for (uint32_t j = 0; j < PER4; ++j) {
        const uint4 c = cnt4[j];
        mx = max(max(max(mx, c.x), max(c.y, c.z)), c.w);
        sum += c.x + c.y + c.z + c.w;
        nz += (c.x != 0) + (c.y != 0) + (c.z != 0) + (c.w != 0);
    }
    if (n_sent && sent_at / (4 * PER4) == tid) {
        mx = 0;
        for (uint32_t j = 0; j < 4 * PER4; ++j) {
            const uint32_t i = tid * 4 * PER4 + j, c = cnt[i];
            mx = max(mx, c - (i == sent_at ? min(c, sent) : 0u));
        }
    }
    uint32_t incl = sum, inz = nz;
    for (uint32_t o = 1; o < 64; o <<= 1) {
        const uint32_t up = __shfl_up(incl, o, 64), uz = __shfl_up(inz, o, 64);
        if (lane >= o) {
            incl += up;
            inz += uz;
        }
        mx = max(mx, __shfl_xor(mx, o, 64));
    }
    if (lane == 63) {
        ws[wave] = incl;
        wz[wave] = inz;
    }
    if (lane == 0) wm[wave] = mx;
    __syncthreads();
    uint32_t run = incl - sum, below = inz - nz, n_live = 0;
    for (uint32_t w = 0; w < 16; ++w) {
        if (w < wave) {
            run += ws[w];
            below += wz[w];
        }
        n_live += wz[w];
    }
    uint32_t at = n_live - 1u - below;
    uint4 *start4 = reinterpret_cast<uint4 *>(start) + (size_t)tid * PER4;
    ulonglong2 *cur2 = reinterpret_cast<ulonglong2 *>(cursor) + (size_t)tid * PER4 * 2;
#pragma unroll 16
    for (uint32_t j = 0; j < PER4; ++j) {
        const uint4 c = cnt4[j];
        const uint4 st = make_uint4(run, run + c.x, run + c.x + c.y, run + c.x + c.y + c.z);
        start4[j] = st;
        if (cursor) {
            cur2[2 * j] = make_ulonglong2(st.x, st.y);
            cur2[2 * j + 1] = make_ulonglong2(st.z, st.w);
        }
        if (live) {
            const uint32_t id = (tid * PER4 + j) * 4;
            if (c.x) live[at--] = make_uint4(id, st.x, c.x, 0u);
            if (c.y) live[at--] = make_uint4(id + 1, st.y, c.y, 0u);
            if (c.z) live[at--] = make_uint4(id + 2, st.z, c.z, 0u);
            if (c.w) live[at--] = make_uint4(id + 3, st.w, c.w, 0u);
        }
        run = st.w + c.w;
    }
    if (tid == 1023) {
        start[EB_TABLE] = run;
        if (total_out) *total_out = run;
        if (n_live_out) *n_live_out = n_live;
        uint32_t m = 0;
        for (uint32_t w = 0; w < 16; ++w) m = max(m, wm[w]);
        if (max_out) *max_out = m;
    }
}
// ... 418 lines not shown
```

Before: 491.7.

## Sort compact hash/payload pairs and recover record ids via coarse lookup table

Adds a compact node-payload path. The radix sort moves 64-bit hash words plus 64-bit packed payload words instead of 32-bit keys plus 16-byte OccPay records, and the record id is dropped from the sorted payload. The nodes kernel recovers each record id with a coarse-table-guided binary search over per-record first indices. This cuts bytes moved per sort pass and per scatter, at the cost of extra dependent lookups in the nodes kernel and templated repair and settle paths.

```diff
diff --git a/seqwin_amd/csrc/device.hpp b/seqwin_amd/csrc/device.hpp
--- a/seqwin_amd/csrc/device.hpp
+++ b/seqwin_amd/csrc/device.hpp
@@ -270,6 +270,8 @@
 void radix_sort_pairs32(uint32_t *&keys, uint32_t *&keys_alt, OccPay *&vals, OccPay *&vals_alt, uint64_t n, unsigned end_bit,
                         hipStream_t stream, uint32_t *d_fail, const StageSource *src = nullptr,
                         const std::function<void()> &after_first = std::function<void()>(), uint32_t *low_out = nullptr);
+void radix_sort_hashpay(uint64_t *&hash, uint64_t *&hash_alt, uint64_t *&pw, uint64_t *&pw_alt, uint64_t n, unsigned end_bit,
+                        hipStream_t stream, uint32_t *d_fail, const StageSource &src, const std::function<void()> &after_first);
 bool sort_pairs32(uint32_t *&keys, uint32_t *&keys_alt, OccPay *&vals, OccPay *&vals_alt, uint64_t n, unsigned end_bit,
                   hipStream_t stream, uint32_t *d_fail, uint32_t *low_out = nullptr);
 struct PartState;
@@ -287,6 +289,7 @@
     DevArray<uint64_t> dst_off;
     uint32_t stage_tiles = 0;
     uint64_t stage_mult = 0;
+    DevArray<uint32_t> rec_first, rec_coarse;
     uint64_t n = 0;
     PartState *part = nullptr;
     OrderedOcc() = default;
@@ -298,6 +301,7 @@
             rec = std::move(o.rec); cand_rows = std::move(o.cand_rows); n = o.n; o.n = 0;
             staged = o.staged; o.staged = false; stage = std::move(o.stage); dst_off = std::move(o.dst_off);
             stage_tiles = o.stage_tiles; stage_mult = o.stage_mult;
+            rec_first = std::move(o.rec_first); rec_coarse = std::move(o.rec_coarse);
             part_state_delete(part); part = o.part; o.part = nullptr;
         }
         return *this;
diff --git a/seqwin_amd/csrc/index.hip b/seqwin_amd/csrc/index.hip
--- a/seqwin_amd/csrc/index.hip
+++ b/seqwin_amd/csrc/index.hip
@@ -6,6 +6,7 @@
 #include <rocprim/rocprim.hpp>
 
 #include "device.hpp"
+#include "rec_table.hpp"
 
 namespace sw {
 
@@ -222,7 +223,7 @@
     uint32_t cnt[NODES_DIGITS];
     uint32_t lstart[NODES_DIGITS];
 };
-template <bool BITS, bool REP, bool SCAT = false>
+template <bool BITS, bool REP, bool SCAT = false, bool CP = false>
 __global__ __launch_bounds__(NODES_THREADS) void k_nodes(const uint32_t *__restrict__ key32, const OccPay *__restrict__ pay, uint64_t n,
                                                uint64_t base, const uint32_t *__restrict__ rec_flag, sw_kmer *__restrict__ kmers,
                                                uint64_t *__restrict__ node_hash, uint32_t *__restrict__ node_start,
@@ -231,8 +232,12 @@
                                                unsigned long long *__restrict__ tbits, unsigned long long *__restrict__ nbits,
                                                unsigned long long *__restrict__ tile_state, uint32_t *__restrict__ ticket,
                                                uint32_t *__restrict__ n_nodes_out, uint32_t *__restrict__ order_bad,
-                                               unsigned long long *__restrict__ cursor, uint32_t dig_shift, uint32_t dig_mask)
-{
+                                               unsigned long long *__restrict__ cursor, uint32_t dig_shift, uint32_t dig_mask,
+                                               const uint32_t *__restrict__ rec_first, const uint32_t *__restrict__ rec_coarse)
+{
+    const uint64_t *hash64 = reinterpret_cast<const uint64_t *>(key32), *pw64 = reinterpret_cast<const uint64_t *>(pay);
+    constexpr uint32_t NO_IDX = 0xFFFFFFFFu;
+    uint32_t xidx[NODES_ROWS];
     __shared__ uint32_t s_tile, s_excl;
     __shared__ uint32_t s_row[NODES_ROWS * NODES_WAVES];
     static_assert(NODES_ROWS * NODES_WAVES <= 128, "the (row, wave) group counts are scanned by one wave, two per lane");
@@ -255,7 +260,21 @@
         const uint64_t s = s0 + (uint64_t)r * NODES_ROW + 2 * threadIdx.x;
         k[r][0] = k[r][1] = 0;
         p[r][0] = p[r][1] = OccPay{0, 0, 0, 0};
-        if (s + 1 < n) {
+        xidx[r] = NO_IDX;
+        if constexpr (CP) {
+            if (s + 1 < n) {
+                const uint4 hh = *reinterpret_cast<const uint4 *>(hash64 + s), ww = *reinterpret_cast<const uint4 *>(pw64 + s);
+                k[r][0] = hh.y;
+                k[r][1] = hh.w;
+                p[r][0] = OccPay{hh.x, ww.x, 0, ww.y};
+                p[r][1] = OccPay{hh.z, ww.z, 0, ww.w};
+            } else if (s < n) {
+                const uint2 hh = *reinterpret_cast<const uint2 *>(hash64 + s), ww = *reinterpret_cast<const uint2 *>(pw64 + s);
+                k[r][0] = hh.y;
+                p[r][0] = OccPay{hh.x, ww.x, 0, ww.y};
+            }
+            if (REP && lane == 63 && s + 2 < n) xidx[r] = reinterpret_cast<const uint2 *>(pw64 + s + 2)->y;
+        } else if (s + 1 < n) {
             const uint2 kk = *reinterpret_cast<const uint2 *>(key32 + s);
             k[r][0] = kk.x;
             k[r][1] = kk.y;
@@ -266,13 +285,21 @@
             p[r][0] = pay[s];
         }
         uint32_t pk = __shfl_up(k[r][1], 1, 64), plow = __shfl_up(p[r][1].low, 1, 64), pidx = __shfl_up(p[r][1].idx, 1, 64);
-        prec[r] = __shfl_up(p[r][1].rec, 1, 64);
+        if constexpr (!CP) prec[r] = __shfl_up(p[r][1].rec, 1, 64);
         if (lane == 0 && s < n && s) {
-            pk = key32[s - 1];
-            const OccPay q = pay[s - 1];
-            plow = q.low;
-            prec[r] = q.rec;
-            pidx = q.idx;
+            if constexpr (CP) {
+                const uint2 hq = *reinterpret_cast<const uint2 *>(hash64 + s - 1);
+                pk = hq.y;
+                plow = hq.x;
+                pidx = reinterpret_cast<const uint2 *>(pw64 + s - 1)->y;
+                xidx[r] = pidx;
+            } else {
+                pk = key32[s - 1];
+                const OccPay q = pay[s - 1];
+                plow = q.low;
+                prec[r] = q.rec;
+                pidx = q.idx;
+            }
         }
         const bool h0 = s < n && (s == 0 || k[r][0] != pk || p[r][0].low != plow);
         const bool h1 = s + 1 < n && (k[r][1] != k[r][0] || p[r][1].low != p[r][0].low);
@@ -294,6 +321,47 @@
         if (lane == 0) s_row[r * NODES_WAVES + wave] = (uint32_t)__popcll(b0) + (uint32_t)__popcll(b1);
     }
     if (misorder && lane == 0) atomicAdd(order_bad, (uint32_t)__popcll(misorder));
+    if constexpr (CP) {
+        constexpr int NS = (BITS || REP) ? 3 : 2;
+        uint32_t lo[NODES_ROWS][NS], hi[NODES_ROWS][NS];
+#pragma unroll
+        for (int r = 0; r < NODES_ROWS; ++r)
+#pragma unroll
+            for (int e = 0; e < NS; ++e) {
+                const uint64_t s = s0 + (uint64_t)r * NODES_ROW + 2 * threadIdx.x;
+                const uint32_t idx = e < 2 ? p[r][e].idx : xidx[r];
+                const bool live = e < 2 ? s + e < n : idx != NO_IDX;
+                lo[r][e] = hi[r][e] = 0;
+                if (live) {
+                    lo[r][e] = rec_coarse[idx >> REC_COARSE_SHIFT];
+                    hi[r][e] = rec_coarse[(idx >> REC_COARSE_SHIFT) + 1u];
+                }
+            }
+        bool more;
+        do {
+            more = false;
+#pragma unroll
+            for (int r = 0; r < NODES_ROWS; ++r)
+#pragma unroll
+                for (int e = 0; e < NS; ++e)
+                    if (lo[r][e] < hi[r][e]) {
+                        const uint32_t idx = e < 2 ? p[r][e].idx : xidx[r];
+                        const uint32_t mid = lo[r][e] + ((hi[r][e] - lo[r][e] + 1u) >> 1);
+                        if (rec_first[mid] <= idx) lo[r][e] = mid; else hi[r][e] = mid - 1u;
+                        more |= lo[r][e] < hi[r][e];
+                    }
+        } while (more);
+#pragma unroll
+        for (int r = 0; r < NODES_ROWS; ++r) {
+            p[r][0].rec = lo[r][0];
+            p[r][1].rec = lo[r][1];
+            prec[r] = 0;
+            if constexpr (NS == 3) {
+                prec[r] = __shfl_up(lo[r][1], 1, 64);
+                if (lane == 0 || lane == 63) prec[r] = lo[r][2];
+            }
+        }
+    }
     uint32_t drank[NODES_ROWS][2];
     if constexpr (SCAT) {
 #pragma unroll
@@ -397,10 +465,17 @@
             if (lane == 63) {
                 nlive = s + 2 < n;
                 if (nlive) {
-                    nk = key32[s + 2];
-                    const OccPay q = pay[s + 2];
-                    nlow = q.low;
-                    nf = rec_flag[q.rec];
+                    if constexpr (CP) {
+                        const uint2 hq = *reinterpret_cast<const uint2 *>(hash64 + s + 2);
+                        nk = hq.y;
+                        nlow = hq.x;
+                        nf = rec_flag[prec[r]];
+                    } else {
+                        nk = key32[s + 2];
+                        const OccPay q = pay[s + 2];
+                        nlow = q.low;
+                        nf = rec_flag[q.rec];
+                    }
                 }
             }
             const bool same01 = live1 && !h1 && (f1 >> 1) == (f0 >> 1);
@@ -1649,6 +1724,21 @@
     __device__ void store(uint64_t q, uint64_t, const uint64_t &v) const { keys[q] = v; }
 };
 
+struct HashPay {
+    uint64_t h, pw;
+};
+struct HashView {
+    using Key = uint32_t;
+    using Elem = HashPay;
+    uint64_t *hash;
+    uint64_t *pw;
+    __device__ uint32_t key(uint64_t q) const { return (uint32_t)(hash[q] >> 32); }
+    __device__ uint64_t low(uint64_t q) const { return hash[q]; }
+    __device__ static uint64_t low_of(const HashPay &v) { return v.h; }
+    __device__ void load(uint64_t q, uint32_t &k, HashPay &v) const { v.h = hash[q]; v.pw = pw[q]; k = (uint32_t)(v.h >> 32); }
+    __device__ void store(uint64_t q, uint32_t, const HashPay &v) const { hash[q] = v.h; pw[q] = v.pw; }
+};
+
 template <class View>
 __device__ __forceinline__ uint32_t descents_of_thread(const View &V, typename View::Key kmask, uint64_t n, uint64_t q0, uint32_t *heads = nullptr)
 {
@@ -1701,6 +1791,32 @@
         if (q == 0 || kq[i] != kp || lq[i] != lp) hm |= 1u << i;
         kp = kq[i];
         lp = lq[i];
+    }
+    if (heads) *heads = (uint32_t)__popc(hm);
+    return m;
+}
+
+__device__ __forceinline__ uint32_t descents_of_thread(const HashView &V, uint32_t kmask, uint64_t n, uint64_t q0, uint32_t *heads = nullptr)
+{
+    uint32_t m = 0, hm = 0;
+    if (heads) *heads = 0;
+    if (q0 >= n) return 0;
+    uint64_t hq[4];
+    if (q0 + 4 <= n) {
+        const ulonglong2 a = *reinterpret_cast<const ulonglong2 *>(V.hash + q0), b = *reinterpret_cast<const ulonglong2 *>(V.hash + q0 + 2);
+        hq[0] = a.x; hq[1] = a.y; hq[2] = b.x; hq[3] = b.y;
+    } else {
+#pragma unroll
+        for (uint32_t i = 0; i < 4; ++i) hq[i] = (q0 + i < n) ? V.hash[q0 + i] : 0ull;
+    }
+    uint64_t hp = q0 ? V.hash[q0 - 1] : 0;
+#pragma unroll
+    for (uint32_t i = 0; i < 4; ++i) {
+        const uint64_t q = q0 + i;
+        if (q >= n) break;
+        if (q && ((uint32_t)(hq[i] >> 32) & kmask) == ((uint32_t)(hp >> 32) & kmask) && hq[i] < hp) m |= 1u << i;
+        if (q == 0 || hq[i] != hp) hm |= 1u << i;
+        hp = hq[i];
     }
     if (heads) *heads = (uint32_t)__popc(hm);
     return m;
@@ -2102,7 +2218,10 @@
     SW_HIP(hipGetLastError());
 }
 
-__global__ void k_bad_runs(const uint32_t *__restrict__ bad, uint32_t n_bad, const uint32_t *__restrict__ key32,
+__device__ __forceinline__ uint32_t run_key(const uint32_t *keys, uint64_t q) { return keys[q]; }
+__device__ __forceinline__ uint32_t run_key(const uint64_t *keys, uint64_t q) { return (uint32_t)(keys[q] >> 32); }
+template <class K>
+__global__ void k_bad_runs(const uint32_t *__restrict__ bad, uint32_t n_bad, const K *__restrict__ key32,
                            uint32_t kmask, uint64_t n, uint32_t *__restrict__ run_start, uint32_t *__restrict__ run_len)
 {
     const uint32_t i = blockIdx.x * blockDim.x + threadIdx.x;
@@ -2116,21 +2235,22 @@
     uint64_t lo = 0, hi = n;
     while (lo < hi) {
         const uint64_t mid = (lo + hi) >> 1;
-        if ((key32[mid] & kmask) < k) lo = mid + 1; else hi = mid;
+        if ((run_key(key32, mid) & kmask) < k) lo = mid + 1; else hi = mid;
     }
     const uint64_t a = lo;
     hi = n;
     while (lo < hi) {
         const uint64_t mid = (lo + hi) >> 1;
-        if ((key32[mid] & kmask) <= k) lo = mid + 1; else hi = mid;
+        if ((run_key(key32, mid) & kmask) <= k) lo = mid + 1; else hi = mid;
     }
     run_start[i] = (uint32_t)a;
     run_len[i] = (uint32_t)(lo - a);
 }
 
-__global__ void k_gather_sub(const uint32_t *__restrict__ key32, const OccPay *__restrict__ pay,
+template <class K, class V>
+__global__ void k_gather_sub(const K *__restrict__ key32, const V *__restrict__ pay,
                              const uint32_t *__restrict__ run_start, const uint64_t *__restrict__ run_off, uint32_t n_bad,
-                             uint64_t n_sub, uint64_t *__restrict__ sub_h, OccPay *__restrict__ sub_v,
+                             uint64_t n_sub, uint64_t *__restrict__ sub_h, V *__restrict__ sub_v,
                              uint32_t *__restrict__ pos)
 {
     const uint64_t t = (uint64_t)blockIdx.x * blockDim.x + threadIdx.x;
@@ -2145,19 +2265,22 @@
         q = (uint64_t)run_start[lo] + (t - run_off[lo]);
         pos[t] = (uint32_t)q;
     }
-    const OccPay v = pay[q];
-    sub_h[t] = ((uint64_t)key32[q] << 32) | v.low;
+    const V v = pay[q];
+    if constexpr (sizeof(K) == 8) sub_h[t] = key32[q];
+    else sub_h[t] = ((uint64_t)key32[q] << 32) | v.low;
     sub_v[t] = v;
 }
 
-__global__ void k_scatter_sub(const uint64_t *__restrict__ sub_h, const OccPay *__restrict__ sub_v,
-                              const uint32_t *__restrict__ pos, uint64_t n_sub, uint32_t *__restrict__ key32,
-                              OccPay *__restrict__ pay)
+template <class K, class V>
+__global__ void k_scatter_sub(const uint64_t *__restrict__ sub_h, const V *__restrict__ sub_v,
+                              const uint32_t *__restrict__ pos, uint64_t n_sub, K *__restrict__ key32,
+                              V *__restrict__ pay)
 {
     const uint64_t t = (uint64_t)blockIdx.x * blockDim.x + threadIdx.x;
     if (t >= n_sub) return;
     const uint64_t q = pos ? pos[t] : t;
-    key32[q] = (uint32_t)(sub_h[t] >> 32);
+    if constexpr (sizeof(K) == 8) key32[q] = sub_h[t];
+    else key32[q] = (uint32_t)(sub_h[t] >> 32);
     pay[q] = sub_v[t];
 }
 
@@ -2175,7 +2298,17 @@
     DevArray<uint32_t> low;
     const uint64_t *rows_src = nullptr;
     OrderedOcc *staged = nullptr;
+    bool compact = false;
+    DevArray<uint64_t> h_a, h_b, pw_a, pw_b;
+    uint64_t *hash = nullptr, *pw = nullptr;
+    DevArray<uint32_t> rec_first, rec_coarse;
 };
+
+bool node_payload_compact()
+{
+    const char *e = SW_TEST_GETENV("SEQWIN_AMD_NODE_PAYLOAD");
+    return !(e && !strcmp(e, "wide"));
+}
 
 void sort_pay(uint64_t n, hipStream_t stream, PaySort &o)
 {
@@ -2186,6 +2319,42 @@
     }
     o.kmask = ~0u << (32 - bits);
     o.n = n;
+    o.compact = o.staged && o.staged->rec_first.p && node_payload_compact();
+    if (o.compact) {
+        OrderedOcc &occ = *o.staged;
+        StageSource S{};
+        S.stage_hash = occ.stage.stage_hash.p;
+        S.stage_kmer = occ.stage.stage_kmer.p;
+        S.tile_count = occ.stage.tile_count.p;
+        S.tile_offset = occ.stage.tile_offset.p;
+        S.dst_off = occ.dst_off.p;
+        S.n_tiles = occ.stage_tiles;
+        S.mult = occ.stage_mult;
+        S.rec_out = occ.rec.p;
+        o.rec_first = std::move(occ.rec_first);
+        o.rec_coarse = std::move(occ.rec_coarse);
+        o.fail.alloc(1);
+        SW_HIP(hipMemsetAsync(o.fail.p, 0, 4, stream));
+        o.h_b.alloc(n);
+        o.pw_b.alloc(n);
+        uint64_t *h = nullptr, *h_alt = o.h_b.p, *pw = nullptr, *pw_alt = o.pw_b.p;
+        radix_sort_hashpay(h, h_alt, pw, pw_alt, n, bits, stream, o.fail.p, S, [&] {
+            occ.stage = SketchOut();
+            occ.dst_off.release();
+            occ.staged = false;
+            o.h_a.alloc(n);
+            o.pw_a.alloc(n);
+            h = o.h_a.p;
+            pw = o.pw_a.p;
+        });
+        o.staged = nullptr;
+        o.hash = h;
+        o.pw = pw;
+        o.cap = (uint32_t)std::min<uint64_t>(n, std::max<uint64_t>(1u << 16, n / 16));
+        o.bad.alloc(o.cap);
+        enqueue_repair(HashView{h, pw}, HashView{h, pw}, o.kmask, n, o.bad.p, o.cap, o.rep, stream);
+        return;
+    }
     o.key_b.alloc(n);
     o.pay_b.alloc(n);
     uint32_t *keys = o.key_a.p, *keys_alt = o.key_b.p;
@@ -2252,16 +2421,22 @@
     else enqueue_repair(PayView{keys, vals}, PayView{keys, vals}, o.kmask, n, o.bad.p, o.cap, o.rep, stream);
 }
 
+template <class K, class V>
+bool settle_general(PaySort &o, K *keys, V *vals, unsigned long long D, hipStream_t stream);
 bool sort_pay_settle(PaySort &o, unsigned long long D, uint32_t status, hipStream_t stream)
 {
     if (D == 0 || status == 0) {
         o.n_repaired = D;
         return false;
     }
+    if (o.compact) return settle_general(o, o.hash, o.pw, D, stream);
+    return settle_general(o, o.key32, o.pay, D, stream);
+}
+template <class K, class V>
+bool settle_general(PaySort &o, K *keys, V *vals, unsigned long long D, hipStream_t stream)
+{
     const uint64_t n = o.n;
     const uint32_t kmask = o.kmask, cap = o.cap;
-    uint32_t *keys = o.key32;
-    OccPay *vals = o.pay;
     DevArray<uint32_t> &bad = o.bad;
     uint64_t n_sub = n;
     DevArray<uint32_t> run_start, run_len, pos;
@@ -2272,7 +2447,7 @@
         run_start.alloc(nb);
         run_len.alloc(nb);
         run_off.alloc((size_t)nb + 1);
-        hipLaunchKernelGGL(k_bad_runs, dim3((unsigned)blocks_for(nb)), dim3(TPB), 0, stream, bad.p, nb, keys, kmask, n,
+        hipLaunchKernelGGL(k_bad_runs<K>, dim3((unsigned)blocks_for(nb)), dim3(TPB), 0, stream, (const uint32_t *)bad.p, nb, (const K *)keys, kmask, n,
                            run_start.p, run_len.p);
         SW_HIP(hipGetLastError());
         exclusive_sum(rocprim::make_transform_iterator(run_len.p, U32ToU64()), run_off.p, nb, (uint64_t)0, stream);
@@ -2285,14 +2460,14 @@
         pos.alloc(n_sub);
     }
     DevArray<uint64_t> sh0(n_sub), sh1(n_sub);
-    DevArray<OccPay> sp0(n_sub), sp1(n_sub);
-    hipLaunchKernelGGL(k_gather_sub, dim3(blocks_for(n_sub)), dim3(TPB), 0, stream, keys, vals, run_start.p,
+    DevArray<V> sp0(n_sub), sp1(n_sub);
+    hipLaunchKernelGGL((k_gather_sub<K, V>), dim3(blocks_for(n_sub)), dim3(TPB), 0, stream, keys, vals, run_start.p,
                        listed ? run_off.p : (const uint64_t *)nullptr, (uint32_t)(listed ? D : 0), n_sub, sh0.p, sp0.p, pos.p);
     SW_HIP(hipGetLastError());
     uint64_t *sk = sh0.p, *sk_alt = sh1.p;
-    OccPay *sv = sp0.p, *sv_alt = sp1.p;
+    V *sv = sp0.p, *sv_alt = sp1.p;
     sort_pairs(sk, sk_alt, sv, sv_alt, n_sub, 0, 64, stream);
-    hipLaunchKernelGGL(k_scatter_sub, dim3(blocks_for(n_sub)), dim3(TPB), 0, stream, sk, sv,
+    hipLaunchKernelGGL((k_scatter_sub<K, V>), dim3(blocks_for(n_sub)), dim3(TPB), 0, stream, sk, sv,
                        listed ? pos.p : (const uint32_t *)nullptr, n_sub, keys, vals);
     SW_HIP(hipGetLastError());
     SW_HIP(hipStreamSynchronize(stream));
@@ -2356,6 +2531,35 @@
     if (i >= n) return;
     key32[i] = (uint32_t)(key64[i] >> 32);
     if (pay[i].idx == 0xFFFFFFFFu) atomicAdd(bad, 1u);
+}
+__global__ void k_compact_to_wide(const uint64_t *__restrict__ hash, const uint64_t *__restrict__ pw, uint64_t n,
+                                  const uint32_t *__restrict__ rec_first, const uint32_t *__restrict__ rec_coarse, uint64_t n_cells,
+                                  uint32_t *__restrict__ key32, OccPay *__restrict__ pay)
+{
+    const uint64_t i = (uint64_t)blockIdx.x * blockDim.x + threadIdx.x;
+    if (i >= n) return;
+    const uint64_t h = hash[i], w = pw[i];
+    OccPay p;
+    p.low = (uint32_t)h;
+    p.pos = (uint32_t)w;
+    p.idx = (uint32_t)(w >> 32);
+    p.rec = (p.idx >> REC_COARSE_SHIFT) < n_cells ? rec_of_index(rec_first, rec_coarse, p.idx) : 0u;
+    key32[i] = (uint32_t)(h >> 32);
+    pay[i] = p;
+}
+void to_wide(PaySort &ps, uint64_t n, hipStream_t stream)
+{
+    ps.key_a.alloc(n);
+    ps.pay_a.alloc(n);
+    hipLaunchKernelGGL(k_compact_to_wide, dim3(blocks_for(n)), dim3(TPB), 0, stream, (const uint64_t *)ps.hash, (const uint64_t *)ps.pw, n,
+                       (const uint32_t *)ps.rec_first.p, (const uint32_t *)ps.rec_coarse.p, rec_coarse_cells(n), ps.key_a.p, ps.pay_a.p);
+    SW_HIP(hipGetLastError());
+    ps.h_a.release(); ps.h_b.release(); ps.pw_a.release(); ps.pw_b.release();
+    ps.hash = ps.pw = nullptr;
+    ps.pay_b.alloc(n);
+    ps.key32 = ps.key_a.p;
+    ps.pay = ps.pay_a.p;
+    ps.compact = false;
 }
 void resort_pay_stable(PaySort &ps, uint64_t n, hipStream_t stream)
 {
@@ -2418,14 +2622,27 @@
         const bool fused = want_fused && rank_out && !direct && nbit > UNSORT_BITS && sort_keys64_is_own(n) &&
                            radix_unsort_perm_begin(perm, n, UNSORT_BITS, nbit, stream);
         {
+            const bool cp = ps.compact;
             auto launch = [&](auto kern) {
-                hipLaunchKernelGGL(kern, dim3(blocks), dim3(NODES_THREADS), 0, stream, ps.key32, ps.pay, n, base, rec_flag, ix.kmers.p,
+                hipLaunchKernelGGL(kern, dim3(blocks), dim3(NODES_THREADS), 0, stream, cp ? (const uint32_t *)ps.hash : (const uint32_t *)ps.key32,
+                                   cp ? (const OccPay *)ps.pw : (const OccPay *)ps.pay, n, base, rec_flag, ix.kmers.p,
                                    np.hash.p, np.start.p, direct ? rank_out : (uint32_t *)nullptr, fused ? uv1.p : uv0.p,
                                    bits ? tbits->p : (unsigned long long *)nullptr, bits ? nbits->p : (unsigned long long *)nullptr,
                                    tile_state.p, words.p, words.p + 1, words.p + 3, fused ? perm.cur_a.p : (unsigned long long *)nullptr,
-                                   fused ? perm.low_bits + 8 : 0u, fused ? (1u << perm.hi_bits) - 1u : 0u);
+                                   fused ? perm.low_bits + 8 : 0u, fused ? (1u << perm.hi_bits) - 1u : 0u,
+                                   (const uint32_t *)ps.rec_first.p, (const uint32_t *)ps.rec_coarse.p);
             };
-            if (fused) {
+            if (cp && fused) {
+                if (bits && rep) launch(k_nodes<true, true, true, true>);
+                else if (bits) launch(k_nodes<true, false, true, true>);
+                else if (rep) launch(k_nodes<false, true, true, true>);
+                else launch(k_nodes<false, false, true, true>);
+            } else if (cp) {
+                if (bits && rep) launch(k_nodes<true, true, false, true>);
+                else if (bits) launch(k_nodes<true, false, false, true>);
+                else if (rep) launch(k_nodes<false, true, false, true>);
+                else launch(k_nodes<false, false, false, true>);
+            } else if (fused) {
                 if (bits && rep) launch(k_nodes<true, true, true>);
                 else if (bits) launch(k_nodes<true, false, true>);
                 else if (rep) launch(k_nodes<false, true, true>);
@@ -2457,13 +2674,14 @@
         SW_HIP(hipMemcpyAsync(back, words.p + 1, 12, hipMemcpyDeviceToHost, stream));
         SW_HIP(hipStreamSynchronize(stream));
         if (getenv("SEQWIN_AMD_DEBUG_NODES"))
-            fprintf(stderr, "[nodes] %llu occurrences (indices of %u bits), attempt %d: unsort route %s, %u nodes, order guard %u\n",
-                    (unsigned long long)n, nbit, attempt, route, back[0], back[2]);
+            fprintf(stderr, "[nodes] %llu occurrences (indices of %u bits), attempt %d: payload %s, unsort route %s, %u nodes, order guard %u\n",
+                    (unsigned long long)n, nbit, attempt, ps.compact ? "compact" : "wide", route, back[0], back[2]);
         if (back[2] == 0) break;
         if (attempt)
             raise(SW_ERR_RUNTIME, "internal error: the node sort is still out of order after the rocPRIM re-sort (%u places)", back[2]);
         order_guard_tripped(0, back[2]);
         radix_demote_rank();
+        if (ps.compact) to_wide(ps, n, stream);
         resort_pay_stable(ps, n, stream);
     }
     const uint32_t n_nodes = back[0];
@@ -2715,13 +2933,33 @@
 
 }
 
+static bool stage_keybits_ok()
+{
+    const char *e = SW_TEST_GETENV("SEQWIN_AMD_SORT_KEYBITS");
+    if (!e) return true;
+    const int b = atoi(e);
+    return node_payload_compact() && b >= 8 && b <= 32 && b % 8 == 0;
+}
 static bool stage_fits_sort(uint64_t n, uint32_t n_tiles)
 {
     if (const char *e = SW_TEST_GETENV("SEQWIN_AMD_ORDER")) {
         if (!strcmp(e, "copy")) return false;
-        if (!strcmp(e, "stage")) return n > 0 && radix_pairs_available() && !SW_TEST_GETENV("SEQWIN_AMD_SORT_KEYBITS");
-    }
-    return n > 0 && sort_pairs_is_own(n, 32) && !SW_TEST_GETENV("SEQWIN_AMD_SORT_KEYBITS") && n / 16 >= n_tiles;
+        if (!strcmp(e, "stage")) return n > 0 && radix_pairs_available() && stage_keybits_ok();
+    }
+    return n > 0 && sort_pairs_is_own(n, 32) && stage_keybits_ok() && n / 16 >= n_tiles;
+}
+
+__global__ void k_rec_first(const uint32_t *__restrict__ rec_tile_off, const uint64_t *__restrict__ dst_off, uint32_t n_records,
+                            uint32_t *__restrict__ rec_first)
+{
+    const uint32_t r = blockIdx.x * blockDim.x + threadIdx.x;
+    if (r <= n_records) rec_first[r] = (uint32_t)dst_off[rec_tile_off[r]];
+}
+__global__ void k_rec_coarse(const uint32_t *__restrict__ rec_first, uint32_t n_records, uint64_t n, uint64_t n_entries,
+                             uint32_t *__restrict__ rec_coarse)
+{
+    const uint64_t c = (uint64_t)blockIdx.x * blockDim.x + threadIdx.x;
+    if (c < n_entries) rec_coarse[c] = rec_coarse_entry(rec_first, n_records, n, c);
 }
 
 __global__ void k_fill_u64(uint64_t *p, uint32_t n, uint64_t v)
@@ -2742,6 +2980,19 @@
         exclusive_sum(rocprim::make_transform_iterator(sk.tile_count.p, U32ToU64()), out.dst_off.p, plan.n_tiles, (uint64_t)0, stream);
         hipLaunchKernelGGL(k_fill_u64, dim3(1), dim3(64), 0, stream, out.dst_off.p + plan.n_tiles, STAGE_PAD, out.n);
         SW_HIP(hipGetLastError());
+        out.rec_first.release();
+        out.rec_coarse.release();
+        if (node_payload_compact() && plan.rec_tile_off.n >= 2 && out.n < 0xFFFFFFFFull) {
+            const uint32_t n_records = (uint32_t)(plan.rec_tile_off.n - 1);
+            const uint64_t n_entries = rec_coarse_cells(out.n) + 1;
+            out.rec_first.alloc((size_t)n_records + 1);
+            out.rec_coarse.alloc(n_entries);
+            hipLaunchKernelGGL(k_rec_first, dim3((unsigned)blocks_for((uint64_t)n_records + 1)), dim3(TPB), 0, stream,
+                               (const uint32_t *)plan.rec_tile_off.p, (const uint64_t *)out.dst_off.p, n_records, out.rec_first.p);
+            hipLaunchKernelGGL(k_rec_coarse, dim3((unsigned)blocks_for(n_entries)), dim3(TPB), 0, stream, (const uint32_t *)out.rec_first.p,
+                               n_records, out.n, n_entries, out.rec_coarse.p);
+            SW_HIP(hipGetLastError());
+        }
         out.stage = std::move(sk);
         out.stage_tiles = plan.n_tiles;
         out.stage_mult = plan.mult;
@@ -3253,6 +3504,10 @@
         ps.key_a = std::move(occ.key32);
         ps.pay_a = std::move(occ.pay);
         if (occ.staged) ps.staged = &occ;
+        if (occ.rec_first.p && occ.rec_first.n != n_records + 1) {
+            occ.rec_first.release();
+            occ.rec_coarse.release();
+        }
         group_occurrences(ps, n, 0, rec_flag.p, stream, ix, by_table ? nullptr : rank.p, bits ? &tbits : nullptr,
                           bits ? &nbits : nullptr, pair_edges ? &rep_marked : nullptr, pair_edges ? &unsort_hold : nullptr, &parts);
         if (!bits || by_table) {
diff --git a/seqwin_amd/csrc/radix.hip b/seqwin_amd/csrc/radix.hip
--- a/seqwin_amd/csrc/radix.hip
+++ b/seqwin_amd/csrc/radix.hip
@@ -578,7 +578,7 @@
 }
 
 constexpr int RP_THREADS = 1024, RP_ITEMS = 7, RP_BITS = 8;
-template <int SRC>
+template <int SRC, bool CP = false>
 __global__ __launch_bounds__(RP_THREADS) void k_rs_pair_pass(const uint32_t *__restrict__ kin, const uint4 *__restrict__ pin,
                                                              uint32_t *__restrict__ kout, uint4 *__restrict__ pout, uint64_t n,
                                                              uint32_t n_tiles, unsigned shift,
@@ -588,9 +588,10 @@
                                                              const StageSource S, uint32_t *__restrict__ lowout, uint32_t fault)
 {
     constexpr bool STAGE = SRC == 1, ROWS = SRC == 2;
+    static_assert(!(ROWS && CP), "the received rows keep OccPay");
     constexpr uint32_t THREADS = RP_THREADS, ITEMS = RP_ITEMS, RADIX = 1u << RP_BITS, WAVES = THREADS / 64, TILE = THREADS * ITEMS;
     __shared__ uint4 sp[TILE];
-    __shared__ uint32_t skey[TILE];
+    __shared__ uint32_t skey[CP ? 1 : TILE];
     __shared__ uint16_t whist[WAVES][RADIX];
     __shared__ uint32_t lstart[RADIX];
     __shared__ unsigned long long goff[RADIX];
@@ -628,8 +629,15 @@
             for (int i = 0; i < (int)ITEMS; ++i) {
                 const uint64_t g = (uint64_t)tl * TILE + wave * (64 * ITEMS) + i * 64 + lane;
                 const bool in_range = tl < n_tiles && g < n;
-                key[i] = in_range ? kin[g] : ~0u;
-                pay[i] = in_range ? pin[g] : uint4{0, 0, 0, 0};
+                if constexpr (CP) {
+                    const uint2 h = in_range ? reinterpret_cast<const uint2 *>(kin)[g] : uint2{0, ~0u};
+                    const uint2 pw = in_range ? reinterpret_cast<const uint2 *>(pin)[g] : uint2{0, 0};
+                    key[i] = h.y;
+                    pay[i] = uint4{h.x, h.y, pw.x, pw.y};
+                } else {
+                    key[i] = in_range ? kin[g] : ~0u;
+                    pay[i] = in_range ? pin[g] : uint4{0, 0, 0, 0};
+                }
             }
         } else {
 #pragma unroll
@@ -683,7 +691,8 @@
                 h ^= h >> 27;
                 const uint32_t rec = pay[i].w;
                 key[i] = li < cnt_tile ? (uint32_t)(h >> 32) : ~0u;
-                pay[i] = uint4{(uint32_t)h, pay[i].z, rec, (uint32_t)(t0 + li)};
+                if constexpr (CP) pay[i] = uint4{(uint32_t)h, (uint32_t)(h >> 32), pay[i].z, (uint32_t)(t0 + li)};
+                else pay[i] = uint4{(uint32_t)h, pay[i].z, rec, (uint32_t)(t0 + li)};
                 if (li < cnt_tile) S.rec_out[t0 + li] = rec;
             }
         }
@@ -746,7 +755,7 @@
                 const uint32_t d = (key[i] >> shift) & (RADIX - 1u);
                 const uint32_t at = pos[i] + lstart[d] + whist[wave][d];
                 if (li < cnt_tile) {
-                    skey[at] = key[i];
+                    if constexpr (!CP) skey[at] = key[i];
                     sp[at] = pay[i];
                 }
             }
@@ -800,12 +809,19 @@
         for (int j = 0; j < (int)ITEMS; ++j) {
             const uint32_t t = j * THREADS + tid;
             if (t < cnt_tile) {
-                const uint32_t k = skey[t];
-                const uint64_t dst = goff[(k >> shift) & (RADIX - 1u)] + t;
-                const uint4 pv = sp[t];
-                kout[dst] = k;
-                pout[dst] = pv;
-                if (lowout) lowout[dst] = pv.x;
+                if constexpr (CP) {
+                    const uint4 pv = sp[t];
+                    const uint64_t dst = goff[(pv.y >> shift) & (RADIX - 1u)] + t;
+                    reinterpret_cast<uint2 *>(kout)[dst] = uint2{pv.x, pv.y};
+                    reinterpret_cast<uint2 *>(pout)[dst] = uint2{pv.z, pv.w};
+                } else {
+                    const uint32_t k = skey[t];
+                    const uint64_t dst = goff[(k >> shift) & (RADIX - 1u)] + t;
+                    const uint4 pv = sp[t];
+                    kout[dst] = k;
+                    pout[dst] = pv;
+                    if (lowout) lowout[dst] = pv.x;
+                }
             }
         }
         tile = ntile;
@@ -872,7 +888,8 @@
 }
 
 __global__ __launch_bounds__(256) void k_rs_stage_prepare(const StageSource S, const uint32_t *__restrict__ chunk_tile, uint64_t n,
-                                                          unsigned n_passes, unsigned long long *__restrict__ chunk_dir,
+                                                          unsigned n_passes, unsigned key_shift,
+                                                          unsigned long long *__restrict__ chunk_dir,
                                                           unsigned long long *__restrict__ hist)
 {
     constexpr uint32_t RADIX = 1u << RP_BITS, CHUNK = 64 * RP_ITEMS;
@@ -933,7 +950,7 @@
             if (c0 + i * 64 + lane < n) {
                 unsigned long long v = hv[i] * S.mult;
                 v ^= v >> 27;
-                const uint32_t k = (uint32_t)(v >> 32);
+                const uint32_t k = (uint32_t)(v >> 32) >> key_shift;
                 for (unsigned p = 0; p < n_passes; ++p) atomicAdd(&h[p * RADIX + ((k >> (RP_BITS * p)) & (RADIX - 1u))], 1u);
             }
         }
@@ -1219,10 +1236,22 @@
     rank_modes()[dev] = 0;
 }
 
-void radix_sort_pairs32(uint32_t *&keys, uint32_t *&keys_alt, OccPay *&vals, OccPay *&vals_alt, uint64_t n, unsigned end_bit,
-                        hipStream_t stream, uint32_t *d_fail, const StageSource *src, const std::function<void()> &after_first,
-                        uint32_t *low_out)
-{
+namespace {
+void sort_pairs32_impl(void *&keys_v, void *&keys_alt_v, void *&vals_v, void *&vals_alt_v, uint64_t n, unsigned end_bit,
+                       hipStream_t stream, uint32_t *d_fail, const StageSource *src, const std::function<void()> &after_first,
+                       uint32_t *low_out, bool compact)
+{
+    uint32_t *keys = (uint32_t *)keys_v, *keys_alt = (uint32_t *)keys_alt_v;
+    OccPay *vals = (OccPay *)vals_v, *vals_alt = (OccPay *)vals_alt_v;
+    auto step = [&] {
+        std::swap(keys_v, keys_alt_v);
+        std::swap(vals_v, vals_alt_v);
+    };
+    auto reload = [&] {
+        keys = (uint32_t *)keys_v; keys_alt = (uint32_t *)keys_alt_v;
+        vals = (OccPay *)vals_v; vals_alt = (OccPay *)vals_alt_v;
+    };
+    const unsigned key_shift = compact ? 32 - end_bit : 0;
     constexpr uint32_t RADIX = 1u << RP_BITS, TILE = RP_THREADS * RP_ITEMS;
     if (n == 0 || end_bit == 0) return;
     if (end_bit > 32 || end_bit % RP_BITS) raise(SW_ERR_RUNTIME, "radix_sort_pairs32: key bits must be a multiple of 8 up to 32");
@@ -1268,7 +1297,7 @@
         hipLaunchKernelGGL(k_rs_chunk_tiles, dim3((stage.n_tiles + 255u) / 256u), dim3(256), 0, stream, stage.tile_count, stage.dst_off,
                            stage.n_tiles, chunk_tile.p);
         hipLaunchKernelGGL(k_rs_stage_prepare, dim3((unsigned)std::min<uint64_t>(2048, (n_chunks + 3) / 4)), dim3(256), 0, stream, stage,
-                           (const uint32_t *)chunk_tile.p, n, n_passes, chunk_dir.p, hist.p);
+                           (const uint32_t *)chunk_tile.p, n, n_passes, key_shift, chunk_dir.p, hist.p);
     } else {
         hipLaunchKernelGGL(k_rs_hist32, dim3((unsigned)((n + 65535) / 65536)), dim3(256), 0, stream, keys, n, n_passes, hist.p);
     }
@@ -1282,23 +1311,52 @@
         const uint32_t epoch = next_epoch(sb, stream);
         const dim3 grid((unsigned)std::min<uint64_t>(n_tiles, (uint64_t)grid_p));
         if (p == 0 && src) {
-            auto first = src->rows ? k_rs_pair_pass<2> : k_rs_pair_pass<1>;
+            auto first = src->rows ? k_rs_pair_pass<2> : compact ? k_rs_pair_pass<1, true> : k_rs_pair_pass<1>;
             hipLaunchKernelGGL(first, grid, dim3(RP_THREADS), 0, stream, (const uint32_t *)nullptr, (const uint4 *)nullptr,
-                               keys_alt, reinterpret_cast<uint4 *>(vals_alt), n, (uint32_t)n_tiles, 0u,
+                               keys_alt, reinterpret_cast<uint4 *>(vals_alt), n, (uint32_t)n_tiles, key_shift,
                                (const unsigned long long *)hist.p, sb.p, epoch, tickets.p, d_fail, stage,
                                n_passes == 1 ? low_out : (uint32_t *)nullptr, fault);
             SW_HIP(hipGetLastError());
             if (after_first) after_first();
         } else {
-            hipLaunchKernelGGL(k_rs_pair_pass<0>, grid, dim3(RP_THREADS), 0, stream, (const uint32_t *)keys,
+            auto pass = compact ? k_rs_pair_pass<0, true> : k_rs_pair_pass<0>;
+            hipLaunchKernelGGL(pass, grid, dim3(RP_THREADS), 0, stream, (const uint32_t *)keys,
                                reinterpret_cast<const uint4 *>(vals), keys_alt, reinterpret_cast<uint4 *>(vals_alt), n, (uint32_t)n_tiles,
-                               RP_BITS * p, (const unsigned long long *)(hist.p + (size_t)p * RADIX), sb.p, epoch, tickets.p + p, d_fail,
-                               none, p + 1 == n_passes ? low_out : (uint32_t *)nullptr, fault);
+                               key_shift + RP_BITS * p, (const unsigned long long *)(hist.p + (size_t)p * RADIX), sb.p, epoch, tickets.p + p,
+                               d_fail, none, p + 1 == n_passes ? low_out : (uint32_t *)nullptr, fault);
             SW_HIP(hipGetLastError());
         }
-        std::swap(keys, keys_alt);
-        std::swap(vals, vals_alt);
-    }
+        step();
+        reload();
+    }
+}
+}
+
+void radix_sort_pairs32(uint32_t *&keys, uint32_t *&keys_alt, OccPay *&vals, OccPay *&vals_alt, uint64_t n, unsigned end_bit,
+                        hipStream_t stream, uint32_t *d_fail, const StageSource *src, const std::function<void()> &after_first,
+                        uint32_t *low_out)
+{
+    void *k = keys, *ka = keys_alt, *v = vals, *va = vals_alt;
+    sort_pairs32_impl(k, ka, v, va, n, end_bit, stream, d_fail, src, [&] {
+        if (after_first) after_first();
+        k = keys;
+        v = vals;
+    }, low_out, false);
+    keys = (uint32_t *)k; keys_alt = (uint32_t *)ka;
+    vals = (OccPay *)v; vals_alt = (OccPay *)va;
+}
+
+void radix_sort_hashpay(uint64_t *&hash, uint64_t *&hash_alt, uint64_t *&pw, uint64_t *&pw_alt, uint64_t n, unsigned end_bit,
+                        hipStream_t stream, uint32_t *d_fail, const StageSource &src, const std::function<void()> &after_first)
+{
+    void *k = hash, *ka = hash_alt, *v = pw, *va = pw_alt;
+    sort_pairs32_impl(k, ka, v, va, n, end_bit, stream, d_fail, &src, [&] {
+        after_first();
+        k = hash;
+        v = pw;
+    }, nullptr, true);
+    hash = (uint64_t *)k; hash_alt = (uint64_t *)ka;
+    pw = (uint64_t *)v; pw_alt = (uint64_t *)va;
 }
 
 namespace {
diff --git a/seqwin_amd/csrc/rec_table.hpp b/seqwin_amd/csrc/rec_table.hpp
--- /dev/null
+++ b/seqwin_amd/csrc/rec_table.hpp
@@ -0,0 +1,38 @@
+#pragma once
+#include <cstdint>
+
+#if defined(__HIPCC__)
+#define SW_REC_HD __host__ __device__ __forceinline__
+#else
+#define SW_REC_HD inline
+#endif
+
+namespace sw {
+
+constexpr unsigned REC_COARSE_SHIFT = 10;
+
+SW_REC_HD uint64_t rec_coarse_cells(uint64_t n) { return (n + ((1ull << REC_COARSE_SHIFT) - 1)) >> REC_COARSE_SHIFT; }
+
+SW_REC_HD uint32_t rec_search(const uint32_t *first, uint32_t lo, uint32_t hi, uint32_t idx)
+{
+    while (lo < hi) {
+        const uint32_t mid = lo + ((hi - lo + 1u) >> 1);
+        if (first[mid] <= idx) lo = mid; else hi = mid - 1u;
+    }
+    return lo;
+}
+
+SW_REC_HD uint32_t rec_coarse_entry(const uint32_t *first, uint32_t n_records, uint64_t n, uint64_t c)
+{
+    const uint64_t i = c << REC_COARSE_SHIFT;
+    if (i >= n) return n_records - 1u;
+    return rec_search(first, 0u, n_records - 1u, (uint32_t)i);
+}
+
+SW_REC_HD uint32_t rec_of_index(const uint32_t *first, const uint32_t *coarse, uint32_t idx)
+{
+    const uint32_t c = idx >> REC_COARSE_SHIFT;
+    return rec_search(first, coarse[c], coarse[c + 1u], idx);
+}
+
+}
```

Measured after the change: 476.4. 0.969x the previous value.
